# AjayAlluri/realtime-fraud-detection

Measured on AMD Instinct MI355X. Metric: scored transactions/sec (whole node), higher is better.
Workload: dtype f32 (features f64, forests f32/f64, blend f64)

## Files before the change

### include/fdengine.h

```cpp
#ifndef FDENGINE_H
#define FDENGINE_H

#include <stddef.h>
#include <stdint.h>

#ifdef __cplusplus
extern "C" {
#endif

#define FD_ABI_VERSION 15

enum fd_status {
  FD_OK = 0,
  FD_ERR_INVALID_ARG = 1,
  FD_ERR_HIP = 2,
  FD_ERR_NOT_LOADED = 3,
  FD_ERR_UNSUPPORTED = 4,
  FD_ERR_OOM = 5,
  FD_ERR_IO = 6,
};

enum fd_forest_kind {
  FD_FOREST_XGB_BINARY_LOGISTIC = 1,
  FD_FOREST_SKLEARN_IFOREST = 2,
  FD_FOREST_SKLEARN_PROBA = 3,
};

typedef struct fd_engine fd_engine;

typedef struct {
  int32_t n_trees;
  const int64_t* tree_offsets;
  const int32_t* left;
  const int32_t* right;
  const int32_t* feature;
  const double* threshold;
  const uint8_t* default_left;
  const double* leaf_value;
} fd_tree_arrays;

typedef struct {
  int32_t kind;
  int32_t num_feature;
  double base_score;
  double if_offset;
  double if_denominator;
} fd_forest_params;

#define FD_MAX_MODELS 8
enum fd_blend_strategy { FD_BLEND_WEIGHTED_AVERAGE = 0, FD_BLEND_VOTING = 1, FD_BLEND_STACKING = 2 };
enum fd_decision { FD_APPROVE = 0, FD_REVIEW = 1, FD_DECLINE = 2, FD_APPROVE_WITH_MONITORING = 3 };
enum fd_risk { FD_VERY_LOW = 0, FD_LOW = 1, FD_MEDIUM = 2, FD_HIGH = 3, FD_CRITICAL = 4 };
typedef struct {
  int32_t n_models;
  int32_t strategy;
  double weight[FD_MAX_MODELS];
  double conf_mult[FD_MAX_MODELS];
  double fraud_threshold;
  double confidence_threshold;
} fd_blend_params;

const char* fd_last_error(void);
int fd_abi_version(void);
const char* fd_build_id(void);
int fd_device_count(int* out);
int fd_engine_create(int device, fd_engine** out);
int fd_engine_destroy(fd_engine* eng);
int fd_engine_set_stream(fd_engine* eng, void* hip_stream);
int fd_engine_reset_stream(fd_engine* eng);
int fd_engine_sync(fd_engine* eng);

int fd_load_forest(fd_engine* eng, int slot, const fd_forest_params* params, const fd_tree_arrays* trees);
int fd_unload_forest(fd_engine* eng, int slot);

int fd_load_xgboost_json(fd_engine* eng, int slot, const char* path);

int fd_xgboost_json_read(const char* path, fd_forest_params* params, int32_t* n_trees, int64_t* n_nodes,
                         fd_tree_arrays* trees);
int fd_forest_info(fd_engine* eng, int slot, int32_t* n_trees, int32_t* depth, int32_t* num_feature);

int fd_forest_predict_device(fd_engine* eng, int slot, const float* d_X, int64_t n, int32_t ld,
                             double* d_prob, double* d_raw, int32_t* d_leaf);
int fd_forest_predict_host(fd_engine* eng, int slot, const float* X, int64_t n, int32_t ld,
                           double* prob, double* raw, int32_t* leaf);

typedef struct {
  int32_t n_trees;
  int32_t n_chunks;
  int32_t chunk;
  int32_t depth;
  int64_t tree_bytes;
  int64_t chunk_stride;
  int64_t blob_bytes;
  int64_t n_leaf_ids;
  float base_margin;
  int32_t layout;
  int64_t n_thresholds;
  int32_t bin_steps;
} fd_pack_info;
int fd_pack_forest_host(const fd_forest_params* params, const fd_tree_arrays* trees, void* blob,
                        int64_t blob_cap, int32_t* leaf_ids, int64_t ids_cap, fd_pack_info* info);
int fd_pack_forest_binned_host(const fd_forest_params* params, const fd_tree_arrays* trees, void* blob,
                               int64_t blob_cap, float* thresholds, int64_t thr_cap, int32_t* offsets,
                               fd_pack_info* info);

typedef struct {
  int32_t kind;
  int32_t n_trees;
  int32_t depth;
  int32_t leaf_bytes;
  int64_t n_nodes;
  int64_t n_leaves;
  float base_margin;
  int32_t pad;
} fd_sparse_info;
int fd_pack_forest_sparse_host(const fd_forest_params* params, const fd_tree_arrays* trees, void* nodes,
                               int64_t nodes_cap, void* leaf_values, int64_t values_cap, int32_t* leaf_ids,
                               int64_t ids_cap, fd_sparse_info* info);

int fd_blend_device(fd_engine* eng, const fd_blend_params* params, int64_t n,
                    const double* const* d_probs, const uint8_t* present,
                    double* d_fraud_prob, double* d_confidence, uint8_t* d_decision, uint8_t* d_risk);
int fd_blend_host(fd_engine* eng, const fd_blend_params* params, int64_t n,
                  const double* const* probs, const uint8_t* present,
                  double* fraud_prob, double* confidence, uint8_t* decision, uint8_t* risk);

enum fd_window_mode {
  FD_WINDOW_REDIS_COMPAT = 0,
  FD_WINDOW_SLIDING = 1
};
#define FD_RAW_FEATURES 16
#define FD_VECTOR_WIDTH 64
#define FD_MAX_SEQ_LEN 16
typedef struct {
  int64_t capacity;
  int32_t window_mode;
  int32_t ring_k;
  int32_t seq_len;
} fd_state_params;
int fd_state_init(fd_engine* eng, const fd_state_params* params);
int fd_state_clear(fd_engine* eng);
int fd_state_info(fd_engine* eng, int64_t* capacity, int64_t* cards);
typedef struct {
  int64_t n;
  const uint64_t* key;
  const double* avg_amount;
  const int32_t* account_age_days;
  const uint64_t* device_fp;
} fd_users;
int fd_state_load_users_host(fd_engine* eng, const fd_users* users);
typedef struct {
  int64_t n;
  const double* fraud_rate;
  const double* risk_multiplier;
} fd_merchants;
int fd_load_merchants_host(fd_engine* eng, const fd_merchants* merchants);
typedef struct {
  const uint64_t* card_key;
  const int64_t* ts_ms;
  const int64_t* amount_cents;
  const int32_t* merchant;
  const uint64_t* device_fp;
  const uint8_t* ip_class;
  const uint8_t* hour;
  const uint8_t* weekend;
} fd_txn_batch;
int fd_features_device(fd_engine* eng, const fd_txn_batch* txns, int64_t n, float* d_vectors, double* d_raw);
int fd_features_host(fd_engine* eng, const fd_txn_batch* txns, int64_t n, float* vectors, double* raw);

#define FD_FEATURE_MAP_WIDTH 64
#define FD_CODE_UNKNOWN 254
typedef struct {
  const double* geo_lat;
  const double* geo_lon;
  const double* merchant_lat;
  const double* merchant_lon;
  const uint8_t* payment_method;
  const uint8_t* transaction_type;
  const uint8_t* card_type;
  const uint8_t* user_agent_flag;
  const double* fraud_score;
} fd_txn_context;
typedef struct {
  double tp_score;
  double fe_score;
  uint8_t tp_decision;
  uint8_t tp_risk;
  uint8_t fe_decision;
  uint8_t fe_risk;
  uint8_t pad[4];
} fd_rule_scores;
typedef struct {
  int64_t n;
  const uint64_t* key;
  const double* risk_score;
  const uint8_t* kyc_status;
  const uint8_t* verified;
  const int8_t* pref_start;
  const int8_t* pref_end;
  const double* weekend_activity;
  const double* online_preference;
  const double* intl_preference;
  const int32_t* txn_frequency;
  const uint8_t* has_patterns;
} fd_users_ext;
typedef struct {
  int64_t n;
  const double* avg_amount;
  const uint8_t* risk_level;
  const uint8_t* blacklisted;
  const uint8_t* category;
  const uint8_t* high_risk_category;
  const uint8_t* open_hour;
  const uint8_t* close_hour;
  const uint8_t* suspicious_name;
} fd_merchants_ext;
int fd_state_load_users_ext_host(fd_engine* eng, const fd_users_ext* users);
int fd_load_merchants_ext_host(fd_engine* eng, const fd_merchants_ext* merchants);
int fd_load_vocab_host(fd_engine* eng, const uint8_t* payment_high_risk, const uint8_t* type_is_refund);
int fd_features_full_device(fd_engine* eng, const fd_txn_batch* txns, const fd_txn_context* ctx, int64_t n,
                            float* d_vectors, double* d_raw, double* d_fmap, fd_rule_scores* d_rules);

typedef struct {
  int32_t input_size;
  int32_t hidden;
  int32_t n_out;
  const float* w_ih;
  const float* w_hh;
  const float* b_ih;
  const float* b_hh;
  const float* w_out;
  const float* b_out;
} fd_lstm_params;
int fd_load_lstm(fd_engine* eng, const fd_lstm_params* params);
int fd_unload_lstm(fd_engine* eng);
int fd_lstm_predict_device(fd_engine* eng, const float* d_seq, int64_t n, int32_t T, double* d_prob);
int fd_lstm_predict_host(fd_engine* eng, const float* seq, int64_t n, int32_t T, double* prob);
#define FD_SLOT_LSTM 64
int fd_features_seq_device(fd_engine* eng, const fd_txn_batch* txns, int64_t n, float* d_vectors, double* d_raw,
                           float* d_seq);

typedef struct {
  int32_t n_layers;
  int32_t dims[9];
  const float* weight[8];
  const float* bias[8];
} fd_mlp_params;
int fd_load_mlp(fd_engine* eng, const fd_mlp_params* params);
int fd_unload_mlp(fd_engine* eng);
int fd_mlp_info(fd_engine* eng, int32_t* n_layers, int32_t* in_dim, int32_t* hidden);
int fd_mlp_predict_device(fd_engine* eng, const float* d_X, int64_t n, int32_t ld, double* d_prob);
int fd_mlp_predict_host(fd_engine* eng, const float* X, int64_t n, int32_t ld, double* prob);
int fd_pack_mlp_host(const fd_mlp_params* params, void* blob, int64_t cap, int64_t* bytes);
#define FD_SLOT_MLP 65

#define FD_GRAPH_FEATURES 5
typedef struct {
// ... 249 lines not shown
```

### realtime-fraud-detection_amd/csrc/engine.hip

```cpp
#include <algorithm>
#include <chrono>
#include <mutex>
#include <cstring>
#include <string>

#include "blend_row.h"
#include "abtest_row.h"
#include "fd_internal.h"
#include "graph_row.h"
#include "host_stage.h"
#include "ingest_parse.h"
#include "text_row.h"

namespace fd {

static thread_local std::string g_last_error;

void set_error(const std::string& msg) { g_last_error = msg; }

Engine::Timed* Engine::next_event_pair(int kind) {
  if (timing_every > 1 && kind >= 0 && kind < 16 && (timing_seq[kind]++ % (unsigned)timing_every) != 0)
    return nullptr;
  if (events_used == events.size()) {
    hipEvent_t a, b;
// ... 361 lines not shown
    ok = fd::comm_sync_stream(e, e.pipe_slot_stream) && ok;
    FD_REQUIRE(ok, FD_ERR_HIP, "engine leaked: streams still busy " + std::to_string(e.comm.timeout_ms) +
                                   " ms after the communicators were aborted (" + e.comm.abort_reason + ")");
  }
  (void)hipStreamSynchronize(e.stream);
  for (auto& f : e.forests) {
    for (auto* b : {&f.split.bins, &f.split.nan, &f.split.leaves}) b->release();
    f.blob.release();
    f.leaf_ids.release();
    f.b_blob.release();
    f.b_thr.release();
    f.b_thr_off.release();
  }
  e.stage.release();
  e.scratch_probs.release();
  e.feat_vec.release();
  fd::windows_release(e);
  fd::sink_release(e);
  fd::graph_release(e);
  fd::text_release(e);
  fd::ab_release(e);
  for (auto* b : {&e.route_blk, &e.route_blk_stream, &e.route_out, &e.route_err, &e.seq_buf, &e.seq_desc, &e.lstm.wpk, &e.lstm.wpk4, &e.lstm.bias,
                  &e.lstm.wout, &e.lstm.bout, &e.state.seq, &e.mlp.blob})
    b->release();
  if (e.aux_stream) {
    (void)hipStreamSynchronize(e.aux_stream);
    (void)hipStreamDestroy(e.aux_stream);
    (void)hipEventDestroy(e.fork_ev);
    (void)hipEventDestroy(e.join_ev);
  }
  if (e.aux2_stream) {
    (void)hipStreamSynchronize(e.aux2_stream);
    (void)hipStreamDestroy(e.aux2_stream);
    (void)hipEventDestroy(e.join2_ev);
  }
  try {
    fd::comm_destroy(e);
  } catch (...) {
  }
  for (hipStream_t st : e.pipe_stream)
    if (st) {
      (void)hipStreamSynchronize(st);
      (void)hipStreamDestroy(st);
    }
  if (e.pipe_slot_stream) {
    (void)hipStreamSynchronize(e.pipe_slot_stream);
    (void)hipStreamDestroy(e.pipe_slot_stream);
  }
  if (e.pipe_entry_ev) (void)hipEventDestroy(e.pipe_entry_ev);
  for (int k = 0; k < Engine::kPipeSlots; ++k) {
    if (e.pipe_slot_ev[k]) (void)hipEventDestroy(e.pipe_slot_ev[k]);
    if (e.pipe_feat_ev[k]) (void)hipEventDestroy(e.pipe_feat_ev[k]);
    if (e.pipe_copy_ev[k]) (void)hipEventDestroy(e.pipe_copy_ev[k]);
    e.pipe_vec[k].release();
    e.pipe_out[k].release();
    e.pipe_seq[k].release();
  }
  for (int k = 0; k < Engine::kSplitRing; ++k) {
    if (e.pipe_done_ev[k]) (void)hipEventDestroy(e.pipe_done_ev[k]);
    e.pipe_split[k].release();
  }
  for (auto* b : {&e.state.uext, &e.state.mext, &e.state.vocab, &e.feat_ext}) b->release();
  for (auto& P1 : e.ens1)
    for (auto* b : {&P1.nodes[0], &P1.nodes[1], &P1.thr}) b->release();
  for (auto* b : {&e.ens.nodes[0], &e.ens.nodes[1], &e.ens.thr})
    b->release();
  {
    fd::IngestTables& t = e.ingest;
    for (auto* b : {&t.mkeys, &t.mvals}) b->release();
    for (int w = 0; w < 3; ++w) {
      t.vkeys[w].release();
      t.vvals[w].release();
    }
  }
  for (auto* b : {&e.state.pages, &e.state.keys, &e.state.merchants, &e.state.err, &e.state.sat,
                  &e.state.bucket_scr})
    b->release();
  for (auto& g : e.state.gs)
    for (auto* b : {&g.slot, &g.bucket_fill, &g.pairs, &g.ovf_cnt, &g.ovf_key, &g.ovf_b, &g.prep}) b->release();
  for (auto& ev : e.events) {
    (void)hipEventDestroy(ev.a);
    (void)hipEventDestroy(ev.b);
    if (ev.c) (void)hipEventDestroy(ev.c);
    if (ev.d) (void)hipEventDestroy(ev.d);
  }
  if (e.own_stream) (void)hipStreamDestroy(e.own_stream);
  delete eng;
  FD_API_END
}

static void rebind_stream(Engine& e, hipStream_t s) {
  for (int k = 0; k < Engine::kDoneRing; ++k)
    if (e.pipe_done_live[k] && s != e.stream) FD_HIP(hipStreamWaitEvent(s, e.pipe_done_ev[k], 0));
  e.stream = s;
}

int fd_engine_set_stream(fd_engine* eng, void* hip_stream) {
  FD_API_BEGIN
  FD_ENGINE_LOCK(eng);
  Engine& e = E(eng);
  rebind_stream(e, static_cast<hipStream_t>(hip_stream));
  FD_API_END
}

int fd_engine_reset_stream(fd_engine* eng) {
  FD_API_BEGIN
  FD_ENGINE_LOCK(eng);
  Engine& e = E(eng);
  rebind_stream(e, e.own_stream);
  FD_API_END
}

int fd_engine_sync(fd_engine* eng) {
  FD_API_BEGIN
  FD_ENGINE_LOCK(eng);
  Engine& e = E(eng);
  if (e.comm.aborted) {
    bool ok = fd::comm_sync_stream(e, e.comm.x_fwd);
    ok = fd::comm_sync_stream(e, e.stream) && ok;
    for (hipStream_t st : e.pipe_stream) ok = fd::comm_sync_stream(e, st) && ok;
    for (hipStream_t st : {e.pipe_slot_stream, e.aux_stream, e.aux2_stream}) ok = fd::comm_sync_stream(e, st) && ok;
    FD_REQUIRE(ok, FD_ERR_HIP, "streams still busy " + std::to_string(e.comm.timeout_ms) +
                                   " ms after the communicators were aborted (" + e.comm.abort_reason + ")");
  }
  FD_HIP(hipStreamSynchronize(e.stream));
  if (e.comm.x_fwd) FD_HIP(hipStreamSynchronize(e.comm.x_fwd));
  for (hipStream_t st : e.pipe_stream)
    if (st) FD_HIP(hipStreamSynchronize(st));
  if (e.pipe_slot_stream) FD_HIP(hipStreamSynchronize(e.pipe_slot_stream));
  if (e.aux_stream) FD_HIP(hipStreamSynchronize(e.aux_stream));
  if (e.aux2_stream) FD_HIP(hipStreamSynchronize(e.aux2_stream));
  fd::route_check(e);
  FD_API_END
}

int fd_engine_set_timing(fd_engine* eng, int enable) {
  FD_API_BEGIN
  FD_ENGINE_LOCK(eng);
  Engine& e = E_quiet(eng);
  e.timing = enable != 0;
  FD_API_END
}

int fd_engine_get_counter(fd_engine* eng, const char* key, int64_t* value) {
  FD_API_BEGIN
  FD_ENGINE_LOCK(eng);
  Engine& e = E_quiet(eng);
  FD_REQUIRE(key && value, FD_ERR_INVALID_ARG, "null key/value");
  const std::string k(key);
  if (k == "pipelined_batches") {
    *value = (int64_t)e.pipe_iter_total;
  } else if (k == "ensemble_single_launches") {
    *value = (int64_t)e.ens_single_total;
  } else if (k == "forest_sparse_launches") {
    *value = (int64_t)e.sparse_total;
  } else if (k == "mlp_launches") {
    *value = (int64_t)e.mlp_total;
  } else if (k == "graph_steps") {
    *value = (int64_t)e.graph.steps;
  } else if (k == "text_calls") {
    *value = (int64_t)e.text.calls;
  } else if (k == "text_nonascii_rows") {
    *value = fd::text_nonascii_rows(e);
  } else if (k == "latency_prebinned_batches") {
    *value = (int64_t)e.prebin_total;
  } else if (k == "pipelined_split_batches") {
    *value = (int64_t)e.pipe_split_total;
  } else if (k == "pipelined_compact_batches") {
    *value = (int64_t)e.pipe_compact_total;
  } else if (k == "pipelined_host_ns") {
    *value = (int64_t)e.pipe_host_ns;
  } else if (k == "pipelined_slot_stream_batches") {
    *value = (int64_t)e.pipe_slot_stream_total;
  } else if (k == "window_saturated") {
    FD_REQUIRE(e.state.ready, FD_ERR_NOT_LOADED, "card state not initialised (fd_state_init)");
    FD_HIP(hipStreamSynchronize(e.stream));
    for (hipStream_t st : e.pipe_stream)
      if (st) FD_HIP(hipStreamSynchronize(st));
    unsigned long long v = 0;
    FD_HIP(hipMemcpy(&v, e.state.sat.ptr, 8, hipMemcpyDeviceToHost));
    *value = (int64_t)v;
  } else if (k == "sharded_steps") {
    *value = (int64_t)e.comm.steps.load();
  } else if (k == "rccl_ops") {
    *value = (int64_t)e.comm.ops.load();
  } else if (k.rfind("sharded_host_ns_", 0) == 0) {
    int i = 0;
    while (i < fd::ShardComm::kHostPhases && k.compare(16, std::string::npos, fd::kShardHostPhase[i]) != 0) ++i;
    FD_REQUIRE(i < fd::ShardComm::kHostPhases, FD_ERR_INVALID_ARG, "unknown counter: " + k);
    *value = (int64_t)e.comm.host_ns[i].load();
  } else {
    FD_REQUIRE(false, FD_ERR_INVALID_ARG, "unknown counter: " + k);
  }
  FD_API_END
}

int fd_engine_set_option(fd_engine* eng, const char* key, int64_t value) {
  FD_API_BEGIN
  FD_ENGINE_LOCK(eng);
  Engine& e = E_quiet(eng);
  FD_REQUIRE(key, FD_ERR_INVALID_ARG, "null key");
  const std::string k(key);
  if (k == "forest_kernel") {
    FD_REQUIRE(value == 0 || value == 1 || value == 2 || value == 3 || value == 6 || value == 8 || value == 11,
               FD_ERR_INVALID_ARG, "forest_kernel must be 0, 1, 2, 3, 6, 8 or 11");
    e.forest_variant = (int)value;
  } else if (k == "ensemble") {
    FD_REQUIRE(value == 0 || value == 1, FD_ERR_INVALID_ARG, "ensemble must be 0 or 1");
    e.ensemble_on = value != 0;
  } else if (k == "ensemble_owner") {
    FD_REQUIRE(value == 0 || value == 1, FD_ERR_INVALID_ARG, "ensemble_owner must be 0 or 1");
    e.ens_owner_fixed = value != 0;
  } else if (k == "ensemble_prio") {
    FD_REQUIRE(value == 0 || value == 1, FD_ERR_INVALID_ARG, "ensemble_prio must be 0 or 1");
    e.ens_prio = value != 0;
  } else if (k == "ensemble_chunks") {
    FD_REQUIRE(value >= 0 && value <= 2, FD_ERR_INVALID_ARG, "ensemble_chunks must be 0, 1 or 2");
    e.ens_chunks = (int)value;
  } else if (k == "compact_vectors") {
    FD_REQUIRE(value >= 0 && value <= 2, FD_ERR_INVALID_ARG, "compact_vectors must be 0, 1 or 2");
    e.compact_vectors = (int)value;
  } else if (k == "latency_fused") {
    FD_REQUIRE(value == 0 || value == 1, FD_ERR_INVALID_ARG, "latency_fused must be 0 or 1");
    e.latency_fused = value != 0;
  } else if (k == "pipeline_lean") {
    FD_REQUIRE(value == 0 || value == 1, FD_ERR_INVALID_ARG, "pipeline_lean must be 0 or 1");
    e.pipe_lean = value != 0;
  } else if (k == "pipeline_gather") {
    FD_REQUIRE(value == 0 || value == 1, FD_ERR_INVALID_ARG, "pipeline_gather must be 0 or 1");
    e.pipe_gather = value != 0;
  } else if (k == "latency_prebin") {
    FD_REQUIRE(value >= 0 && value <= 3, FD_ERR_INVALID_ARG, "latency_prebin must be 0, 1, 2 or 3");
    e.latency_prebin = value != 0;
    if (value) e.latency_prebin_mode = (int)value;
  } else if (k == "small_streams") {
    FD_REQUIRE(value >= 0 && value <= 2, FD_ERR_INVALID_ARG, "small_streams must be 0, 1 or 2");
    e.small_streams = (int)value;
  } else if (k == "count_exchange") {
    FD_REQUIRE(value >= -1 && value <= 1, FD_ERR_INVALID_ARG, "count_exchange must be -1, 0 or 1");
    FD_REQUIRE(!e.comm.pending, FD_ERR_INVALID_ARG, "count_exchange: a prefetched batch's counts are in flight");
    e.comm.count_mode = (int)value;
    e.comm.count_gather = value == 1 || (value < 0 && e.comm.world >= 4);
  } else if (k == "comm_timeout_ms") {
    FD_REQUIRE(value >= 1, FD_ERR_INVALID_ARG, "comm_timeout_ms must be >= 1");
    e.comm.timeout_ms = value;
  } else if (k == "stream_priority") {
    FD_REQUIRE(value >= 0 && value <= 3, FD_ERR_INVALID_ARG, "stream_priority must be in 0..3");
    FD_REQUIRE(!e.pipe_stream[0] && !e.comm.x_fwd, FD_ERR_INVALID_ARG,
               "stream_priority: set before the first pipelined call and fd_comm_init");
    e.stream_prio = (int)value;
  } else if (k == "bucket_keys") {
    FD_REQUIRE(value == 0 || (value >= 8 && value <= 512 && (value & (value - 1)) == 0), FD_ERR_INVALID_ARG,
               "bucket_keys must be 0 or a power of two in 8..512");
    e.state.bucket_keys = (int)value;
  } else if (k == "ensemble_bin_global") {
    FD_REQUIRE(value == 0 || value == 1, FD_ERR_INVALID_ARG, "ensemble_bin_global must be 0 or 1");
    e.ens_bin_global = value != 0;
  } else if (k == "lean_group") {
    FD_REQUIRE(value >= 0 && value <= 2, FD_ERR_INVALID_ARG, "lean_group must be 0, 1 or 2");
    e.state.lean_group = (int)value;
  } else if (k == "slot_gather") {
    FD_REQUIRE(value == 0 || value == 1, FD_ERR_INVALID_ARG, "slot_gather must be 0 or 1");
    e.state.slot_gather = value != 0;
  } else if (k == "slot_stream") {
    FD_REQUIRE(value >= -1 && value <= 2, FD_ERR_INVALID_ARG, "slot_stream must be -1, 0, 1 or 2");
    FD_REQUIRE(!e.pipe_slot_stream || (int)value == e.pipe_slot_mode, FD_ERR_INVALID_ARG,
               "slot_stream: set before the first pipelined call");
    e.pipe_slot_mode = (int)value;
  } else if (k == "slot_prio") {
    FD_REQUIRE(value == 0 || value == 1, FD_ERR_INVALID_ARG, "slot_prio must be 0 or 1");
    e.state.slot_prio = value != 0;
  } else if (k == "feature_prio") {
    FD_REQUIRE(value == 0 || value == 1, FD_ERR_INVALID_ARG, "feature_prio must be 0 or 1");
    e.state.feat_prio = value != 0;
  } else if (k == "bucket_spread") {
    FD_REQUIRE(value == 0 || value == 1, FD_ERR_INVALID_ARG, "bucket_spread must be 0 or 1");
    e.state.bucket_spread = value != 0;
  } else if (k == "timing_every") {
    FD_REQUIRE(value >= 1 && value <= 1000000, FD_ERR_INVALID_ARG, "timing_every must be >= 1");
    e.timing_every = (int)value;
    for (auto& q : e.timing_seq) q = 0;
  } else if (k == "seq_ring_lstm") {
    FD_REQUIRE(value == 0 || value == 1, FD_ERR_INVALID_ARG, "seq_ring_lstm must be 0 or 1");
    e.seq_ring_lstm = value != 0;
  } else if (k == "lstm_rows") {
    FD_REQUIRE(value == 0 || value == 4 || value == 16, FD_ERR_INVALID_ARG, "lstm_rows must be 0, 4 or 16");
    e.lstm_rows = (int)value;
  } else if (k == "mlp_form") {
    FD_REQUIRE(value == 0 || value == 1, FD_ERR_INVALID_ARG, "mlp_form must be 0 or 1");
    e.mlp_form = (int)value;
  } else if (k == "mlp_wgs_per_cu") {
    FD_REQUIRE(value >= 0 && value <= 8, FD_ERR_INVALID_ARG, "mlp_wgs_per_cu must be in 0..8");
    e.mlp_wgs_per_cu = (int)value;
  } else if (k == "ingest_stop_after") {
    FD_REQUIRE(value >= 0 && value <= 3, FD_ERR_INVALID_ARG, "ingest_stop_after must be in 0..3");
    e.ingest.stop_after = (int)value;
  } else if (k == "rule_fraud_threshold_permille") {
    FD_REQUIRE(value >= 0 && value <= 1000, FD_ERR_INVALID_ARG, "rule_fraud_threshold_permille must be in 0..1000");
    e.state.tp_threshold = (double)value / 1000.0;
  } else {
    throw fd::Error(FD_ERR_INVALID_ARG, "unknown option: " + k);
  }
  FD_API_END
}

int fd_timing_read(fd_engine* eng, int kind, double* total_ms, int64_t* launches) {
  FD_API_BEGIN
  FD_ENGINE_LOCK(eng);
  Engine& e = E_quiet(eng);
  double tot = 0.0;
  int64_t cnt = 0;
  for (size_t i = 0; i < e.events_used; ++i) {
    if (kind >= 0 && e.events[i].kind != kind) continue;
    FD_HIP(hipEventSynchronize(e.events[i].b));
    float ms = 0.f;
    FD_HIP(hipEventElapsedTime(&ms, e.events[i].a, e.events[i].b));
    tot += ms;
    if (e.events[i].split) {
      FD_HIP(hipEventSynchronize(e.events[i].d));
      FD_HIP(hipEventElapsedTime(&ms, e.events[i].c, e.events[i].d));
      tot += ms;
    }
    ++cnt;
  }
  if (total_ms) *total_ms = tot;
  if (launches) *launches = cnt;
  FD_API_END
}

int fd_timing_reset(fd_engine* eng) {
  FD_API_BEGIN
  FD_ENGINE_LOCK(eng);
  Engine& e = E_quiet(eng);
  for (size_t i = 0; i < e.events_used; ++i) {
    FD_HIP(hipEventSynchronize(e.events[i].b));
    if (e.events[i].split) FD_HIP(hipEventSynchronize(e.events[i].d));
  }
  e.events_used = 0;
  FD_API_END
}

int fd_load_forest(fd_engine* eng, int slot, const fd_forest_params* params, const fd_tree_arrays* trees) {
  FD_API_BEGIN
  FD_ENGINE_LOCK(eng);
  Engine& e = E(eng);
  FD_REQUIRE(params && trees, FD_ERR_INVALID_ARG, "null params/trees");
  fd::PackedForest& pf = slot_of(e, slot);
  FD_HIP(hipStreamSynchronize(e.stream));
  pf.loaded = false;
  fd::repack_forest(pf, *params, *trees);
  FD_API_END
}

int fd_pack_forest_host(const fd_forest_params* params, const fd_tree_arrays* trees, void* blob,
                        int64_t blob_cap, int32_t* leaf_ids, int64_t ids_cap, fd_pack_info* info) {
  FD_API_BEGIN
  FD_REQUIRE(params && trees && info, FD_ERR_INVALID_ARG, "null params/trees/info");
  const fd::HostPack hp = fd::pack_forest_host(*params, *trees);
  info->n_trees = hp.n_trees;
  info->n_chunks = hp.n_chunks;
  info->chunk = hp.chunk;
  info->depth = hp.depth;
  info->tree_bytes = (int64_t)hp.tree_bytes;
  info->chunk_stride = (int64_t)hp.chunk_stride;
  info->blob_bytes = (int64_t)hp.blob.size();
  info->n_leaf_ids = (int64_t)hp.leaf_ids.size();
  info->base_margin = hp.base_margin;
  info->layout = 0;
  info->n_thresholds = (int64_t)hp.b_thr.size();
  info->bin_steps = hp.bin_steps;
  if (blob) {
    FD_REQUIRE(blob_cap >= (int64_t)hp.blob.size(), FD_ERR_INVALID_ARG, "blob buffer too small");
    std::memcpy(blob, hp.blob.data(), hp.blob.size());
  }
  if (leaf_ids) {
    FD_REQUIRE(ids_cap >= (int64_t)hp.leaf_ids.size(), FD_ERR_INVALID_ARG, "leaf id buffer too small");
    std::memcpy(leaf_ids, hp.leaf_ids.data(), hp.leaf_ids.size() * sizeof(int32_t));
  }
  FD_API_END
}

int fd_pack_forest_binned_host(const fd_forest_params* params, const fd_tree_arrays* trees, void* blob,
                               int64_t blob_cap, float* thresholds, int64_t thr_cap, int32_t* offsets,
                               fd_pack_info* info) {
  FD_API_BEGIN
  FD_REQUIRE(params && trees && info, FD_ERR_INVALID_ARG, "null params/trees/info");
  const fd::HostPack hp = fd::pack_forest_host(*params, *trees);
  FD_REQUIRE(hp.binned, FD_ERR_UNSUPPORTED,
             "forest has no binned layout (depth > 8 or > 65534 distinct thresholds in a feature)");
  info->n_trees = hp.n_trees;
  info->n_chunks = hp.b_n_chunks;
  info->chunk = hp.b_chunk;
  info->depth = hp.depth;
  info->tree_bytes = (int64_t)hp.b_tree_bytes;
  info->chunk_stride = (int64_t)hp.b_chunk_stride;
  info->blob_bytes = (int64_t)hp.b_blob.size();
  info->n_leaf_ids = (int64_t)hp.leaf_ids.size();
  info->base_margin = hp.base_margin;
  info->layout = 1;
  info->n_thresholds = (int64_t)hp.b_thr.size();
  info->bin_steps = hp.bin_steps;
  if (blob) {
    FD_REQUIRE(blob_cap >= (int64_t)hp.b_blob.size(), FD_ERR_INVALID_ARG, "blob buffer too small");
    std::memcpy(blob, hp.b_blob.data(), hp.b_blob.size());
  }
  if (thresholds) {
    FD_REQUIRE(thr_cap >= (int64_t)hp.b_thr.size(), FD_ERR_INVALID_ARG, "threshold buffer too small");
    std::memcpy(thresholds, hp.b_thr.data(), hp.b_thr.size() * sizeof(float));
  }
  if (offsets) std::memcpy(offsets, hp.b_thr_off.data(), hp.b_thr_off.size() * sizeof(int32_t));
  FD_API_END
}

int fd_pack_forest_sparse_host(const fd_forest_params* params, const fd_tree_arrays* trees, void* nodes,
                               int64_t nodes_cap, void* leaf_values, int64_t values_cap, int32_t* leaf_ids,
                               int64_t ids_cap, fd_sparse_info* info) {
  FD_API_BEGIN
  FD_REQUIRE(params && trees && info, FD_ERR_INVALID_ARG, "null params/trees/info");
  const fd::SparsePack sp = fd::pack_forest_sparse_host(*params, *trees);
  *info = fd_sparse_info{};
  info->kind = sp.kind;
  info->n_trees = sp.n_trees;
  info->depth = sp.depth;
  info->leaf_bytes = sp.leaf_bytes;
  info->n_nodes = sp.n_nodes;
  info->n_leaves = sp.n_leaves;
  info->base_margin = sp.base_margin;
  if (nodes) {
    FD_REQUIRE(nodes_cap >= sp.n_nodes, FD_ERR_INVALID_ARG, "node buffer too small");
    std::memcpy(nodes, sp.nodes.data(), sp.nodes.size() * sizeof(uint32_t));
  }
  if (leaf_values) {
    FD_REQUIRE(values_cap >= sp.n_leaves, FD_ERR_INVALID_ARG, "leaf value buffer too small");
    std::memcpy(leaf_values, sp.leaf_val.data(), sp.leaf_val.size());
  }
  if (leaf_ids) {
    FD_REQUIRE(ids_cap >= sp.n_leaves, FD_ERR_INVALID_ARG, "leaf id buffer too small");
    std::memcpy(leaf_ids, sp.leaf_ids.data(), sp.leaf_ids.size() * sizeof(int32_t));
  }
  FD_API_END
}

int fd_load_xgboost_json(fd_engine* eng, int slot, const char* path) {
  FD_API_BEGIN
  FD_ENGINE_LOCK(eng);
  Engine& e = E(eng);
  fd::PackedForest& pf = slot_of(e, slot);
  fd::XgbModel m;
  fd::read_xgboost_json(path, m);
  fd_forest_params p{};
  p.kind = FD_FOREST_XGB_BINARY_LOGISTIC;
  p.num_feature = m.num_feature;
  p.base_score = m.base_score;
  fd_tree_arrays t{};
  t.n_trees = (int32_t)(m.offsets.size() - 1);
  t.tree_offsets = m.offsets.data();
  t.left = m.left.data();
  t.right = m.right.data();
  t.feature = m.feature.data();
  t.threshold = m.threshold.data();
  t.default_left = m.default_left.data();
  t.leaf_value = m.leaf_value.data();
  FD_REQUIRE(t.n_trees > 0, FD_ERR_INVALID_ARG, "xgboost json: no trees");
  FD_HIP(hipStreamSynchronize(e.stream));
  pf.loaded = false;
  fd::repack_forest(pf, p, t);
  FD_API_END
}

int fd_xgboost_json_read(const char* path, fd_forest_params* params, int32_t* n_trees, int64_t* n_nodes,
                         fd_tree_arrays* trees) {
  FD_API_BEGIN
  fd::XgbModel m;
  fd::read_xgboost_json(path, m);
  const int32_t T = (int32_t)(m.offsets.size() - 1);
  const int64_t M = (int64_t)m.left.size();
  if (params) {
    *params = fd_forest_params{};
    params->kind = FD_FOREST_XGB_BINARY_LOGISTIC;
    params->num_feature = m.num_feature;
    params->base_score = m.base_score;
  }
  if (n_trees) *n_trees = T;
  if (n_nodes) *n_nodes = M;
  if (trees) {
    FD_REQUIRE(trees->tree_offsets && trees->left && trees->right && trees->feature && trees->threshold &&
                   trees->default_left && trees->leaf_value,
               FD_ERR_INVALID_ARG, "incomplete output arrays");
    trees->n_trees = T;
    std::memcpy(const_cast<int64_t*>(trees->tree_offsets), m.offsets.data(), (size_t)(T + 1) * 8);
    std::memcpy(const_cast<int32_t*>(trees->left), m.left.data(), (size_t)M * 4);
    std::memcpy(const_cast<int32_t*>(trees->right), m.right.data(), (size_t)M * 4);
    std::memcpy(const_cast<int32_t*>(trees->feature), m.feature.data(), (size_t)M * 4);
    std::memcpy(const_cast<double*>(trees->threshold), m.threshold.data(), (size_t)M * 8);
    std::memcpy(const_cast<uint8_t*>(trees->default_left), m.default_left.data(), (size_t)M);
    std::memcpy(const_cast<double*>(trees->leaf_value), m.leaf_value.data(), (size_t)M * 8);
  }
  FD_API_END
}

int fd_unload_forest(fd_engine* eng, int slot) {
  FD_API_BEGIN
  FD_ENGINE_LOCK(eng);
  Engine& e = E(eng);
  fd::PackedForest& pf = slot_of(e, slot);
  FD_HIP(hipStreamSynchronize(e.stream));
  pf.blob.release();
  pf.leaf_ids.release();
  pf.b_blob.release();
  pf.b_thr.release();
  pf.b_thr_off.release();
  for (auto* b : {&pf.split.bins, &pf.split.nan, &pf.split.leaves}) b->release();
  for (auto* b : {&pf.sp.nodes, &pf.sp.leaf_val, &pf.sp.leaf_ids}) b->release();
  pf.sp.gen = 0;
  pf.sparse_only = false;
  pf.binned = false;
  pf.loaded = false;
  pf.gen = 0;
  FD_API_END
}

int fd_forest_info(fd_engine* eng, int slot, int32_t* n_trees, int32_t* depth, int32_t* num_feature) {
  FD_API_BEGIN
  FD_ENGINE_LOCK(eng);
  Engine& e = E(eng);
  fd::PackedForest& pf = slot_of(e, slot);
  FD_REQUIRE(pf.loaded, FD_ERR_NOT_LOADED, "Model in slot " + std::to_string(slot) + " not loaded");
  if (n_trees) *n_trees = pf.n_trees;
  if (depth) *depth = pf.depth;
  if (num_feature) *num_feature = pf.num_feature;
  FD_API_END
}

int fd_forest_predict_device(fd_engine* eng, int slot, const float* d_X, int64_t n, int32_t ld,
// ... 105 lines not shown
  st.out(dr, raw, (size_t)n * FD_RAW_FEATURES);
  st.upload();
  fd::launch_features(e, d, n, dv, dr);
  st.download(false);
  fd::features_check(e);
  FD_API_END
}

int fd_score_matrix_device(fd_engine* eng, const fd_blend_params* params, const int32_t* slots,
                           const double* const* ext_probs, const uint8_t* present, const float* d_X,
                           int64_t n, int32_t ld, double* d_model_probs, double* d_fraud_prob,
                           double* d_confidence, uint8_t* d_decision, uint8_t* d_risk) {
  FD_API_BEGIN
  FD_ENGINE_LOCK(eng);
  Engine& e = E(eng);
  FD_REQUIRE(params && d_X && ld > 0 && n >= 0, FD_ERR_INVALID_ARG, "bad arguments");
  score_matrix(e, *params, slots, ext_probs, present, d_X, n, ld, d_model_probs, d_fraud_prob, d_confidence,
               d_decision, d_risk);
  FD_API_END
}

int fd_score_matrix_host(fd_engine* eng, const fd_blend_params* params, const int32_t* slots,
                         const double* const* ext_probs, const uint8_t* present, const float* X, int64_t n,
                         int32_t ld, double* model_probs, double* fraud_prob, double* confidence,
                         uint8_t* decision, uint8_t* risk) {
  FD_API_BEGIN
  FD_ENGINE_LOCK(eng);
  Engine& e = E(eng);
  FD_REQUIRE(params && slots && X && fraud_prob && ld > 0 && n >= 0, FD_ERR_INVALID_ARG, "bad arguments");
  FD_REQUIRE(params->n_models > 0 && params->n_models <= FD_MAX_MODELS, FD_ERR_INVALID_ARG, "n_models out of range");
  if (n == 0) return FD_OK;
  const int M = params->n_models;
  Stage st(e);
  const float* dX;
  const double* dext[FD_MAX_MODELS] = {};
  double *dMP, *dfp, *dconf;
  uint8_t *ddec, *drisk;
  st.in(dX, X, (size_t)n * ld);
  for (int m = 0; m < M; ++m) {
    if (slots[m] >= 0 || (present && !present[m])) continue;
    FD_REQUIRE(ext_probs && ext_probs[m], FD_ERR_INVALID_ARG, "model without slot needs an external probability column");
    st.in(dext[m], ext_probs[m], (size_t)n);
  }
  st.out(dMP, model_probs, (size_t)n * M);
  st.out(dfp, fraud_prob, (size_t)n);
  st.out(dconf, confidence, (size_t)n);
  st.out(ddec, decision, (size_t)n);
  st.out(drisk, risk, (size_t)n);
  st.upload();
  score_matrix(e, *params, slots, dext, present, dX, n, ld, dMP, dfp, dconf, ddec, drisk);
  st.download();
  FD_API_END
}

static void score_batch_body(Engine& e, const fd_blend_params& p, const int32_t* slots, const double* const* ext,
                             const uint8_t* present, const fd_txn_batch& t, int64_t n, float* d_vectors,
                             double* dMP, double* dfp, double* dconf, uint8_t* ddec, uint8_t* drisk) {
  float* vec = d_vectors;
  if (!vec) {
    e.feat_vec.ensure((size_t)n * FD_VECTOR_WIDTH * 4);
    vec = e.feat_vec.as<float>();
  }
  float* seq = lstm_seq_buffer(e, p, slots, present, n);
  unsigned long long* desc = nullptr;
  if (seq && e.seq_ring_lstm && n < 4096 && (e.lstm_rows == 0 || e.lstm_rows == 4)) {
    e.seq_desc.ensure((size_t)n * sizeof(unsigned long long));
    desc = e.seq_desc.as<unsigned long long>();
    if (!e.state.slot_gather) FD_HIP(hipMemsetAsync(desc, 0xff, (size_t)n * sizeof(unsigned long long), e.stream));
  }
  fd::launch_features(e, t, n, vec, nullptr, seq, nullptr, nullptr, false, 0, nullptr, false, desc);
  score_matrix(e, p, slots, ext, present, vec, n, FD_VECTOR_WIDTH, dMP, dfp, dconf, ddec, drisk, seq, e.state.S,
               nullptr, nullptr, false, desc);
}

int fd_score_batch_device(fd_engine* eng, const fd_blend_params* params, const int32_t* slots,
                          const double* const* ext_probs, const uint8_t* present, const fd_txn_batch* txns,
                          int64_t n, float* d_vectors, double* d_model_probs, double* d_fraud_prob,
                          double* d_confidence, uint8_t* d_decision, uint8_t* d_risk) {
  FD_API_BEGIN
  FD_ENGINE_LOCK(eng);
  Engine& e = E(eng);
  FD_REQUIRE(params && txns && n >= 0, FD_ERR_INVALID_ARG, "bad arguments");
  if (n == 0) return FD_OK;
  FD_REQUIRE(slots != nullptr && d_fraud_prob != nullptr, FD_ERR_INVALID_ARG, "null slots/output");
  score_batch_body(e, *params, slots, ext_probs, present, *txns, n, d_vectors, d_model_probs, d_fraud_prob,
                   d_confidence, d_decision, d_risk);
  FD_API_END
}

__global__ void __launch_bounds__(256)
pipe_out_copy_kernel(const double* __restrict__ fp, const double* __restrict__ conf, const uint8_t* __restrict__ dec,
                     const uint8_t* __restrict__ risk, const double* __restrict__ mp, int n_mp, int64_t n,
                     double* __restrict__ o_fp, double* __restrict__ o_conf, uint8_t* __restrict__ o_dec,
                     uint8_t* __restrict__ o_risk, double* __restrict__ o_mp, const float4* __restrict__ vec,
                     float4* __restrict__ o_vec, const uint64_t* __restrict__ res, uint64_t* __restrict__ o_res) {
  const int64_t i = (int64_t)blockIdx.x * blockDim.x + threadIdx.x;
  const int64_t stride = (int64_t)gridDim.x * blockDim.x;
  if (o_vec) {
    const int64_t total = n * (FD_VECTOR_WIDTH / 4);
    for (int64_t q = i; q < total; q += stride) o_vec[q] = vec[q];
  }
  if (o_res) {
    const int64_t total = n * (int64_t)(sizeof(fd::ResultRecord) / 8);
    for (int64_t q = i; q < total; q += stride) o_res[q] = res[q];
  }
  if (i >= n) return;
  if (o_fp) o_fp[i] = fp[i];
  if (o_conf) o_conf[i] = conf[i];
  if (o_dec) o_dec[i] = dec[i];
  if (o_risk) o_risk[i] = risk[i];
  for (int m = 0; m < n_mp; ++m) o_mp[(size_t)m * n + i] = mp[(size_t)m * n + i];
}

static void pipe_step(Engine& e, const fd_blend_params* params, const int32_t* slots, const double* const* ext_probs,
                      const uint8_t* present, const fd_txn_batch* txns, const void* records, int64_t n,
                      float* d_vectors, double* d_model_probs, double* d_fraud_prob, double* d_confidence,
                      uint8_t* d_decision, uint8_t* d_risk, void* d_results, void* input_ready,
                      bool results_in_place = false) {
  for (int k = 0; k < 2; ++k)
    if (!e.pipe_stream[k]) e.pipe_stream[k] = fd::make_stream(e.stream_prio >= 1 ? 1 : 0);
  if (e.pipe_slot_mode < 0)
    e.pipe_slot_mode = (e.state.ready && e.state.cap >= (1ll << 26)) ? 2 : 0;
  if (e.pipe_slot_mode && !e.pipe_slot_stream) {
    e.pipe_slot_stream = fd::make_stream(e.pipe_slot_mode == 1 ? 1 : -1);
    for (int k = 0; k < Engine::kPipeSlots; ++k) FD_HIP(hipEventCreateWithFlags(&e.pipe_slot_ev[k], kStreamEventFlags));
  }
  if (!e.pipe_entry_ev) {
    FD_HIP(hipEventCreateWithFlags(&e.pipe_entry_ev, kStreamEventFlags));
    for (int k = 0; k < Engine::kPipeSlots; ++k) {
      FD_HIP(hipEventCreateWithFlags(&e.pipe_feat_ev[k], kStreamEventFlags));
      FD_HIP(hipEventCreateWithFlags(&e.pipe_copy_ev[k], kStreamEventFlags));
    }
    for (int k = 0; k < Engine::kDoneRing; ++k) FD_HIP(hipEventCreateWithFlags(&e.pipe_done_ev[k], kStreamEventFlags));
  }
  constexpr int nbuf = 2;
  const int s = (int)(e.pipe_iter % (unsigned long long)nbuf);
  const int prev = s ^ 1;
  hipStream_t Sc = e.pipe_stream[e.pipe_iter & 1];
  hipStream_t Sf = Sc;
  hipStream_t Ss = e.pipe_slot_stream;
  if (e.pipe_dirty) {
    FD_HIP(hipEventRecord(e.pipe_entry_ev, e.stream));
    FD_HIP(hipStreamWaitEvent(Sf, e.pipe_entry_ev, 0));
    if (Ss) FD_HIP(hipStreamWaitEvent(Ss, e.pipe_entry_ev, 0));
    e.pipe_dirty = false;
  }
  if (input_ready) FD_HIP(hipStreamWaitEvent(Sf, static_cast<hipEvent_t>(input_ready), 0));
  if (Ss && input_ready) FD_HIP(hipStreamWaitEvent(Ss, static_cast<hipEvent_t>(input_ready), 0));
  if (Ss && e.pipe_feat_live[s]) FD_HIP(hipStreamWaitEvent(Ss, e.pipe_feat_ev[s], 0));
  if (e.pipe_copy_live[s] && e.pipe_copy_vec[s]) FD_HIP(hipStreamWaitEvent(Sf, e.pipe_copy_ev[s], 0));
  hipEvent_t before_buckets = e.pipe_feat_live[prev] ? e.pipe_feat_ev[prev] : nullptr;
  int compact = (e.compact_vectors && d_vectors == nullptr && fd::ensemble_applies(e, *params, slots, present, n))
                    ? e.compact_vectors : 0;
  e.pipe_vec[s].ensure((size_t)n * FD_VECTOR_WIDTH * 4);
  float* vec = e.pipe_vec[s].as<float>();
  const int sr = (int)(e.pipe_iter % (unsigned long long)Engine::kSplitRing);
  float* seq = nullptr;
  bool want_seq = false;
  for (int m = 0; m < params->n_models && m < FD_MAX_MODELS; ++m)
    want_seq = want_seq || (slots && slots[m] == FD_SLOT_LSTM && !(present && !present[m]));
  if (want_seq) {
    FD_REQUIRE(e.state.ready && e.state.S > 0, FD_ERR_INVALID_ARG,
               "the LSTM head needs card history: fd_state_params.seq_len > 0");
    e.pipe_seq[s].ensure((size_t)n * e.state.S * fd::kSeqInput * sizeof(float));
    seq = e.pipe_seq[s].as<float>();
  }
  const bool lean = e.pipe_lean && !(e.pipe_gather && e.state.slot_gather && n <= fd::kGatherBatchMax && !Ss);
  if (compact == 2 && (!lean || want_seq || e.state.S > 0)) compact = 1;
  if (compact == 2) {
    e.pipe_split[sr].ensure((size_t)n * 64);
    vec = e.pipe_split[sr].as<float>();
    if (Ss && e.pipe_done_live[sr]) FD_HIP(hipStreamWaitEvent(Ss, e.pipe_done_ev[sr], 0));
  }
  {
    struct SlotPass {
      Engine& e;
      ~SlotPass() { e.slot_pass_stream = nullptr, e.slot_pass_ev = nullptr; }
    } slot_pass{e};
    e.slot_pass_stream = Ss;
    e.slot_pass_ev = Ss ? e.pipe_slot_ev[s] : nullptr;
    if (records)
      fd::launch_features_records(e, records, n, vec, seq, Sf, lean, s, before_buckets, compact);
    else
      fd::launch_features(e, *txns, n, vec, nullptr, seq, nullptr, Sf, lean, s, before_buckets, compact);
  }
  FD_HIP(hipEventRecord(e.pipe_feat_ev[s], Sf));
  e.pipe_feat_live[s] = true;
  const int pr = (sr + Engine::kDoneRing - 1) % Engine::kDoneRing;
  if (e.pipe_done_live[pr] && !compact && !fd::ensemble_applies(e, *params, slots, present, n))
    FD_HIP(hipStreamWaitEvent(Sc, e.pipe_done_ev[pr], 0));
  const int n_mp = d_model_probs ? params->n_models : 0;
  const size_t n8 = (size_t)n * 8, a8 = ((size_t)n + 7) & ~(size_t)7;
  const bool in_place = records && results_in_place;
  const size_t rbytes = records && !in_place ? (size_t)n * sizeof(fd::ResultRecord) : 0;
  e.pipe_out[s].ensure((2 + (size_t)n_mp) * n8 + 2 * a8 + rbytes);
  char* so = e.pipe_out[s].as<char>();
  double* s_fp = reinterpret_cast<double*>(so);
  double* s_conf = (d_confidence || records) ? reinterpret_cast<double*>(so + n8) : nullptr;
  double* s_mp = n_mp ? reinterpret_cast<double*>(so + 2 * n8) : nullptr;
  uint8_t* s_dec = (d_decision || records) ? reinterpret_cast<uint8_t*>(so + (2 + (size_t)n_mp) * n8) : nullptr;
  uint8_t* s_risk = (d_risk || records) ? reinterpret_cast<uint8_t*>(so + (2 + (size_t)n_mp) * n8 + a8) : nullptr;
  auto* s_res = !records ? nullptr
                         : in_place ? static_cast<fd::ResultRecord*>(d_results)
                                    : reinterpret_cast<fd::ResultRecord*>(so + (2 + (size_t)n_mp) * n8 + 2 * a8);
  if (e.pipe_copy_live[s]) FD_HIP(hipStreamWaitEvent(Sc, e.pipe_copy_ev[s], 0));
  ++e.pipe_iter;
  ++e.pipe_iter_total;
  e.pipe_compact_total += compact != 0;
  e.pipe_split_total += compact == 2;
  e.pipe_slot_stream_total += Ss != nullptr;
  {
    struct Swap {
      Engine& e;
      hipStream_t saved;
      ~Swap() { e.stream = saved; }
    } swap{e, e.stream};
    e.stream = Sc;
    const auto* rec = static_cast<const fd::RouteRecord*>(records);
    if (!score_matrix(e, *params, slots, ext_probs, present, vec, n, FD_VECTOR_WIDTH, s_mp, s_fp, s_conf, s_dec,
                      s_risk, seq, e.state.S, rec, s_res, compact) &&
        records)
      fd::launch_result_pack(e, s_fp, s_conf, s_dec, s_risk, rec, n, s_res);
  }
  FD_HIP(hipEventRecord(e.pipe_done_ev[sr], Sc));
  e.pipe_done_live[sr] = true;
  FD_HIP(hipStreamWaitEvent(e.stream, e.pipe_done_ev[sr], 0));
  if (in_place) {
    e.pipe_copy_live[s] = false;
    return;
  }
  hipLaunchKernelGGL(pipe_out_copy_kernel, dim3((unsigned)((n + 255) / 256)), dim3(256), 0, e.stream, s_fp, s_conf,
                     s_dec, s_risk, s_mp, n_mp, n, records ? nullptr : d_fraud_prob, d_confidence, d_decision, d_risk,
                     d_model_probs, reinterpret_cast<const float4*>(vec), reinterpret_cast<float4*>(d_vectors),
                     reinterpret_cast<const uint64_t*>(s_res), static_cast<uint64_t*>(d_results));
  FD_HIP(hipGetLastError());
  FD_HIP(hipEventRecord(e.pipe_copy_ev[s], e.stream));
  e.pipe_copy_live[s] = true;
  e.pipe_copy_vec[s] = d_vectors != nullptr;
}

int fd_score_batch_pipelined(fd_engine* eng, const fd_blend_params* params, const int32_t* slots,
                             const double* const* ext_probs, const uint8_t* present, const fd_txn_batch* txns,
                             int64_t n, float* d_vectors, double* d_model_probs, double* d_fraud_prob,
                             double* d_confidence, uint8_t* d_decision, uint8_t* d_risk, void* input_ready) {
  FD_API_BEGIN
  FD_ENGINE_LOCK(eng);
  Engine& e = E_quiet(eng);
  FD_REQUIRE(params && txns && n >= 0, FD_ERR_INVALID_ARG, "bad arguments");
  if (n == 0) return FD_OK;
  FD_REQUIRE(d_fraud_prob != nullptr, FD_ERR_INVALID_ARG, "null fraud_prob output");
  FD_REQUIRE(params->n_models >= 1 && params->n_models <= FD_MAX_MODELS, FD_ERR_INVALID_ARG, "bad n_models");
  const auto t0 = std::chrono::steady_clock::now();
  pipe_step(e, params, slots, ext_probs, present, txns, nullptr, n, d_vectors, d_model_probs, d_fraud_prob,
            d_confidence, d_decision, d_risk, nullptr, input_ready);
  e.pipe_host_ns += (unsigned long long)std::chrono::duration_cast<std::chrono::nanoseconds>(
                        std::chrono::steady_clock::now() - t0).count();
  FD_API_END
}

int fd_score_records_pipelined(fd_engine* eng, const fd_blend_params* params, const int32_t* slots,
                               const uint8_t* present, const void* d_records, int64_t n, void* d_results,
                               void* input_ready) {
  FD_API_BEGIN
  FD_ENGINE_LOCK(eng);
  Engine& e = E_quiet(eng);
  FD_REQUIRE(params && slots && n >= 0, FD_ERR_INVALID_ARG, "bad arguments");
  FD_REQUIRE(params->n_models >= 1 && params->n_models <= FD_MAX_MODELS, FD_ERR_INVALID_ARG, "bad n_models");
  for (int m = 0; m < params->n_models; ++m)
    FD_REQUIRE(slots[m] >= 0 || (present && !present[m]), FD_ERR_INVALID_ARG,
               "routed scoring needs every present model in a forest slot, FD_SLOT_LSTM or FD_SLOT_MLP");
  if (n == 0) return FD_OK;
  FD_REQUIRE(d_records != nullptr && d_results != nullptr, FD_ERR_INVALID_ARG, "null records / results");
  pipe_step(e, params, slots, nullptr, present, nullptr, d_records, n, nullptr, nullptr, nullptr, nullptr, nullptr,
            nullptr, d_results, input_ready);
  FD_API_END
}

extern "C++" hipStream_t fd::make_stream(int level) {
  hipStream_t st = nullptr;
  if (level == 0) {
    FD_HIP(hipStreamCreateWithFlags(&st, hipStreamNonBlocking));
    return st;
  }
  int least = 0, greatest = 0;
  FD_HIP(hipDeviceGetStreamPriorityRange(&least, &greatest));
  FD_HIP(hipStreamCreateWithPriority(&st, hipStreamNonBlocking, level > 0 ? greatest : least));
  return st;
}

int fd_comm_unique_id(const char* rccl_path, uint8_t* id_out) {
  FD_API_BEGIN
  FD_REQUIRE(id_out, FD_ERR_INVALID_ARG, "null id");
  fd::comm_unique_id(rccl_path, id_out);
  FD_API_END
}

int fd_comm_init(fd_engine* eng, const char* rccl_path, int32_t rank, int32_t world, const uint8_t* id_fwd,
                 const uint8_t* id_back) {
  FD_API_BEGIN
  FD_ENGINE_LOCK(eng);
  Engine& e = E_quiet(eng);
  fd::comm_init(e, rccl_path, rank, world, id_fwd, id_back);
  FD_API_END
}

int fd_comm_destroy(fd_engine* eng) {
  FD_API_BEGIN
  FD_ENGINE_LOCK(eng);
  Engine& e = E_quiet(eng);
  fd::comm_destroy(e);
  FD_API_END
}

int fd_sharded_step(fd_engine* eng, const fd_blend_params* params, const int32_t* slots, const uint8_t* present,
                    const fd_txn_batch* txns, int64_t n, uint64_t batch_id, void* input_ready,
                    const fd_txn_batch* next, int64_t next_n, uint64_t next_id, void* next_ready,
                    double* d_fraud_prob, double* d_confidence, uint8_t* d_decision, uint8_t* d_risk,
                    int64_t* split_sizes) {
  FD_API_BEGIN
  FD_ENGINE_LOCK(eng);
  Engine& e = E_quiet(eng);
  fd::ShardComm& c = e.comm;
  FD_REQUIRE(c.ready, FD_ERR_NOT_LOADED, "no communicators (fd_comm_init)");
  FD_REQUIRE(!c.aborted, FD_ERR_HIP, "communicators aborted (" + c.abort_reason + "): fd_comm_destroy, then fd_comm_init");
  FD_REQUIRE(params && slots && txns && n >= 0 && (!next || next_n >= 0), FD_ERR_INVALID_ARG, "bad arguments");
// ... 943 lines not shown
```

### realtime-fraud-detection_amd/csrc/ensemble.hip

```cpp
#include <algorithm>
#include <atomic>
#include <cstring>

#include "blend_row.h"
#include "walk_common.h"

namespace fd {

static std::atomic<uint64_t> g_forest_gen{0};

void forest_loaded(PackedForest& pf, const fd_forest_params& p, const fd_tree_arrays& t) {
  pf.gen = ++g_forest_gen;
  pf.params = p;
  const int64_t m = t.tree_offsets[t.n_trees];
  pf.t_off.assign(t.tree_offsets, t.tree_offsets + t.n_trees + 1);
  pf.t_left.assign(t.left, t.left + m);
  pf.t_right.assign(t.right, t.right + m);
  pf.t_feature.assign(t.feature, t.feature + m);
  pf.t_threshold.assign(t.threshold, t.threshold + m);
  pf.t_leaf.assign(t.leaf_value, t.leaf_value + m);
  if (t.default_left)
    pf.t_dleft.assign(t.default_left, t.default_left + m);
  else
    pf.t_dleft.assign((size_t)m, 0);
}

namespace {

constexpr int kEnsWG = 1024;
constexpr int kMaxPass = 64;

template <bool WIDE>
struct EnsCfg {
  static constexpr int CHA = WIDE ? 24 : 20;
  static constexpr int CHB = WIDE ? 16 : 12;
  static constexpr uint32_t BUF = (uint32_t)(CHA * (1024 + 256 * 4) > CHB * (1024 + 256 * 8) ? CHA * (1024 + 256 * 4)
                                                                                             : CHB * (1024 + 256 * 8));
};
inline uint32_t ens_buf(bool wide) { return wide ? EnsCfg<true>::BUF : EnsCfg<false>::BUF; }
constexpr uint32_t kEnsTile = 4u * kTile * 8u;

__host__ __device__ constexpr uint32_t ens_xs_bytes(int nf) { return (uint32_t)((nf + 1) / 2) * 1024u; }

size_t ens_lds(int nf, bool wide) {
  return (size_t)ens_xs_bytes(nf) + 2 * (size_t)ens_buf(wide) + 2 * (size_t)kEnsTile + kTile * 4 + kTile * 8 + 128 +
         1024;
}

struct EnsArgs {
  const float* X;
  int64_t n;
  int ld, nf;
  const float* thr;
  int vec4;
  int compact;
  int owner_fixed;
  int prio;
  int n_pass;
  int pad0;
  unsigned long long pass_global;
  const char* img;
  const char* nodes[2];
  int n_chunks[2];
  int stride[2];
  float base_margin;
  int pad1;
  double if_offset, if_denom;
  int pos[2];
  int mcol[2];
  double* mp;
  double* fp;
  double* conf;
  uint8_t* dec;
  uint8_t* risk;
  const RouteRecord* rec;
  ResultRecord* res;
  int pass_f[kMaxPass + 1];
  int img_off[kMaxPass + 1];
  int thr_off[kMaxFeatures + 1];
  uint16_t cbin[kMaxFeatures];
  alignas(4) uint16_t lut[8 * 32];
  BlendConsts blend;
#ifdef FD_FOREST_PROFILE
  int prof_slot;
  int clk_slot;
#endif
};

constexpr uint32_t kLinkMask = 0x3F8u;

template <int D, int TPG, bool NAN_AWARE>
__device__ __forceinline__ void walk_ens(uint32_t buf, int t0, uint32_t lane4, uint32_t (&leaf)[TPG]) {
  uint32_t tb[TPG], node[TPG], kl[TPG], kr[TPG], xw[TPG];
#pragma unroll
  for (int j = 0; j < TPG; ++j) {
    tb[j] = buf + (uint32_t)(t0 + j) * 1024u;
    asm volatile("" : "+v"(tb[j]));
    node[j] = lds_load<uint32_t>(tb[j] + 4u);
  }
#pragma unroll
  for (int j = 0; j < TPG; ++j) {
    xw[j] = lds_load<uint16_t>((node[j] & 0xFC02u) | lane4);
    if (D > 1) {
      const u32x2 k = lds_load<u32x2>(tb[j] + 8u);
      kl[j] = k.x;
      kr[j] = k.y;
    }
  }
#pragma unroll
  for (int l = 0; l < D; ++l) {
#pragma unroll
    for (int j = 0; j < TPG; ++j) {
      bool right = xw[j] > (node[j] >> 16);
      if (NAN_AWARE) {
        if (xw[j] == 0xFFFFu) right = (node[j] & 1u) == 0u;
      }
      if (l + 1 < D) {
        uint32_t a = kl[j], b = kr[j];
        asm volatile("" : "+v"(a), "+v"(b));
        node[j] = right ? b : a;
        xw[j] = lds_load<uint16_t>((node[j] & 0xFC02u) | lane4);
        if (l + 2 < D) {
          const u32x2 k = lds_load<u32x2>((node[j] & kLinkMask) | tb[j]);
          kl[j] = k.x;
          kr[j] = k.y;
        }
      } else {
        leaf[j] = ((node[j] & kLinkMask) >> 2) + (right ? 1u : 0u);
      }
    }
  }
}

template <int D, int TPG>
__device__ __forceinline__ unsigned long long walk_pack(uint32_t cur, int gg, uint32_t lane4, bool tile_nan) {
  static_assert(TPG <= 8, "a byte per tree in a u64");
  uint32_t leaf[TPG];
  if (tile_nan)
    walk_ens<D, TPG, true>(cur, gg * TPG, lane4, leaf);
  else
    walk_ens<D, TPG, false>(cur, gg * TPG, lane4, leaf);
  uint32_t lo = 0, hi = 0;
#pragma unroll
  for (int j = 0; j < TPG; ++j) {
    if (j < 4) lo |= leaf[j] << (8 * j);
    else hi |= leaf[j] << (8 * (j - 4));
  }
  return ((unsigned long long)hi << 32) | lo;
}

template <int D, int TPG, int CH, typename LeafT>
__device__ __forceinline__ void owner_sum(uint32_t buf, uint32_t tile, uint32_t acc, int txn) {
  constexpr int NL = 1 << D;
  unsigned long long w[4];
#pragma unroll
  for (int q = 0; q < 4; ++q) w[q] = lds_load<unsigned long long>(tile + (uint32_t)(q * kTile + txn) * 8u);
  LeafT v[CH];
#pragma unroll
  for (int t = 0; t < CH; ++t) {
    const uint32_t idx = (uint32_t)(w[t / TPG] >> (8 * (t % TPG))) & 0xFFu;
    v[t] = lds_load<LeafT>(buf + (uint32_t)(CH * 1024) + ((uint32_t)(t * NL) + idx) * (uint32_t)sizeof(LeafT));
  }
  LeafT s = lds_load<LeafT>(acc + (uint32_t)txn * (uint32_t)sizeof(LeafT));
#pragma unroll
  for (int t = 0; t < CH; ++t) s += v[t];
  lds_store<LeafT>(acc + (uint32_t)txn * (uint32_t)sizeof(LeafT), s);
}

__device__ __forceinline__ void stage_pieces(const char* __restrict__ src, uint32_t dst, int bytes, int nparts,
                                             int part) {
  const int lane = threadIdx.x & 63;
  const int pieces = bytes >> 10;
  for (int p = part; p < pieces; p += nparts) {
    const char* g = src + (p << 10) + lane * 16;
    const uint32_t m0 = __builtin_amdgcn_readfirstlane(dst + ((uint32_t)p << 10));
    asm volatile(
        "s_mov_b32 m0, %0\n\t"
        "s_nop 0\n\t"
        "global_load_lds_dwordx4 %1, off"
        :
        : "s"(m0), "v"(g)
        : "memory", "m0");
  }
}

__host__ __device__ __forceinline__ int thr_pad(int g) { return g + (g >> 5); }

#ifdef FD_FOREST_PROFILE
constexpr int kEprofSlots = 4;
__device__ unsigned long long g_eprof[kEprofSlots * 256 * 16 * 16];
static int g_eprof_next = 0;
constexpr int kEclkSlots = 1024;
__device__ unsigned long long g_eclk[kEclkSlots * 4 * 4];
static int g_eclk_next = 0;
#define FD_ESTAMP(var) const unsigned long long var = __builtin_amdgcn_s_memtime()
#else
#define FD_ESTAMP(var)
#endif

template <int L>
__device__ __forceinline__ void search_lockstep(const float (&vv)[L], const int (&o)[L], const int (&cnt)[L],
                                                int (&pos)[L], int steps, bool glob, uint32_t tl, int o0,
                                                const float* __restrict__ thr) {
  if (!glob) {
    for (int st = steps; st > 0; st >>= 1) {
      float t[L];
#pragma unroll
      for (int k = 0; k < L; ++k) {
        const int np = pos[k] + st;
        const int idx = np <= cnt[k] ? np - 1 : 0;
        t[k] = lds_load<float>(tl + (uint32_t)thr_pad(o[k] - o0 + idx) * 4u);
      }
#pragma unroll
      for (int k = 0; k < L; ++k) {
        const int np = pos[k] + st;
        pos[k] = (np <= cnt[k] && t[k] <= vv[k]) ? np : pos[k];
      }
    }
  } else {
    for (int st = steps; st > 0; st >>= 1) {
      float t[L];
#pragma unroll
      for (int k = 0; k < L; ++k) {
        const int np = pos[k] + st;
        t[k] = thr[o[k] + (np <= cnt[k] ? np - 1 : 0)];
      }
#pragma unroll
      for (int k = 0; k < L; ++k) {
        const int np = pos[k] + st;
        pos[k] = (np <= cnt[k] && t[k] <= vv[k]) ? np : pos[k];
      }
    }
  }
}

template <int Q>
__device__ __forceinline__ void bin_compact_constants(const EnsArgs& a, uint16_t* Xs, int txn) {
  uint32_t* X32 = reinterpret_cast<uint32_t*>(Xs);
#pragma unroll
  for (int j = Q; j < kMaxFeatures / 2; j += 4) {
    const int f = 2 * j;
    const bool c0 = compact_src(f) < 0 && f < a.nf, c1 = compact_src(f + 1) < 0 && f + 1 < a.nf;
    if (c0 && c1)
      X32[j * 256 + txn] = (uint32_t)a.cbin[f] | ((uint32_t)a.cbin[f + 1] << 16);
    else if (c0)
      Xs[j * 512 + txn * 2] = a.cbin[f];
    else if (c1)
      Xs[j * 512 + txn * 2 + 1] = a.cbin[f + 1];
  }
}

constexpr int kLutN = 32;
static_assert(kIntSlots * kLutN == 8 * 32, "EnsArgs::lut");
constexpr int kIntOf[4][6] = {{-1, 2, -1, 6, -1, -1}, {-1, 3, 5, -1, -1, -1}, {0, 4, -1, -1, -1, -1},
                              {1, -1, -1, 7, -1, -1}};
constexpr int kNSearched[4] = {4, 4, 3, 3};
constexpr int kSearched[4][4] = {{0, 2, 4, 5}, {0, 3, 4, 5}, {2, 3, 4, 0}, {1, 2, 4, 0}};
constexpr bool int_tables_agree() {
  for (int q = 0; q < 4; ++q) {
    int ns = 0;
    for (int i = 0; i < 6; ++i) {
      const int ci = q + 4 * i;
      const int want = ci < kCompactSlots ? int_slot(ci) : -1;
      if (kIntOf[q][i] != want) return false;
      if (ci < kCompactSlots && want < 0) {
        if (ns >= 4 || kSearched[q][ns] != i) return false;
        ++ns;
      }
    }
    if (ns != kNSearched[q]) return false;
  }
  return true;
}
static_assert(int_tables_agree(), "kIntOf / kSearched must follow kIntCompact and kCompactSlot");

template <int Q>
__device__ __forceinline__ void load_compact(const float* __restrict__ xr, float (&v)[16]) {
  const unsigned long long ib = *reinterpret_cast<const unsigned long long*>(xr + 14);
#pragma unroll
  for (int i = 0; i < 6; ++i) {
    const int ci = Q + 4 * i;
    if (ci >= kCompactSlots) {
      v[i] = 0.f;
    } else if (int_slot(ci) >= 0) {
      v[i] = (float)(unsigned)((ib >> (8 * int_slot(ci))) & 0xFFull);
    } else {
      v[i] = xr[compact_word(ci)];
    }
  }
}

template <int Q>
__device__ __forceinline__ void load_split(const uint4* __restrict__ ra, const uint4* __restrict__ rb,
                                           float (&v)[16]) {
  const uint4 a0 = ra[0], a1 = ra[1], b0 = rb[0], b1 = rb[1];
  const unsigned fa = a1.w >> 24;
  const int na = (fa & 1u) ? 1 : 0;
  const int nu = ((b1.z >> 8) & 1u) ? 1 : 0;
  const int nc = ((b1.y >> 8) & 0xFFu) ? 1 : 0;
  const int n2 = na + nu + nc;
  auto byte = [](unsigned w, int k) { return (float)((w >> (8 * k)) & 0xFFu); };
#pragma unroll
  for (int i = 0; i < 6; ++i) {
    const int ci = Q + 4 * i;
    float x = 0.f;
    switch (ci) {
      case 0: x = __uint_as_float(a0.x); break;
      case 1: x = __uint_as_float(a0.y); break;
      case 2: x = byte(a1.w, 0); break;
      case 3: x = byte(a1.w, 1); break;
      case 4: x = byte(a1.w, 2); break;
      case 5: x = byte(b1.y, 0); break;
      case 6: x = byte(b1.y, 1); break;
      case 7: x = __uint_as_float(b0.x); break;
      case 8: x = __uint_as_float(b0.y); break;
      case 9: x = byte(b1.y, 2); break;
      case 10: x = __uint_as_float(a0.w); break;
      case 11: x = __uint_as_float(a1.x); break;
      case 12: x = byte(b1.y, 3); break;
      case 13: x = __uint_as_float(a1.y); break;
      case 14: x = __uint_as_float(b0.z); break;
      case 15: x = byte(b1.z, 0); break;
      default:
        if (ci < kCompactSlots) {
          const int k = ci - 16;
          const float first = (na && k == 0) ? __uint_as_float(a0.z)
                                             : ((nu && k == na) ? __uint_as_float(b0.w) : __uint_as_float(b1.x));
          const int t = k - n2;
          x = k < n2 ? first
                     : (t == 0 ? __uint_as_float(a1.z)
                               : (t == 1 ? ((fa & 2u) ? 1.f : 0.f) : (t == 2 ? ((fa & 4u) ? 1.f : 0.f) : 0.f)));
        }
        break;
    }
    v[i] = x;
  }
}

template <int Q, int L, bool LUT>
__device__ __forceinline__ void bin_compact_pass(const EnsArgs& a, const float (&v)[16], uint16_t* Xs,
                                                 int txn, int f0, int f1, bool glob, uint32_t tl, int o0,
                                                 int& anynan, uint32_t lut) {
  constexpr int NV = (kCompactSlots - Q + 3) / 4;
  constexpr int NS = LUT ? kNSearched[Q] : NV;
#pragma unroll
  for (int i = 0; i < NV; ++i) {
    const int ks = LUT ? kIntOf[Q][i] : -1;
    if (ks < 0) continue;
    const int f = kCompactSlot[Q + 4 * i];
    if (!(f >= f0 && f < f1 && f < a.nf)) continue;
    const float x = v[i];
    uint16_t bin;
    if (x != x) {
      anynan = 1;
      bin = (uint16_t)0xFFFFu;
    } else if (x >= 0.f && x < (float)kLutN && x == truncf(x)) {
      bin = lds_load<uint16_t>(lut + (uint32_t)(ks * kLutN + (int)x) * 2u);
    } else {
      const int o = a.thr_off[f], cnt = a.thr_off[f + 1] - o;
      int pos = 0;
#pragma unroll
      for (int st = 1 << 15; st > 0; st >>= 1)
        if (pos + st <= cnt && a.thr[o + pos + st - 1] <= x) pos += st;
      bin = (uint16_t)pos;
    }
    Xs[(f >> 1) * 512 + txn * 2 + (f & 1)] = bin;
  }
#pragma unroll
  for (int g0 = 0; g0 < NS; g0 += L) {
    float vv[L];
    int o[L], cnt[L], pos[L];
    bool act[L];
    int steps = 0;
#pragma unroll
    for (int k = 0; k < L; ++k) {
      const int i = LUT ? kSearched[Q][g0 + k < NS ? g0 + k : 0] : (g0 + k < NS ? g0 + k : 0);
      const int f = kCompactSlot[Q + 4 * i];
      act[k] = g0 + k < NS && f >= f0 && f < f1 && f < a.nf;
      vv[k] = act[k] ? v[i] : 0.f;
      o[k] = act[k] ? a.thr_off[f] : o0;
      cnt[k] = act[k] ? a.thr_off[f + 1] - o[k] : 0;
      pos[k] = 0;
      steps = max(steps, lift_steps(cnt[k]));
    }
    search_lockstep<L>(vv, o, cnt, pos, steps, glob, tl, o0, a.thr);
#pragma unroll
    for (int k = 0; k < L; ++k) {
      const int i = LUT ? kSearched[Q][g0 + k < NS ? g0 + k : 0] : (g0 + k < NS ? g0 + k : 0);
      const int f = kCompactSlot[Q + 4 * i];
      if (act[k]) {
        const bool nan = vv[k] != vv[k];
        anynan |= nan ? 1 : 0;
        Xs[(f >> 1) * 512 + txn * 2 + (f & 1)] = nan ? (uint16_t)0xFFFFu : (uint16_t)pos[k];
      }
    }
  }
}

template <int D, int OUT, bool WIDE, bool LUT = true>
__global__ void __launch_bounds__(kEnsWG) ensemble_kernel(EnsArgs a) {
  constexpr int kCHA = EnsCfg<WIDE>::CHA, kCHB = EnsCfg<WIDE>::CHB;
  constexpr uint32_t kEnsBuf = EnsCfg<WIDE>::BUF;
  constexpr int TPGA = kCHA / 4, TPGB = kCHB / 4;
  extern __shared__ __attribute__((aligned(16))) char smem[];
  const uint32_t sdyn = (uint32_t)(size_t)((lds_char*)smem);
  const uint32_t s0 = (sdyn + 1023u) & ~1023u;
  char* const lbase = smem + (s0 - sdyn);
  const int tid = threadIdx.x, wave = tid >> 6, lane = tid & 63;
  const int gg = __builtin_amdgcn_readfirstlane(wave >> 2);
  const int txn = ((wave & 3) << 6) + lane;
  const uint32_t lane4 = s0 + (uint32_t)txn * 4u;
  const uint32_t bufA = s0 + ens_xs_bytes(a.nf), bufB = bufA + kEnsBuf;
  const uint32_t tile0 = bufB + kEnsBuf, tile1 = tile0 + kEnsTile;
  const uint32_t accA = tile1 + kEnsTile, accB = accA + kTile * 4;
  const uint32_t flags = accB + kTile * 8, owner_cnt = flags + 64;
  const int64_t row = (int64_t)blockIdx.x * kTile + txn;
  const bool valid = row < a.n;
  const int nA = a.n_chunks[0], G = nA + a.n_chunks[1];

#ifdef FD_FOREST_PROFILE
  unsigned long long pr_top = 0, pr_walk = 0, pr_sync = 0, pr_dma = 0, pr_st[8] = {0, 0, 0, 0, 0, 0, 0, 0};
#endif
  FD_ESTAMP(pr_t0);
#ifdef FD_FOREST_PROFILE
  const unsigned long long pr_rt0 = __builtin_amdgcn_s_memrealtime();
#endif
  {
    const int k_prio = a.prio, k_compact = a.compact, k_npass = a.n_pass, k_vec4 = a.vec4, k_ld = a.ld;
    const unsigned long long k_pg = a.pass_global;
    const float* k_x = a.X;
    const char* k_img = a.img;
    const int k_i0 = a.img_off[0], k_i1 = a.img_off[1], k_f1 = a.pass_f[1];
    asm volatile("" ::"s"(k_prio), "s"(k_compact), "s"(k_npass), "s"(k_vec4), "s"(k_ld), "s"(k_pg), "s"(k_x),
                 "s"(k_img), "s"(k_i0), "s"(k_i1), "s"(k_f1), "s"(nA), "s"(G), "s"(a.n));
  }
  if (a.prio) __builtin_amdgcn_s_setprio(2);
  int anynan = 0;
  const bool early0 = G > 0 && a.n_pass == 1 && (a.pass_global & 1ull) != 0;
  {
    uint16_t* Xs = reinterpret_cast<uint16_t*>(lbase);
    const int q = __builtin_amdgcn_readfirstlane(tid >> 8);
    const int fq = q * 16;
    float v[16];
    if (valid && a.compact == 2) {
      const uint4* ra = reinterpret_cast<const uint4*>(a.X) + 2 * row;
      const uint4* rb = reinterpret_cast<const uint4*>(a.X) + 2 * (a.n + row);
      switch (q) {
        case 0: load_split<0>(ra, rb, v); bin_compact_constants<0>(a, Xs, txn); break;
        case 1: load_split<1>(ra, rb, v); bin_compact_constants<1>(a, Xs, txn); break;
        case 2: load_split<2>(ra, rb, v); bin_compact_constants<2>(a, Xs, txn); break;
        default: load_split<3>(ra, rb, v); bin_compact_constants<3>(a, Xs, txn); break;
      }
    } else if (valid && a.compact) {
      const float* xr = a.X + row * (int64_t)kCompactWidth;
      switch (q) {
        case 0: load_compact<0>(xr, v); bin_compact_constants<0>(a, Xs, txn); break;
        case 1: load_compact<1>(xr, v); bin_compact_constants<1>(a, Xs, txn); break;
        case 2: load_compact<2>(xr, v); bin_compact_constants<2>(a, Xs, txn); break;
        default: load_compact<3>(xr, v); bin_compact_constants<3>(a, Xs, txn); break;
      }
    } else if (valid) {
      const float* xr = a.X + row * (int64_t)a.ld;
      const int ncopy = a.ld < a.nf ? a.ld : a.nf;
      if (a.vec4 && fq + 16 <= ncopy) {
        const float4* x4 = reinterpret_cast<const float4*>(xr + fq);
#pragma unroll
        for (int k = 0; k < 4; ++k) {
          const float4 t = x4[k];
          v[4 * k] = t.x;
          v[4 * k + 1] = t.y;
          v[4 * k + 2] = t.z;
          v[4 * k + 3] = t.w;
        }
      } else {
#pragma unroll
        for (int k = 0; k < 16; ++k) v[k] = fq + k < ncopy ? xr[fq + k] : __builtin_nanf("");
      }
    }
    if (a.n_pass > 0 && !(a.pass_global & 1ull))
      stage_pieces(a.img + a.img_off[0], bufA, a.img_off[1] - a.img_off[0], kEnsWG / 64, wave);
    if (early0) stage_chunk_asm(nA > 0 ? a.nodes[0] : a.nodes[1], bufA, nA > 0 ? a.stride[0] : a.stride[1], kEnsWG / 64);
#ifdef FD_FOREST_PROFILE
    pr_st[0] = __builtin_amdgcn_s_memtime();
#endif
    if (LUT && a.compact && tid < kIntSlots * kLutN / 2)
      lds_store<uint32_t>(accA + (uint32_t)tid * 4u, reinterpret_cast<const uint32_t*>(a.lut)[tid]);
    constexpr int kLock = 4;
    for (int p = 0; p < a.n_pass; ++p) {
      const int f0 = a.pass_f[p], f1 = a.pass_f[p + 1];
      const bool glob = (a.pass_global >> p) & 1ull;
      const int o0 = a.thr_off[f0];
      const uint32_t tl = bufA;
      if (!glob) {
        if (p > 0)
          stage_pieces(a.img + a.img_off[p], bufA, a.img_off[p + 1] - a.img_off[p], kEnsWG / 64, wave);
        dma_wait();
        __syncthreads();
      } else if (LUT && a.compact && p == 0) {
        __syncthreads();
      }
#ifdef FD_FOREST_PROFILE
      if (p < 3) pr_st[1 + 2 * p] = __builtin_amdgcn_s_memtime();
#endif
      if (LUT && valid && a.compact) {
        switch (q) {
          case 0: bin_compact_pass<0, kLock, true>(a, v, Xs, txn, f0, f1, glob, tl, o0, anynan, accA); break;
          case 1: bin_compact_pass<1, kLock, true>(a, v, Xs, txn, f0, f1, glob, tl, o0, anynan, accA); break;
          case 2: bin_compact_pass<2, kLock, true>(a, v, Xs, txn, f0, f1, glob, tl, o0, anynan, accA); break;
          default: bin_compact_pass<3, kLock, true>(a, v, Xs, txn, f0, f1, glob, tl, o0, anynan, accA); break;
        }
      } else if (valid && a.compact) {
        switch (q) {
          case 0: bin_compact_pass<0, kLock, false>(a, v, Xs, txn, f0, f1, glob, tl, o0, anynan, accA); break;
          case 1: bin_compact_pass<1, kLock, false>(a, v, Xs, txn, f0, f1, glob, tl, o0, anynan, accA); break;
          case 2: bin_compact_pass<2, kLock, false>(a, v, Xs, txn, f0, f1, glob, tl, o0, anynan, accA); break;
          default: bin_compact_pass<3, kLock, false>(a, v, Xs, txn, f0, f1, glob, tl, o0, anynan, accA); break;
        }
      } else if (valid) {
#pragma unroll
        for (int kk = 0; kk < 16; kk += kLock) {
          const int fb = fq + kk;
          if (fb + kLock - 1 < f0 || fb >= f1) continue;
          float vv[kLock];
          int o[kLock], cnt[kLock], pos[kLock];
          bool act[kLock];
          int steps = 0;
#pragma unroll
          for (int k = 0; k < kLock; ++k) {
            const int f = fb + k;
            act[k] = f >= f0 && f < f1;
            vv[k] = act[k] ? v[kk + k] : 0.f;
            o[k] = act[k] ? a.thr_off[f] : o0;
            cnt[k] = act[k] ? a.thr_off[f + 1] - o[k] : 0;
            pos[k] = 0;
            steps = max(steps, lift_steps(cnt[k]));
          }
          if (!glob) {
            for (int st = steps; st > 0; st >>= 1) {
              float t[kLock];
#pragma unroll
              for (int k = 0; k < kLock; ++k) {
                const int np = pos[k] + st;
                const int idx = np <= cnt[k] ? np - 1 : 0;
                t[k] = lds_load<float>(tl + (uint32_t)thr_pad(o[k] - o0 + idx) * 4u);
              }
#pragma unroll
              for (int k = 0; k < kLock; ++k) {
                const int np = pos[k] + st;
                pos[k] = (np <= cnt[k] && t[k] <= vv[k]) ? np : pos[k];
              }
            }
          } else {
            for (int st = steps; st > 0; st >>= 1) {
              float t[kLock];
#pragma unroll
              for (int k = 0; k < kLock; ++k) {
                const int np = pos[k] + st;
                t[k] = a.thr[o[k] + (np <= cnt[k] ? np - 1 : 0)];
              }
#pragma unroll
              for (int k = 0; k < kLock; ++k) {
                const int np = pos[k] + st;
                pos[k] = (np <= cnt[k] && t[k] <= vv[k]) ? np : pos[k];
              }
            }
          }
#pragma unroll
          for (int k = 0; k < kLock; ++k) {
            const int f = fb + k;
            if (act[k]) {
              const bool nan = vv[k] != vv[k];
              anynan |= nan ? 1 : 0;
              Xs[(f >> 1) * 512 + txn * 2 + (f & 1)] = nan ? (uint16_t)0xFFFFu : (uint16_t)pos[k];
            }
          }
        }
      }
      __syncthreads();
#ifdef FD_FOREST_PROFILE
      if (p < 3) pr_st[2 + 2 * p] = __builtin_amdgcn_s_memtime();
#endif
    }
  }
  if (G > 0 && !early0)
    stage_pieces(nA > 0 ? a.nodes[0] : a.nodes[1], bufA, nA > 0 ? a.stride[0] : a.stride[1], kEnsWG / 64, wave);
  if (gg == 0) {
    lds_store<float>(accA + txn * 4, a.base_margin);
    lds_store<double>(accB + txn * 8, 0.0);
  }
  if (tid == 0) lds_store<uint32_t>(owner_cnt, 0u);
  dma_wait();
  const bool tile_nan = tile_any(anynan, reinterpret_cast<uint32_t*>(lbase + (flags - s0)), kEnsWG / 64);

  FD_ESTAMP(pr_t1);
  for (int g = 0; g < G; ++g) {
    FD_ESTAMP(q0);
    const bool owner = gg == (a.owner_fixed ? 0 : ((g - 1) & 3));
    if (owner) {
      if (g > 0) {
        const int c = g - 1;
        const uint32_t bp = (c & 1) ? bufB : bufA, tp = (c & 1) ? tile1 : tile0;
        if (c < nA) owner_sum<D, TPGA, kCHA, float>(bp, tp, accA, txn);
        else owner_sum<D, TPGB, kCHB, double>(bp, tp, accB, txn);
        if (lane == 0)
          __hip_atomic_fetch_add(reinterpret_cast<uint32_t*>(lbase + (owner_cnt - s0)), 1u, __ATOMIC_RELAXED,
                                 __HIP_MEMORY_SCOPE_WORKGROUP);
        while (__hip_atomic_load(reinterpret_cast<uint32_t*>(lbase + (owner_cnt - s0)), __ATOMIC_RELAXED,
                                 __HIP_MEMORY_SCOPE_WORKGROUP) < 4u * (uint32_t)g)
          __builtin_amdgcn_s_sleep(1);
      }
      if (g + 1 < G) {
        const int h = g + 1, fb = h >= nA ? 1 : 0;
        stage_pieces(a.nodes[fb] + (size_t)(fb ? h - nA : h) * a.stride[fb], (g & 1) ? bufA : bufB, a.stride[fb], 4,
                  wave & 3);
      }
    }
    const uint32_t cur = (g & 1) ? bufB : bufA, tw = (g & 1) ? tile1 : tile0;
    FD_ESTAMP(q1);
    const unsigned long long w =
        g < nA ? walk_pack<D, TPGA>(cur, gg, lane4, tile_nan) : walk_pack<D, TPGB>(cur, gg, lane4, tile_nan);
    lds_store<unsigned long long>(tw + (uint32_t)(gg * kTile + txn) * 8u, w);
    FD_ESTAMP(q2);
    if (owner) dma_wait();
#ifdef FD_FOREST_PROFILE
    const unsigned long long q2d = __builtin_amdgcn_s_memtime();
#endif
    __syncthreads();
#ifdef FD_FOREST_PROFILE
    const unsigned long long q3 = __builtin_amdgcn_s_memtime();
    pr_top += q1 - q0;
    pr_walk += q2 - q1;
    pr_dma += q2d - q2;
    pr_sync += q3 - q2;
#endif
  }
  if (G > 0 && gg == (a.owner_fixed ? 0 : ((G - 1) & 3))) {
    const int c = G - 1;
    const uint32_t bp = (c & 1) ? bufB : bufA, tp = (c & 1) ? tile1 : tile0;
    if (c < nA) owner_sum<D, TPGA, kCHA, float>(bp, tp, accA, txn);
    else owner_sum<D, TPGB, kCHB, double>(bp, tp, accB, txn);
  }
  __syncthreads();
#ifdef FD_FOREST_PROFILE
  if (lane == 0 && blockIdx.x < 256) {
    unsigned long long* o = g_eprof + (size_t)a.prof_slot * 256 * 16 * 16 + ((size_t)blockIdx.x * 16 + wave) * 16;
    for (int k = 0; k < 7; ++k) o[6 + k] = pr_st[k] ? pr_st[k] - pr_t0 : 0;
    o[0] = pr_t1 - pr_t0;
    o[1] = pr_top;
    o[2] = pr_walk;
    o[3] = pr_sync;
    o[13] = pr_dma;
    o[4] = pr_t0;
    o[5] = __builtin_amdgcn_s_memtime();
    o[14] = pr_rt0;
    o[15] = __builtin_amdgcn_s_memrealtime();
    if (wave == 0 && (blockIdx.x & 63) == 0) {
      unsigned long long* c = g_eclk + ((size_t)a.clk_slot * 4 + (blockIdx.x >> 6)) * 4;
      c[0] = pr_t0;
      c[1] = o[5];
      c[2] = pr_rt0;
      c[3] = o[15];
    }
  }
#endif
  if (gg != 0 || !valid) return;

  double pa, pb;
  {
    const float mg = lds_load<float>(accA + txn * 4);
    const float xm = fminf(-mg, 88.7f);
    const float denom = expf(xm) + 1.0f + 1e-16f;
    pa = (double)(1.0f / denom);
  }
  {
    const double d = lds_load<double>(accB + txn * 8);
    const double qd = (a.if_denom != 0.0) ? d / a.if_denom : 1.0;
    const double score = pow(2.0, -qd);
    const double decision = -score - a.if_offset;
    pb = 1.0 / (1.0 + exp(decision));
  }
  if (OUT == 2) {
    a.fp[row] = nA > 0 ? pa : pb;
    if (a.mp) a.mp[row] = nA > 0 ? (double)lds_load<float>(accA + txn * 4) : lds_load<double>(accB + txn * 8);
    return;
  }
  double raw[FD_MAX_MODELS];
#pragma unroll
  for (int m = 0; m < FD_MAX_MODELS; ++m) raw[m] = m == a.pos[0] ? pa : (m == a.pos[1] ? pb : 0.0);
  if (a.mp) {
    a.mp[(size_t)a.mcol[0] * a.n + row] = pa;
    a.mp[(size_t)a.mcol[1] * a.n + row] = pb;
  }
  double fp, conf;
  uint8_t dec, risk;
  blend_row(a.blend, raw, fp, conf, dec, risk);
  if (OUT == 0) {
    a.fp[row] = fp;
    if (a.conf) a.conf[row] = conf;
    if (a.dec) a.dec[row] = dec;
    if (a.risk) a.risk[row] = risk;
  } else {
    ResultRecord r;
    r.fraud_prob = fp;
    r.confidence = conf;
    r.seq = a.rec[row].seq;
    r.decision = dec;
    r.risk = risk;
    r.pad = 0;
    a.res[row] = r;
  }
}

template <int OUT, bool WIDE>
const void* pick_ensemble(int D) {
  switch (D) {
    case 1: return (const void*)ensemble_kernel<1, OUT, WIDE>;
    case 2: return (const void*)ensemble_kernel<2, OUT, WIDE>;
    case 3: return (const void*)ensemble_kernel<3, OUT, WIDE>;
    case 4: return (const void*)ensemble_kernel<4, OUT, WIDE>;
    case 5: return (const void*)ensemble_kernel<5, OUT, WIDE>;
    case 6: return (const void*)ensemble_kernel<6, OUT, WIDE>;
    case 7: return (const void*)ensemble_kernel<7, OUT, WIDE>;
    case 8: return (const void*)ensemble_kernel<8, OUT, WIDE>;
    default: return nullptr;
  }
}

const void* pick_ensemble(int out, bool wide, int D) {
  if (wide) return out == 1 ? pick_ensemble<1, true>(D) : out == 2 ? pick_ensemble<2, true>(D) : pick_ensemble<0, true>(D);
  return out == 1 ? pick_ensemble<1, false>(D) : out == 2 ? pick_ensemble<2, false>(D) : pick_ensemble<0, false>(D);
}

fd_tree_arrays arrays_of(const PackedForest& f) {
  fd_tree_arrays t{};
  t.n_trees = f.n_trees;
  t.tree_offsets = f.t_off.data();
  t.left = f.t_left.data();
  t.right = f.t_right.data();
  t.feature = f.t_feature.data();
  t.threshold = f.t_threshold.data();
  t.default_left = f.t_dleft.data();
  t.leaf_value = f.t_leaf.data();
  return t;
}

void plan_passes(const std::vector<float>& thr, const std::vector<int32_t>& off, int nf, bool wide, EnsPassSet& ps,
                 std::vector<float>& img) {
  const size_t stage_floats = (2 * (size_t)ens_buf(wide) + 2 * (size_t)kEnsTile) / 4;
  ps = EnsPassSet{};
  ps.f.push_back(0);
  ps.img_off.push_back((int)(img.size() * 4));
  int f = 0;
  while (f < nf) {
    int g = f;
    while (g < nf && (size_t)(off[g + 1] - off[f]) + (size_t)(off[g + 1] - off[f]) / 32 + 1 <= stage_floats) ++g;
    const int np = (int)ps.f.size() - 1;
    FD_REQUIRE(np < kMaxPass, FD_ERR_UNSUPPORTED, "ensemble binning plan too long");
    if (g == f) {
      ps.glob |= 1ull << np;
      g = f + 1;
    } else {
      const int cnt = off[g] - off[f];
      const size_t words = cnt > 0 ? (size_t)thr_pad(cnt - 1) + 1 : 0;
      const size_t base = img.size();
      img.resize(base + (words + 255) / 256 * 256, 0.f);
      for (int i = 0; i < cnt; ++i) img[base + (size_t)thr_pad(i)] = thr[(size_t)off[f] + i];
    }
    ps.f.push_back(g);
    ps.img_off.push_back((int)(img.size() * 4));
    f = g;
  }
}

bool build_plan(Engine& e, EnsemblePlan& P, int sa, int sb, bool wide) {
  P.valid = false;
  const PackedForest* F[2] = {sa >= 0 ? &e.forests[sa] : nullptr, sb >= 0 ? &e.forests[sb] : nullptr};
  if (!F[0] && !F[1]) return false;
  int D = 0, nf = -1;
  for (const PackedForest* f : F) {
    if (!f) continue;
    if (f->sparse_only || !f->binned || f->t_off.empty() || (nf >= 0 && f->num_feature != nf)) return false;
    nf = f->num_feature;
    D = std::max(D, f->depth);
  }
  if (D > 8) return false;
  if (ens_lds(nf, wide) > kLdsBudget) return false;
  HostPack hp[2];
  for (int k = 0; k < 2; ++k) {
    if (!F[k]) continue;
    hp[k] = pack_forest_host(F[k]->params, arrays_of(*F[k]), D);
    if (!hp[k].binned || hp[k].depth != D) return false;
  }
  std::vector<std::vector<float>> merged(nf);
  for (int f = 0; f < nf; ++f) {
    for (int k = 0; k < 2; ++k) {
      if (!F[k]) continue;
      const HostPack& h = hp[k];
      merged[f].insert(merged[f].end(), h.b_thr.begin() + h.b_thr_off[f], h.b_thr.begin() + h.b_thr_off[f + 1]);
    }
    std::sort(merged[f].begin(), merged[f].end());
    merged[f].erase(std::unique(merged[f].begin(), merged[f].end()), merged[f].end());
    if (merged[f].size() > (size_t)kMaxBins) return false;
  }
  std::vector<float> thr;
  std::vector<int32_t> off(nf + 1, 0);
  int maxc = 0;
  for (int f = 0; f < nf; ++f) {
    thr.insert(thr.end(), merged[f].begin(), merged[f].end());
    off[f + 1] = (int32_t)thr.size();
    maxc = std::max(maxc, (int)merged[f].size());
  }
  const int NL = 1 << D;
  const int CH[2] = {wide ? EnsCfg<true>::CHA : EnsCfg<false>::CHA, wide ? EnsCfg<true>::CHB : EnsCfg<false>::CHB};
  const size_t leaf_sz[2] = {sizeof(float), sizeof(double)};
  for (int k = 0; k < 2; ++k) {
    if (!F[k]) {
      P.n_trees[k] = P.n_chunks[k] = 0;
      P.CH[k] = CH[k];
      P.stride[k] = 0;
      continue;
    }
    const HostPack& h = hp[k];
    const int T = h.n_trees, nc = (T + CH[k] - 1) / CH[k];
    const size_t leaf_bytes = (size_t)CH[k] * NL * leaf_sz[k];
    const size_t stride = ((size_t)CH[k] * 1024 + leaf_bytes + 1023) / 1024 * 1024;
    FD_REQUIRE(stride <= ens_buf(wide), FD_ERR_UNSUPPORTED, "ensemble chunk exceeds its LDS buffer");
    std::vector<char> blob((size_t)nc * stride, 0);
    for (int i = 0; i < T; ++i) {
      const char* src = h.b_blob.data() + (size_t)(i / h.b_chunk) * h.b_chunk_stride + (size_t)(i % h.b_chunk) *
                                                                                          h.b_tree_bytes;
      char* chunk = blob.data() + (size_t)(i / CH[k]) * stride;
      uint32_t* dst = reinterpret_cast<uint32_t*>(chunk + (size_t)(i % CH[k]) * 1024);
      for (int s = 1; s < NL; ++s) {
        uint32_t w;
        std::memcpy(&w, src + (size_t)s * 4, 4);
        const uint32_t f = (w >> 10) & 63u;
        if (!h.pad[(size_t)i * NL + s]) {
          const int j = (int)(w >> 16);
          const float t = h.b_thr[h.b_thr_off[f] + j];
          const uint32_t jm = (uint32_t)(std::lower_bound(merged[f].begin(), merged[f].end(), t) - merged[f].begin());
          w = (jm << 16) | (w & 0xFFFFu);
        }
        const uint32_t link = s < (NL >> 1) ? (uint32_t)s : (uint32_t)(s - (NL >> 1));
        dst[s] = (w & 0xFFFF0001u) | ((f >> 1) << 10) | (link << 3) | ((f & 1u) << 1);
      }
      std::memcpy(chunk + (size_t)CH[k] * 1024 + (size_t)(i % CH[k]) * NL * leaf_sz[k], src + (size_t)NL * 4,
                  (size_t)NL * leaf_sz[k]);
    }
    P.nodes[k].ensure(blob.size());
    FD_HIP(hipMemcpy(P.nodes[k].ptr, blob.data(), blob.size(), hipMemcpyHostToDevice));
    P.n_trees[k] = T;
    P.CH[k] = CH[k];
    P.n_chunks[k] = nc;
    P.stride[k] = stride;
  }
  P.thr.ensure(std::max<size_t>(4, thr.size() * sizeof(float)));
  if (!thr.empty()) FD_HIP(hipMemcpy(P.thr.ptr, thr.data(), thr.size() * sizeof(float), hipMemcpyHostToDevice));
  P.h_thr_off = off;
  P.h_cbin.assign(kMaxFeatures, 0);
  for (int f = 0; f < nf && f < kMaxFeatures; ++f) {
    const int src = compact_src(f);
    if (src >= 0) continue;
    const float val = src == -2 ? 0.5f : 0.0f;
    P.h_cbin[f] = (uint16_t)(std::upper_bound(merged[f].begin(), merged[f].end(), val) - merged[f].begin());
  }
  {
    std::vector<uint16_t> lut((size_t)kIntSlots * kLutN, 0);
    for (int k = 0; k < kIntSlots; ++k) {
      const int f = kCompactSlot[kIntCompact[k]];
      if (f >= nf) continue;
      for (int x = 0; x < kLutN; ++x)
        lut[(size_t)k * kLutN + x] =
            (uint16_t)(std::upper_bound(merged[f].begin(), merged[f].end(), (float)x) - merged[f].begin());
    }
    P.h_lut = lut;
  }
  {
    std::vector<float> img;
    plan_passes(thr, off, nf, wide, P.passes, img);
    P.img.ensure(std::max<size_t>(1024, img.size() * sizeof(float)));
    if (!img.empty()) FD_HIP(hipMemcpy(P.img.ptr, img.data(), img.size() * sizeof(float), hipMemcpyHostToDevice));
  }
  P.max_feature_thr = maxc;
  P.slot[0] = sa;
  P.slot[1] = sb;
  P.gen[0] = F[0] ? F[0]->gen : 0;
  P.gen[1] = F[1] ? F[1]->gen : 0;
  P.n_forests = (F[0] ? 1 : 0) + (F[1] ? 1 : 0);
  P.D = D;
  P.nf = nf;
  P.wide = wide;
  P.kind[0] = FD_FOREST_XGB_BINARY_LOGISTIC;
  P.kind[1] = FD_FOREST_SKLEARN_IFOREST;
  P.base_margin = F[0] ? hp[0].base_margin : 0.f;
  P.if_offset = F[1] ? F[1]->if_offset : 0.0;
  P.if_denominator = F[1] ? F[1]->if_denominator : 0.0;
  P.valid = true;
  return true;
}

bool plan_current(const Engine& e, const EnsemblePlan& P, int sa, int sb, bool wide) {
  return P.valid && P.wide == wide && P.slot[0] == sa && P.slot[1] == sb &&
         P.gen[0] == (sa >= 0 ? e.forests[sa].gen : 0) && P.gen[1] == (sb >= 0 ? e.forests[sb].gen : 0);
}

bool want_wide(const Engine& e) { return e.ens_chunks == 1 || (e.ens_chunks == 0 && !e.comm.ready); }

}

#ifdef FD_FOREST_PROFILE
extern "C" __attribute__((visibility("default"))) int fd_debug_ens_profile(unsigned long long* out, int n) {
  return (int)hipMemcpyFromSymbol(out, HIP_SYMBOL(g_eprof), sizeof(unsigned long long) * (size_t)n);
}
extern "C" __attribute__((visibility("default"))) int fd_debug_ens_profile_next(void) { return g_eprof_next; }
extern "C" __attribute__((visibility("default"))) int fd_debug_ens_clock(unsigned long long* out, int n) {
  return (int)hipMemcpyFromSymbol(out, HIP_SYMBOL(g_eclk), sizeof(unsigned long long) * (size_t)n);
}
extern "C" __attribute__((visibility("default"))) int fd_debug_ens_clock_next(void) { return g_eclk_next; }
#endif

namespace {
struct Pair {
  int sa = -1, sb = -1, pa = -1, pb = -1, ma = -1, mb = -1;
};

bool select_pair(Engine& e, const fd_blend_params& p, const int32_t* slots, const uint8_t* present, int64_t n,
                 Pair& q) {
  if (!e.ensemble_on || e.forest_variant != 0 || n <= 0) return false;
  if ((n + kTile - 1) / kTile < kSplitTiles) return false;
  int k = 0;
  for (int m = 0; m < p.n_models; ++m) {
    if (present && !present[m]) continue;
    const int s = slots[m];
    if (s < 0 || s >= kMaxSlots || !e.forests[s].loaded || e.forests[s].sparse_only) return false;
    const int kind = e.forests[s].kind;
    if (kind == FD_FOREST_XGB_BINARY_LOGISTIC && q.sa < 0) {
      q.sa = s;
      q.pa = k;
      q.ma = m;
    } else if (kind == FD_FOREST_SKLEARN_IFOREST && q.sb < 0) {
      q.sb = s;
      q.pb = k;
      q.mb = m;
    } else {
      return false;
    }
    ++k;
  }
  if (q.sa < 0 || q.sb < 0) return false;
  const bool wide = want_wide(e);
  if (!plan_current(e, e.ens, q.sa, q.sb, wide) && !build_plan(e, e.ens, q.sa, q.sb, wide)) return false;
  return true;
}
}

namespace {
void plan_args(const EnsemblePlan& P, const float* dX, int64_t n, int32_t ld, bool owner_fixed, EnsArgs& a) {
  a.X = dX;
  a.n = n;
  a.ld = ld;
  a.nf = P.nf;
  a.thr = P.thr.as<const float>();
  FD_REQUIRE(P.nf <= kMaxFeatures, FD_ERR_UNSUPPORTED, "ensemble: more than 64 features");
  for (int f = 0; f <= P.nf; ++f) a.thr_off[f] = P.h_thr_off[f];
  a.owner_fixed = owner_fixed ? 1 : 0;
  for (int f = 0; f < kMaxFeatures; ++f) a.cbin[f] = f < (int)P.h_cbin.size() ? P.h_cbin[f] : 0;
  for (size_t k = 0; k < P.h_lut.size() && k < sizeof(a.lut) / sizeof(a.lut[0]); ++k) a.lut[k] = P.h_lut[k];
  a.vec4 = (ld % 4 == 0 && (reinterpret_cast<uintptr_t>(dX) & 15u) == 0) ? 1 : 0;
  const EnsPassSet& ps = P.passes;
  a.n_pass = (int)ps.f.size() - 1;
  for (int p = 0; p <= a.n_pass; ++p) {
    a.pass_f[p] = ps.f[p];
    a.img_off[p] = ps.img_off[p];
  }
  a.pass_global = ps.glob;
  a.img = P.img.as<const char>();
  for (int q = 0; q < 2; ++q) {
    a.nodes[q] = P.nodes[q].as<const char>();
    a.n_chunks[q] = P.n_chunks[q];
    a.stride[q] = (int)P.stride[q];
  }
  a.base_margin = P.base_margin;
  a.if_offset = P.if_offset;
  a.if_denom = P.if_denominator;
}

bool run_plan(Engine& e, const EnsemblePlan& P, EnsArgs& a, int out, int timing_kind) {
  const void* fn = pick_ensemble(out, P.wide, P.D);
  if (!fn) return false;
  const size_t lds = ens_lds(P.nf, P.wide);
  FD_HIP(hipFuncSetAttribute(fn, hipFuncAttributeMaxDynamicSharedMemorySize, (int)lds));
  const int64_t blocks = (a.n + kTile - 1) / kTile;
  Engine::Timed* ev = e.timing ? e.next_event_pair(timing_kind) : nullptr;
  if (ev) FD_HIP(hipEventRecord(ev->a, e.stream));
#ifdef FD_FOREST_PROFILE
  a.prof_slot = g_eprof_next;
  g_eprof_next = (g_eprof_next + 1) % kEprofSlots;
  a.clk_slot = g_eclk_next;
  g_eclk_next = (g_eclk_next + 1) % kEclkSlots;
#endif
  void* args[] = {&a};
  FD_HIP(hipLaunchKernel(fn, dim3((unsigned)blocks), dim3(kEnsWG), args, lds, e.stream));
  if (ev) FD_HIP(hipEventRecord(ev->b, e.stream));
  return true;
}
}

bool ensemble_applies(Engine& e, const fd_blend_params& p, const int32_t* slots, const uint8_t* present, int64_t n) {
  Pair q;
  return select_pair(e, p, slots, present, n, q);
}

bool launch_ensemble(Engine& e, const fd_blend_params& p, const int32_t* slots, const uint8_t* present,
                     const float* dX, int64_t n, int32_t ld, double* dMP, double* dfp, double* dconf, uint8_t* ddec,
                     uint8_t* drisk, const RouteRecord* records, ResultRecord* results, int compact) {
  Pair q;
  if (!select_pair(e, p, slots, present, n, q)) return false;
  const int pa = q.pa, pb = q.pb, ma = q.ma, mb = q.mb;
  EnsArgs a{};
  plan_args(e.ens, dX, n, compact ? kCompactWidth : ld, e.ens_owner_fixed, a);
  a.compact = compact;
  if (compact && e.ens_bin_global) {
    a.n_pass = 1;
    a.pass_f[0] = 0;
    a.pass_f[1] = e.ens.nf;
    a.pass_global = 1ull;
  }
  a.prio = e.ens_prio ? 1 : 0;
  a.pos[0] = pa;
  a.pos[1] = pb;
  a.mcol[0] = ma;
  a.mcol[1] = mb;
  a.blend = blend_consts(p, present);
  a.mp = dMP;
  a.fp = dfp;
  a.conf = dconf;
  a.dec = ddec;
  a.risk = drisk;
  a.rec = records;
  a.res = results;
  const int out = results ? 1 : 0;
  FD_REQUIRE(out == 1 || dfp != nullptr, FD_ERR_INVALID_ARG, "null output");
  return run_plan(e, e.ens, a, out, FD_TIMING_ENSEMBLE);
}

bool launch_ensemble_single(Engine& e, int slot, const float* dX, int64_t n, int32_t ld, double* dprob,
                            double* draw, hipStream_t stream) {
  if (!e.ensemble_on || e.forest_variant != 0 || n <= 0) return false;
  if ((n + kTile - 1) / kTile < kSplitTiles) return false;
  if (slot < 0 || slot >= kMaxSlots || !e.forests[slot].loaded || e.forests[slot].sparse_only) return false;
  const bool xgb = e.forests[slot].kind == FD_FOREST_XGB_BINARY_LOGISTIC;
  const int sa = xgb ? slot : -1, sb = xgb ? -1 : slot;
  EnsemblePlan& P = e.ens1[slot];
  const bool wide = want_wide(e);
  if (!plan_current(e, P, sa, sb, wide) && !build_plan(e, P, sa, sb, wide)) return false;
  EnsArgs a{};
  plan_args(P, dX, n, ld, e.ens_owner_fixed, a);
  a.prio = e.ens_prio ? 1 : 0;
  a.fp = dprob;
  a.mp = draw;
  const hipStream_t saved = e.stream;
  if (stream) e.stream = stream;
  bool ok = false;
  try {
    ok = run_plan(e, P, a, 2, xgb ? FD_TIMING_XGB : FD_TIMING_IFOREST);
  } catch (...) {
    e.stream = saved;
    throw;
  }
  e.stream = saved;
  if (ok) ++e.ens_single_total;
  return ok;
}


}
```

### realtime-fraud-detection_amd/csrc/fd_internal.h

```cpp
#pragma once

#include <hip/hip_runtime.h>

#include <atomic>
#include <chrono>
#include <condition_variable>
#include <cstddef>
#include <cstdint>
#include <mutex>
#include <stdexcept>
#include <string>
#include <thread>
#include <vector>

#include "fdengine.h"
#include "key_hash.h"

namespace fd {

constexpr int kMaxSlots = 8;
constexpr int kTile = 256;
constexpr int kGatherBatchMax = 4096;
constexpr int kMaxFeatures = 64;
constexpr int kCompactWidth = 16;
// ... 19 lines not shown
  for (int k = 0; k < kCompactSlots; ++k)
    if (kCompactSlot[k] == f) return k;
  return (f == 12 || f == 24 || f == 25 || f == 33 || f == 34) ? -2 : -1;
}
constexpr int kMaxDepth = 10;
constexpr int64_t kSparseMaxNodes = 1ll << 24;
constexpr size_t kLdsBudget = 160 * 1024;
constexpr int kMaxBins = 65534;
constexpr int kSplitTiles = 128;
constexpr int kSeqInput = 16;
constexpr unsigned long long kSeqMaterialized = 1ull << 63;
constexpr int kLstmHidden = 128;

#ifdef FD_FOREST_PROFILE
constexpr int kTlKernels = 8;
#define FD_TL_BUF(name) __device__ unsigned long long name[fd::kTlKernels * 1024 * 4]
#define FD_TL(buf, kid, k)                                                                            \
  do {                                                                                                \
    const unsigned tl_b = blockIdx.x + blockIdx.y * gridDim.x;                                        \
    if (threadIdx.x == 0 && tl_b < 1024u) buf[((kid) * 1024 + tl_b) * 4 + (k)] = __builtin_amdgcn_s_memrealtime(); \
  } while (0)
#else
#define FD_TL(buf, kid, k) \
  do {                     \
  } while (0)
#endif

struct Error : std::runtime_error {
  int code;
  Error(int c, const std::string& m) : std::runtime_error(m), code(c) {}
};

void set_error(const std::string& msg);

#define FD_HIP(call)                                                                       \
  do {                                                                                     \
    hipError_t _e = (call);                                                                \
    if (_e != hipSuccess)                                                                  \
      throw ::fd::Error(FD_ERR_HIP, std::string(#call) + ": " + hipGetErrorString(_e));    \
  } while (0)

#define FD_REQUIRE(cond, code, msg)              \
  do {                                           \
    if (!(cond)) throw ::fd::Error((code), (msg)); \
  } while (0)


struct DeviceBuffer {
  void* ptr = nullptr;
  size_t bytes = 0;
  void ensure(size_t need) {
    if (need <= bytes) return;
    release();
    FD_HIP(hipMalloc(&ptr, need));
    bytes = need;
  }
  void ensure_headroom(size_t need) {
    if (need > bytes) ensure(need + need / 4);
  }
  void release() {
    if (ptr) (void)hipFree(ptr);
    ptr = nullptr;
    bytes = 0;
  }
  template <class T>
  T* as() const { return static_cast<T*>(ptr); }
};

struct SplitScratch {
  DeviceBuffer bins, nan, leaves;
};

struct PreBin {
  const float* thr[2] = {};
  const int32_t* thr_off[2] = {};
  uint32_t* bins[2] = {};
  uint32_t* nan[2] = {};
  int nf[2] = {};
  int64_t n = 0, n_pad = 0;
  int ld = 0;
  int steps[2] = {};
  bool thr_nonempty = false;
  const void* fx = nullptr;
  const void* ff = nullptr;
  const float* X = nullptr;
  bool want = false, done = false;
};

struct SparseImage {
  DeviceBuffer nodes, leaf_val, leaf_ids;
  int64_t n_nodes = 0, n_leaves = 0;
  uint64_t gen = 0;
};

struct PackedForest {
  bool loaded = false;
  bool sparse_only = false;
  mutable SparseImage sp;
  int kind = 0;
  int n_trees = 0;
  int n_chunks = 0;
  int chunk = 0;
  int depth = 0;
  int num_feature = 0;
  size_t tree_bytes = 0;
  size_t chunk_stride = 0;
  float base_margin = 0.f;
  double if_offset = 0.0;
  double if_denominator = 0.0;
  DeviceBuffer blob;
  DeviceBuffer leaf_ids;
  bool binned = false;
  int b_chunk = 0, b_n_chunks = 0, bin_steps = 0;
  size_t b_tree_bytes = 0, b_chunk_stride = 0;
  DeviceBuffer b_blob;
  DeviceBuffer b_thr;
  DeviceBuffer b_thr_off;
  int b_n_thr = 0;
  int n_chunk = 0, n_n_chunks = 0;
  size_t n_chunk_stride = 0;
  DeviceBuffer n_blob;
  DeviceBuffer n_leaves;
  mutable SplitScratch split;
  uint64_t gen = 0;
  fd_forest_params params{};
  std::vector<int64_t> t_off;
  std::vector<int32_t> t_left, t_right, t_feature;
  std::vector<double> t_threshold, t_leaf;
  std::vector<uint8_t> t_dleft;
};

struct EnsPassSet {
  std::vector<int> f, img_off;
  unsigned long long glob = 0;
};

struct EnsemblePlan {
  bool valid = false;
  bool wide = true;
  int slot[2] = {-1, -1};
  uint64_t gen[2] = {0, 0};
  int n_forests = 0, D = 0, nf = 0;
  int kind[2] = {0, 0}, n_trees[2] = {0, 0}, CH[2] = {0, 0}, n_chunks[2] = {0, 0};
  size_t stride[2] = {0, 0};
  float base_margin = 0.f;
  double if_offset = 0.0, if_denominator = 0.0;
  DeviceBuffer nodes[2], thr;
  std::vector<int32_t> h_thr_off;
  std::vector<uint16_t> h_cbin;
  std::vector<uint16_t> h_lut;
  DeviceBuffer img;
  EnsPassSet passes;
  int max_feature_thr = 0;
};

struct __attribute__((aligned(16))) RouteRecord {
  unsigned long long key;
  long long ts;
  long long cents;
  unsigned long long dfp;
  int merchant;
  unsigned seq;
  unsigned char ipc, hour, wk;
  unsigned char pm;
  unsigned flags;
};
struct __attribute__((aligned(8))) ResultRecord {
  double fraud_prob;
  double confidence;
  unsigned seq;
  unsigned char decision, risk;
  unsigned short pad;
};

struct LstmModel {
  bool loaded = false;
  int input_size = 0, n_out = 0;
  DeviceBuffer wpk, wpk4, bias, wout, bout;
  bool hh_finite = false;
};

constexpr int kGraphChunk = 16384;
struct GraphState {
  bool ready = false;
  int H = 0;
  int cap = 0;
  int cur = 0;
  int64_t total = 0;
  int64_t base = 0;
  DeviceBuffer log[2];
  DeviceBuffer dm;
  unsigned long long steps = 0;
};

constexpr int kTextChunk = 65536;
struct TextState {
  DeviceBuffer acc;
  DeviceBuffer count;
  unsigned long long calls = 0;
};

struct AbTest {
  bool live = false;
  uint64_t salt = 0;
  double threshold = 0.0;
};
struct AbState {
  AbTest tests[FD_AB_MAX_TESTS];
  DeviceBuffer state;
  DeviceBuffer partials;
  DeviceBuffer part;
  DeviceBuffer index;
  DeviceBuffer rows;
};
struct AbScatter {
  const int32_t* idx;
  int64_t n;
  int64_t count[2];
  int models[2];
  int m_max;
  const double *p_fp, *p_conf;
  const uint8_t *p_dec, *p_risk;
  const double* p_mp[2];
  double *fp, *conf;
  uint8_t *dec, *risk;
  double* mp;
};

struct MlpModel {
  bool loaded = false;
  bool hot = false;
  int n_layers = 0;
  int dims[9] = {};
  int words = 0;
  int cus = 0, occ_ref = 1, occ_lds = 1;
  DeviceBuffer blob;
};

struct __attribute__((aligned(128))) CardHeader {
  long long last_ts;
  unsigned char ring_n, ring_head;
  unsigned char unsorted;
  unsigned char pad0;
  unsigned char wc[3], pad1;
  unsigned flags;
  int rc_cnt;
  long long ws[3];
  unsigned wod[3];
  unsigned pad2;
  unsigned long long key;
  double avg;
  int age;
  int pad3;
  unsigned long long fp[3];
  long long pad4[2];
};
static_assert(sizeof(CardHeader) == 128, "CardHeader must be one 128-B line");
static_assert(offsetof(CardHeader, key) == 64 && offsetof(CardHeader, wod) + sizeof(unsigned) * 3 <= 64,
              "the mutable fields in bytes 0-63, the key at 64 (snapshot.hip reads it there)");
constexpr int kCardHeaderBytes = (int)sizeof(CardHeader);

struct __attribute__((aligned(16))) RingEvent {
  long long ts;
  long long cents;
};

struct CardPages {
  char* base;
  long long stride;
  __host__ __device__ __forceinline__ CardHeader* hdr(long long s) const {
    return reinterpret_cast<CardHeader*>(base + s * stride);
  }
  __host__ __device__ __forceinline__ RingEvent* ring(long long s) const {
    return reinterpret_cast<RingEvent*>(base + s * stride + kCardHeaderBytes);
  }
};

#ifdef __HIP_DEVICE_COMPILE__
#define FD_CARD_SLOT_QUAL __device__ __forceinline__
#else
#define FD_CARD_SLOT_QUAL __device__ inline
#endif
FD_CARD_SLOT_QUAL long long card_slot(unsigned long long* keys, CardPages pg, long long mask, unsigned long long key) {
  if (key == 0ull) key = 1ull;
  long long h = (long long)(fmix64(key) & (unsigned long long)mask);
  if (mask >= 7) {
    long long g = h & ~7ll;
    int j0 = (int)(h & 7);
    for (long long p = 0; p <= mask + 8; p += 8) {
      const uint4* q = reinterpret_cast<const uint4*>(keys + g);
      uint4 w[4];
#pragma unroll
      for (int u = 0; u < 4; ++u) w[u] = q[u];
#pragma unroll
      for (int j = 0; j < 8; ++j) {
        if (j < j0) continue;
        const uint4 v = w[j >> 1];
        const unsigned long long k = (j & 1) ? (((unsigned long long)v.w << 32) | v.z)
                                             : (((unsigned long long)v.y << 32) | v.x);
        if (k == key) return g + j;
        if (k == 0ull) {
          const unsigned long long old = atomicCAS(&keys[g + j], 0ull, key);
          if (old == 0ull) {
            pg.hdr(g + j)->key = key;
            return g + j;
          }
          if (old == key) return g + j;
// ... 51 lines not shown
struct WindowState {
  bool ready = false;
  int64_t cap = 0, cand_cap = 0;
  int64_t ooo = 10000;
  int64_t wm = INT64_MIN;
  int64_t min_seen = INT64_MAX;
  int64_t max_seen = INT64_MIN;
  bool observed = false;
  DeviceBuffer ulog[2], mlog[2];
  int ucur = 0, mcur = 0;
  int64_t ucount = 0, mcount = 0;
  DeviceBuffer keys, vals, sort_tmp, uout, mout, scalars;
};

struct SinkState {
  bool ready = false;
  unsigned long long cap = 0, ucap = 0;
  DeviceBuffer table, users, err;
};

struct IngestTables {
  DeviceBuffer mkeys, mvals, vkeys[3], vvals[3];
  unsigned long long mmask = 0, vmask[3] = {0, 0, 0};
  bool mloaded = false, vloaded[3] = {false, false, false};
  int stop_after = 0;
};

struct ShardComm {
  bool ready = false;
  bool aborted = false;
  std::string abort_reason;
  int rank = 0, world = 1;
  const void* api = nullptr;
  void* fwd = nullptr;
  void* back = nullptr;
  hipStream_t x_fwd = nullptr;
  DeviceBuffer rec[2], cnt[2], back_buf;
  static constexpr int kInbox = 3;
  DeviceBuffer inbox[kInbox];
  DeviceBuffer res[kInbox];
  hipEvent_t in_ev[kInbox] = {}, inbox_ev[kInbox] = {};
  bool inbox_live[kInbox] = {};
  int inbox_next = 0;
  int inbox_of[2] = {0, 0};
  DeviceBuffer route_blk;
  int64_t* h_cnt[2] = {nullptr, nullptr};
  int64_t* d_hcnt[2] = {nullptr, nullptr};
  unsigned long long cnt_seq[2] = {0, 0};
  bool pending = false;
  unsigned long long pending_id = 0;
  int64_t pending_n = 0;
  int pending_slot = 0, next_slot = 0;
  int64_t split[2][2 * FD_MAX_SHARDS] = {};
  int64_t timeout_ms = 120000;
  int count_mode = -1;
  bool count_gather = false;
  int device = 0;
  static constexpr int kHostPhases = 8;
  std::atomic<unsigned long long> steps{0}, host_ns[kHostPhases] = {};
  std::atomic<unsigned long long> ops{0};
};
inline const char* const kShardHostPhase[ShardComm::kHostPhases] = {
    "wait", "partition", "counts", "count_copy", "records", "score", "back", "scatter"};
struct HostLaps {
  ShardComm& c;
  std::chrono::steady_clock::time_point t = std::chrono::steady_clock::now();
  void operator()(int ph) {
    const auto now = std::chrono::steady_clock::now();
    c.host_ns[ph].fetch_add((unsigned long long)std::chrono::duration_cast<std::chrono::nanoseconds>(now - t).count(),
                            std::memory_order_relaxed);
    t = now;
  }
};

inline int64_t floor_div_host(int64_t a, int64_t b) {
  int64_t q = a / b;
  if ((a % b != 0) && ((a < 0) != (b < 0))) --q;
  return q;
}

struct Engine {
  int device = 0;
  hipStream_t own_stream = nullptr;
  hipStream_t stream = nullptr;
  PackedForest forests[kMaxSlots];
  CardStore state;
  LstmModel lstm;
  MlpModel mlp;
  unsigned long long mlp_total = 0;
  GraphState graph;
  TextState text;
  AbState ab;
  WindowState windows;
  IngestTables ingest;
  SinkState sink;
  hipStream_t aux_stream = nullptr;
  hipEvent_t fork_ev = nullptr, join_ev = nullptr;
  hipStream_t aux2_stream = nullptr;
  hipEvent_t join2_ev = nullptr;
  DeviceBuffer seq_buf;
  DeviceBuffer seq_desc;
  DeviceBuffer feat_vec, feat_ext;
  static constexpr int kPipeSlots = 2;
  hipStream_t pipe_stream[2] = {nullptr, nullptr};
  static constexpr int kDoneRing = 4;
  hipEvent_t pipe_entry_ev = nullptr, pipe_feat_ev[kPipeSlots] = {}, pipe_done_ev[kDoneRing] = {};
  bool pipe_feat_live[kPipeSlots] = {}, pipe_done_live[kDoneRing] = {};
  bool pipe_dirty = true;
  int pipe_slot_mode = -1;
  hipStream_t pipe_slot_stream = nullptr;
  hipEvent_t pipe_slot_ev[kPipeSlots] = {};
  hipStream_t slot_pass_stream = nullptr;
  hipEvent_t slot_pass_ev = nullptr;
  unsigned long long pipe_iter = 0;
  unsigned long long pipe_iter_total = 0;
  unsigned long long sparse_total = 0;
  unsigned long long ens_single_total = 0;
  unsigned long long pipe_split_total = 0;
  unsigned long long pipe_compact_total = 0;
  unsigned long long pipe_host_ns = 0;
  unsigned long long pipe_slot_stream_total = 0;
  bool pipe_lean = true;
  bool pipe_gather = true;
  DeviceBuffer pipe_vec[kPipeSlots], pipe_seq[kPipeSlots];
  static constexpr int kSplitRing = 4;
  static_assert(kSplitRing == kDoneRing, "the split-row ring's buffers are released by the done events");
  DeviceBuffer pipe_split[kSplitRing];
  DeviceBuffer pipe_out[kPipeSlots];
  hipEvent_t pipe_copy_ev[kPipeSlots] = {};
  bool pipe_copy_live[kPipeSlots] = {};
  bool pipe_copy_vec[kPipeSlots] = {};
  int small_streams = 0;
  bool latency_fused = true;
  bool seq_ring_lstm = true;
  bool latency_prebin = true;
  int latency_prebin_mode = 3;
  PreBin prebin;
  unsigned long long prebin_total = 0;
  bool ens_prio = true;
  bool ens_bin_global = false;
  int compact_vectors = 2;
  int stream_prio = 3;
  DeviceBuffer stage;
  DeviceBuffer scratch_probs;
  DeviceBuffer route_blk, route_out, route_err;
  DeviceBuffer route_blk_stream;
  ShardComm comm;
  EnsemblePlan ens;
  EnsemblePlan ens1[kMaxSlots];
  bool route_err_live = false;
  int forest_variant = 0;
  bool ens_owner_fixed = true;
  int ens_chunks = 0;
  int mlp_form = 0;
  int mlp_wgs_per_cu = 0;
  int lstm_rows = 0;
  bool ensemble_on = true;
  bool timing = false;
  int timing_every = 1;
  unsigned long long timing_seq[16] = {};
  struct Timed {
    hipEvent_t a, b;
    int kind;
    hipEvent_t c = nullptr, d = nullptr;
    bool split = false;
  };
  std::vector<Timed> events;
  size_t events_used = 0;
  void activate() const { FD_HIP(hipSetDevice(device)); }
  Timed* next_event_pair(int kind);
};

struct HostPack {
  std::vector<char> blob;
  std::vector<int32_t> leaf_ids;
  int kind = 0, n_trees = 0, n_chunks = 0, chunk = 0, depth = 0, num_feature = 0;
  size_t tree_bytes = 0, chunk_stride = 0;
  float base_margin = 0.f;
  bool binned = false;
  std::vector<char> b_blob;
  std::vector<float> b_thr;
  std::vector<int32_t> b_thr_off;
  int b_chunk = 0, b_n_chunks = 0, bin_steps = 0;
  size_t b_tree_bytes = 0, b_chunk_stride = 0;
  std::vector<char> n_blob, n_leaves;
  int n_chunk = 0, n_n_chunks = 0;
  size_t n_chunk_stride = 0;
  std::vector<uint8_t> pad;
};
HostPack pack_forest_host(const fd_forest_params& p, const fd_tree_arrays& t, int min_depth = 0);
void repack_forest(PackedForest& pf, const fd_forest_params& p, const fd_tree_arrays& t);
float sklearn_threshold_to_lt(double thr);
struct SparsePack {
  std::vector<uint32_t> nodes;
  std::vector<char> leaf_val;
  std::vector<int32_t> leaf_ids;
  int kind = 0, n_trees = 0, depth = 0, num_feature = 0, leaf_bytes = 0;
  int64_t n_nodes = 0, n_leaves = 0;
  float base_margin = 0.f;
};
SparsePack pack_forest_sparse_host(const fd_forest_params& p, const fd_tree_arrays& t);
int forest_depth_probe(const fd_tree_arrays& t);
void load_forest_sparse(PackedForest& pf, const fd_forest_params& p, const fd_tree_arrays& t);
void launch_forest_sparse(Engine& e, const PackedForest& pf, const float* d_X, int64_t n, int32_t ld, double* d_prob,
                          double* d_raw, int32_t* d_leaf, hipStream_t stream);
bool launch_forest_pair(Engine& e, const PackedForest& pa, const PackedForest& pb, const float* d_X, int64_t n,
                        int32_t ld, double* d_prob_a, double* d_prob_b);
void launch_forest(Engine& e, const PackedForest& pf, const float* d_X, int64_t n, int32_t ld,
                   double* d_prob, double* d_raw, int32_t* d_leaf, hipStream_t stream = nullptr);
struct BlendConsts;
bool launch_forest_pair_blend(Engine& e, const PackedForest& p1, const PackedForest& p2, const float* d_X, int64_t n,
                              int32_t ld, const BlendConsts& bc, const double* const* cols, int pos1, int pos2,
                              double* dfp, double* dconf, uint8_t* ddec, uint8_t* drisk,
                              hipEvent_t before_blend = nullptr);
bool forest_pair_prebin(Engine& e, const PackedForest& p1, const PackedForest& p2, const float* d_X, int64_t n,
                        int32_t ld);
void windows_init(Engine& e, const fd_window_params& p);
void windows_step(Engine& e, const fd_txn_batch& t, const fd_window_inputs& in, int64_t n, bool flush,
                  fd_user_window* u_out, int64_t u_cap, int64_t* n_user, fd_merchant_window* m_out, int64_t m_cap,
                  int64_t* n_merch);
void windows_release(Engine& e);
void windows_observe(Engine& e, int64_t max_event_ts);
void merchant_windows_merge(const fd_merchant_window* p, int64_t n, fd_merchant_window* out, int64_t* n_out);
void ingest_set_vocab(Engine& e, int which, const uint8_t* bytes, const int64_t* offsets, int64_t n);
void ingest_set_merchants(Engine& e, const uint8_t* bytes, const int64_t* offsets, int64_t n);
void launch_ingest(Engine& e, const uint8_t* d_bytes, const int64_t* d_offsets, int64_t n, const fd_ingest_out& out);
void sink_init(Engine& e, const fd_sink_params& p);
void sink_update(Engine& e, const fd_txn_batch& t, const fd_window_inputs& in, int64_t n);
void sink_query(Engine& e, int kind, const int64_t* bucket, const int32_t* merchant, int64_t n, fd_aggregate* out);
void sink_evict_before(Engine& e, int64_t hour, int64_t* kept_entries, int64_t* kept_users);
void sink_release(Engine& e);
void state_snapshot(Engine& e, const char* path, int shard, int n_shards, int64_t* bytes_written);
void state_restore(Engine& e, const char* path, int shard, int n_shards, int flags, int64_t* cards_restored);
void state_init(Engine& e, const fd_state_params& p);
void state_clear(Engine& e);
int64_t state_count(Engine& e);
void load_users(Engine& e, const fd_users& u);
void load_merchants(Engine& e, const fd_merchants& m);
void launch_features(Engine& e, const fd_txn_batch& t, int64_t n, float* d_vec, double* d_raw,
                     float* d_seq = nullptr, double* d_vel5 = nullptr, hipStream_t stream = nullptr,
                     bool lean = false, int set = 0, hipEvent_t before_buckets = nullptr, int compact = 0,
                     unsigned long long* d_seq_desc = nullptr);
void launch_features_records(Engine& e, const void* d_records, int64_t n, float* d_vec, float* d_seq,
                             hipStream_t stream = nullptr, bool lean = false, int set = 0,
                             hipEvent_t before_buckets = nullptr, int compact = 0);
void load_users_ext(Engine& e, const fd_users_ext& u);
void load_merchants_ext(Engine& e, const fd_merchants_ext& m);
void load_vocab(Engine& e, const uint8_t* pay_high_risk, const uint8_t* type_refund);
void launch_features_full(Engine& e, const fd_txn_batch& t, const fd_txn_context& c, int64_t n, float* d_vec,
                          double* d_raw, double* d_fmap, fd_rule_scores* d_rules);
void features_check(Engine& e);
hipStream_t make_stream(int level);
unsigned shard_of_host(unsigned long long key, unsigned G);
void launch_route_partition(Engine& e, const fd_txn_batch& t, const fd_window_inputs* extra, int64_t n, int G,
                            void* d_records, int64_t* d_counts, hipStream_t stream = nullptr,
                            DeviceBuffer* scratch = nullptr, bool timed = true);
void launch_route_count(const fd_txn_batch& t, int64_t n, int G, int64_t* totals, hipStream_t st, DeviceBuffer& blk);
struct CountPublish {
  int64_t* cnt;
  int G;
  int gather_rank;
  int64_t* h;
  unsigned long long* h_seq;
  unsigned long long seq;
};
void launch_route_place(const fd_txn_batch& t, int64_t n, int G, void* d_records, hipStream_t st, DeviceBuffer& blk,
                        const CountPublish* pub = nullptr);
void launch_route_unpack(Engine& e, const void* d_records, const void* d_results, int64_t n, const fd_txn_batch& out,
                         uint8_t* pm, uint8_t* fraud, double* score);
void launch_result_pack(Engine& e, const double* fp, const double* conf, const uint8_t* dec, const uint8_t* risk,
                        const RouteRecord* records, int64_t n, void* d_results);
void launch_result_scatter(Engine& e, const void* d_results, int64_t n, double* fp, double* conf, uint8_t* dec,
                           uint8_t* risk);
void route_check(Engine& e);
void comm_unique_id(const char* rccl_path, uint8_t* out);
void comm_init(Engine& e, const char* rccl_path, int rank, int world, const uint8_t* id_fwd, const uint8_t* id_back);
void comm_destroy(Engine& e);
void comm_abort(Engine& e, const std::string& reason);
bool comm_sync_stream(Engine& e, hipStream_t st);
void comm_launch_counts(Engine& e, const fd_txn_batch& t, int64_t n, hipEvent_t ready, int slot, HostLaps& L);
void comm_wait_counts(Engine& e, int slot, int64_t n, HostLaps& L);
void comm_forward_group(Engine& e, int slot, const fd_txn_batch* next, int64_t next_n, hipEvent_t next_ready,
                        int next_slot, HostLaps& L);
void comm_exchange(Engine& e, bool back, hipStream_t st, const void* sendbuf, const int64_t* send, void* recvbuf,
                   const int64_t* recv, size_t elem);
void load_lstm(Engine& e, const fd_lstm_params& p);
void launch_lstm(Engine& e, hipStream_t stream, const float* d_seq, int64_t n, int T, double* d_prob,
                 const unsigned long long* d_desc = nullptr);
std::vector<uint32_t> pack_mlp_host(const fd_mlp_params& p);
void load_mlp(Engine& e, const fd_mlp_params& p);
void launch_mlp(Engine& e, hipStream_t stream, const float* d_X, int64_t n, int32_t ld, double* d_prob);
void graph_init(Engine& e, const fd_graph_params& p);
void graph_clear(Engine& e);
void graph_release(Engine& e);
void graph_info(Engine& e, int64_t* total, int64_t* held);
void graph_step(Engine& e, const fd_txn_batch& t, int64_t n, double* d_out);
void text_release(Engine& e);
int64_t text_nonascii_rows(Engine& e);
void text_features(Engine& e, const uint8_t* d_bytes, const int64_t* d_off, int64_t n, double* d_feat,
                   uint8_t* d_patterns, uint8_t* d_status);
const AbTest& ab_test(Engine& e, int id);
void ab_create(Engine& e, int id, const fd_ab_params& p);
void ab_destroy(Engine& e, int id);
void ab_clear(Engine& e, int id);
void ab_release(Engine& e);
void ab_assign(Engine& e, int id, const uint64_t* d_keys, int64_t n, uint8_t* d_variant);
// ... 28 lines not shown
```

### realtime-fraud-detection_amd/fdengine/_native.py

```python
from __future__ import annotations

import ctypes as C
import os
from pathlib import Path

PKG_ROOT = Path(__file__).resolve().parent.parent
REPO_ROOT = PKG_ROOT.parent
LIB_PATH = Path(os.environ.get("FDENGINE_LIB", PKG_ROOT / "lib" / "libfdengine.so"))

FD_OK = 0
FD_ERR_INVALID_ARG = 1
FD_ERR_HIP = 2
FD_ERR_NOT_LOADED = 3
FD_ERR_UNSUPPORTED = 4
FD_ERR_OOM = 5
FD_ERR_IO = 6
FD_RESTORE_SKIP_WINDOWS = 1
FD_RESTORE_SKIP_SINK = 2

FD_FOREST_XGB_BINARY_LOGISTIC = 1
FD_FOREST_SKLEARN_IFOREST = 2
FD_FOREST_SKLEARN_PROBA = 3

FD_MAX_MODELS = 8
# ... 221 lines not shown
FD_SLOT_MLP = 65
FD_GRAPH_FEATURES = 5
GRAPH_COLUMNS = ("user_centrality", "merchant_centrality", "clustering_coefficient", "path_length_anomaly",
                 "community_anomaly")
FD_TEXT_FIELDS = 4
FD_TEXT_PATTERNS = 5
FD_TEXT_FEATURES = 14
FD_TEXT_NONASCII = 1
TEXT_FIELDS = ("merchant_name", "description", "category", "location")
TEXT_COLUMNS = ("merchant_name_length", "description_length", "total_text_length", "merchant_name_unique_chars",
                "merchant_name_char_diversity", "numbers_in_merchant", "numbers_in_description", "total_numbers",
                "special_chars_merchant", "special_chars_description", "total_special_chars", "merchant_word_count",
                "description_word_count", "total_word_count")
TEXT_PATTERNS = ("crypto_keywords", "gift_card_keywords", "urgent_language", "suspicious_merchant",
                 "known_scam_patterns")
FD_AB_MAX_TESTS = 8
FD_AB_NO_LABEL = 255
FD_SEQ_INPUT = 16
FD_MAX_SHARDS = 64
FD_ROUTE_RECORD_BYTES = 48
FD_RESULT_RECORD_BYTES = 24
FD_WINDOW_REDIS_COMPAT = 0
FD_WINDOW_SLIDING = 1
FD_RAW_FEATURES = 16
FD_VECTOR_WIDTH = 64
TXN_FIELDS = ("card_key", "ts_ms", "amount_cents", "merchant", "device_fp", "ip_class", "hour", "weekend")

_vp = C.c_void_p
_i32 = C.c_int32
_i64 = C.c_int64
_dp = C.POINTER(C.c_double)

SIGNATURES = {
    "fd_last_error": (C.c_char_p, []),
    "fd_build_id": (C.c_char_p, []),
    "fd_abi_version": (C.c_int, []),
    "fd_device_count": (C.c_int, [C.POINTER(C.c_int)]),
    "fd_engine_create": (C.c_int, [C.c_int, C.POINTER(_vp)]),
    "fd_engine_destroy": (C.c_int, [_vp]),
    "fd_engine_set_stream": (C.c_int, [_vp, _vp]),
    "fd_engine_reset_stream": (C.c_int, [_vp]),
    "fd_engine_sync": (C.c_int, [_vp]),
    "fd_load_forest": (C.c_int, [_vp, C.c_int, C.POINTER(fd_forest_params), C.POINTER(fd_tree_arrays)]),
    "fd_unload_forest": (C.c_int, [_vp, C.c_int]),
    "fd_load_xgboost_json": (C.c_int, [_vp, C.c_int, C.c_char_p]),
    "fd_xgboost_json_read": (C.c_int, [C.c_char_p, C.POINTER(fd_forest_params), C.POINTER(_i32), C.POINTER(_i64),
                                       C.POINTER(fd_tree_arrays)]),
    "fd_forest_info": (C.c_int, [_vp, C.c_int, C.POINTER(_i32), C.POINTER(_i32), C.POINTER(_i32)]),
    "fd_forest_predict_device": (C.c_int, [_vp, C.c_int, _vp, _i64, _i32, _vp, _vp, _vp]),
    "fd_forest_predict_host": (C.c_int, [_vp, C.c_int, _vp, _i64, _i32, _vp, _vp, _vp]),
    "fd_blend_device": (C.c_int, [_vp, C.POINTER(fd_blend_params), _i64, C.POINTER(_vp), _vp, _vp, _vp, _vp, _vp]),
    "fd_blend_host": (C.c_int, [_vp, C.POINTER(fd_blend_params), _i64, C.POINTER(_vp), _vp, _vp, _vp, _vp, _vp]),
    "fd_score_matrix_device": (C.c_int, [_vp, C.POINTER(fd_blend_params), _vp, C.POINTER(_vp), _vp, _vp, _i64, _i32,
                                         _vp, _vp, _vp, _vp, _vp]),
    "fd_score_matrix_host": (C.c_int, [_vp, C.POINTER(fd_blend_params), _vp, C.POINTER(_vp), _vp, _vp, _i64, _i32,
                                       _vp, _vp, _vp, _vp, _vp]),
    "fd_state_init": (C.c_int, [_vp, C.POINTER(fd_state_params)]),
    "fd_state_clear": (C.c_int, [_vp]),
    "fd_state_info": (C.c_int, [_vp, C.POINTER(_i64), C.POINTER(_i64)]),
    "fd_state_load_users_host": (C.c_int, [_vp, C.POINTER(fd_users)]),
    "fd_load_merchants_host": (C.c_int, [_vp, C.POINTER(fd_merchants)]),
    "fd_features_device": (C.c_int, [_vp, C.POINTER(fd_txn_batch), _i64, _vp, _vp]),
    "fd_features_host": (C.c_int, [_vp, C.POINTER(fd_txn_batch), _i64, _vp, _vp]),
    "fd_score_batch_device": (C.c_int, [_vp, C.POINTER(fd_blend_params), _vp, C.POINTER(_vp), _vp,
                                        C.POINTER(fd_txn_batch), _i64, _vp, _vp, _vp, _vp, _vp, _vp]),
    "fd_score_batch_pipelined": (C.c_int, [_vp, C.POINTER(fd_blend_params), _vp, C.POINTER(_vp), _vp,
                                           C.POINTER(fd_txn_batch), _i64, _vp, _vp, _vp, _vp, _vp, _vp, _vp]),
    "fd_state_load_users_ext_host": (C.c_int, [_vp, C.POINTER(fd_users_ext)]),
    "fd_load_merchants_ext_host": (C.c_int, [_vp, C.POINTER(fd_merchants_ext)]),
    "fd_load_vocab_host": (C.c_int, [_vp, _vp, _vp]),
    "fd_features_full_device": (C.c_int, [_vp, C.POINTER(fd_txn_batch), C.POINTER(fd_txn_context), _i64, _vp, _vp,
                                          _vp, _vp]),
    "fd_load_lstm": (C.c_int, [_vp, C.POINTER(fd_lstm_params)]),
    "fd_unload_lstm": (C.c_int, [_vp]),
    "fd_lstm_predict_device": (C.c_int, [_vp, _vp, _i64, _i32, _vp]),
    "fd_lstm_predict_host": (C.c_int, [_vp, _vp, _i64, _i32, _vp]),
    "fd_load_mlp": (C.c_int, [_vp, C.POINTER(fd_mlp_params)]),
    "fd_unload_mlp": (C.c_int, [_vp]),
    "fd_mlp_info": (C.c_int, [_vp, C.POINTER(_i32), C.POINTER(_i32), C.POINTER(_i32)]),
    "fd_mlp_predict_device": (C.c_int, [_vp, _vp, _i64, _i32, _vp]),
    "fd_mlp_predict_host": (C.c_int, [_vp, _vp, _i64, _i32, _vp]),
    "fd_pack_mlp_host": (C.c_int, [C.POINTER(fd_mlp_params), _vp, _i64, C.POINTER(_i64)]),
    "fd_graph_init": (C.c_int, [_vp, C.POINTER(fd_graph_params)]),
    "fd_graph_clear": (C.c_int, [_vp]),
    "fd_graph_info": (C.c_int, [_vp, C.POINTER(_i64), C.POINTER(_i64)]),
    "fd_graph_step_device": (C.c_int, [_vp, C.POINTER(fd_txn_batch), _i64, _vp]),
    "fd_graph_step_host": (C.c_int, [_vp, C.POINTER(fd_txn_batch), _i64, _vp]),
    "fd_graph_features_host": (C.c_int, [_vp, _vp, _vp, _i64, _i32, _vp]),
    "fd_text_features_device": (C.c_int, [_vp, C.POINTER(fd_text_batch), _i64, _vp, _vp, _vp]),
    "fd_text_features_host": (C.c_int, [_vp, C.POINTER(fd_text_batch), _i64, _vp, _vp, _vp]),
    "fd_text_features_ref_host": (C.c_int, [_vp, _vp, _i64, _vp, _vp, _vp]),
    "fd_ab_create": (C.c_int, [_vp, _i32, C.POINTER(fd_ab_params)]),
    "fd_ab_destroy": (C.c_int, [_vp, _i32]),
    "fd_ab_clear": (C.c_int, [_vp, _i32]),
    "fd_ab_assign_device": (C.c_int, [_vp, _i32, _vp, _i64, _vp]),
    "fd_ab_assign_host": (C.c_int, [_vp, _i32, _vp, _i64, _vp]),
    "fd_ab_partition_device": (C.c_int, [_vp, _vp, _i64, _vp, _vp]),
    "fd_ab_partition_host": (C.c_int, [_vp, _vp, _i64, _vp, _vp]),
    "fd_ab_score_matrix_device": (C.c_int, [_vp, _i32, C.POINTER(fd_ab_model_set), C.POINTER(fd_ab_model_set), _vp,
                                            _vp, _i64, _i32, _vp, _vp, _vp, _vp, _vp, _vp]),
    "fd_ab_score_matrix_host": (C.c_int, [_vp, _i32, C.POINTER(fd_ab_model_set), C.POINTER(fd_ab_model_set), _vp,
                                          _vp, _i64, _i32, _vp, _vp, _vp, _vp, _vp, _vp]),
    "fd_ab_record_device": (C.c_int, [_vp, _i32, _vp, _vp, _vp, _vp, C.c_double, _vp, _i64]),
    "fd_ab_record_host": (C.c_int, [_vp, _i32, _vp, _vp, _vp, _vp, C.c_double, _vp, _i64]),
    "fd_ab_state_host": (C.c_int, [_vp, _i32, C.POINTER(fd_ab_state)]),
    "fd_ab_state_merge_host": (C.c_int, [C.POINTER(fd_ab_state), C.POINTER(fd_ab_state), C.POINTER(fd_ab_state)]),
    "fd_ab_bucket_host": (C.c_int, [_vp, _i64, C.c_uint64, _vp]),
    "fd_ab_record_ref_host": (C.c_int, [_vp, _vp, _vp, _vp, C.c_double, _vp, _i64, C.POINTER(fd_ab_state)]),
    "fd_features_seq_device": (C.c_int, [_vp, C.POINTER(fd_txn_batch), _i64, _vp, _vp, _vp]),
    "fd_shard_of_host": (C.c_int, [_vp, _i64, _i32, _vp]),
    "fd_route_partition_device": (C.c_int, [_vp, C.POINTER(fd_txn_batch), _i64, _i32, _vp, _vp]),
    "fd_route_partition_ex_device": (C.c_int, [_vp, C.POINTER(fd_txn_batch), C.POINTER(fd_window_inputs), _i64, _i32,
                                               _vp, _vp]),
    "fd_route_unpack_device": (C.c_int, [_vp, _vp, _vp, _i64, C.POINTER(fd_txn_batch), _vp, _vp, _vp]),
    "fd_windows_observe": (C.c_int, [_vp, _i64]),
    "fd_merchant_windows_merge": (C.c_int, [_vp, _i64, _vp, C.POINTER(_i64)]),
    "fd_score_records_device": (C.c_int, [_vp, C.POINTER(fd_blend_params), _vp, _vp, _vp, _i64, _vp]),
    "fd_score_records_pipelined": (C.c_int, [_vp, C.POINTER(fd_blend_params), _vp, _vp, _vp, _i64, _vp, _vp]),
    "fd_comm_unique_id": (C.c_int, [C.c_char_p, _vp]),
    "fd_comm_init": (C.c_int, [_vp, C.c_char_p, _i32, _i32, _vp, _vp]),
    "fd_comm_destroy": (C.c_int, [_vp]),
    "fd_sharded_step": (C.c_int, [_vp, C.POINTER(fd_blend_params), _vp, _vp, C.POINTER(fd_txn_batch), _i64,
                                  C.c_uint64, _vp, C.POINTER(fd_txn_batch), _i64, C.c_uint64, _vp, _vp, _vp, _vp, _vp,
                                  _vp]),
    "fd_route_partition_stream": (C.c_int, [_vp, C.POINTER(fd_txn_batch), C.POINTER(fd_window_inputs), _i64, _i32,
                                            _vp, _vp, _vp]),
    "fd_route_scatter_results_device": (C.c_int, [_vp, _vp, _i64, _vp, _vp, _vp, _vp]),
    "fd_windows_init": (C.c_int, [_vp, C.POINTER(fd_window_params)]),
    "fd_windows_step_device": (C.c_int, [_vp, C.POINTER(fd_txn_batch), C.POINTER(fd_window_inputs), _i64, C.c_int,
                                         _vp, _i64, C.POINTER(_i64), _vp, _i64, C.POINTER(_i64)]),
    "fd_windows_step_host": (C.c_int, [_vp, C.POINTER(fd_txn_batch), C.POINTER(fd_window_inputs), _i64, C.c_int,
                                       _vp, _i64, C.POINTER(_i64), _vp, _i64, C.POINTER(_i64)]),
    "fd_windows_stats": (C.c_int, [_vp, C.POINTER(_i64), C.POINTER(_i64), C.POINTER(_i64)]),
    "fd_state_snapshot": (C.c_int, [_vp, C.c_char_p, _i32, _i32, C.POINTER(_i64)]),
    "fd_state_restore": (C.c_int, [_vp, C.c_char_p, _i32, _i32, _i32, C.POINTER(_i64)]),
    "fd_hash64": (C.c_int, [_vp, _i64, C.POINTER(C.c_uint64)]),
    "fd_sink_init": (C.c_int, [_vp, C.POINTER(fd_sink_params)]),
    "fd_sink_update_device": (C.c_int, [_vp, C.POINTER(fd_txn_batch), C.POINTER(fd_window_inputs), _i64]),
    "fd_sink_update_host": (C.c_int, [_vp, C.POINTER(fd_txn_batch), C.POINTER(fd_window_inputs), _i64]),
    "fd_sink_query_host": (C.c_int, [_vp, _i32, _vp, _vp, _i64, _vp]),
    "fd_sink_evict_before": (C.c_int, [_vp, _i64, C.POINTER(_i64), C.POINTER(_i64)]),
    "fd_ingest_set_vocab": (C.c_int, [_vp, _i32, _vp, _vp, _i64]),
    "fd_ingest_set_merchants": (C.c_int, [_vp, _vp, _vp, _i64]),
    "fd_ingest_json_device": (C.c_int, [_vp, _vp, _vp, _i64, C.POINTER(fd_ingest_out)]),
    "fd_ingest_json_host": (C.c_int, [_vp, _vp, _vp, _i64, C.POINTER(fd_ingest_out)]),
    "fd_ingest_scalar_host": (C.c_int, [_i32, _vp, _i32, _dp, C.POINTER(_i64), C.POINTER(_i32)]),
    "fd_engine_set_timing": (C.c_int, [_vp, C.c_int]),
    "fd_engine_set_option": (C.c_int, [_vp, C.c_char_p, _i64]),
    "fd_engine_get_counter": (C.c_int, [_vp, C.c_char_p, C.POINTER(_i64)]),
    "fd_timing_read": (C.c_int, [_vp, C.c_int, _dp, C.POINTER(_i64)]),
    "fd_timing_reset": (C.c_int, [_vp]),
    "fd_pack_forest_host": (C.c_int, [C.POINTER(fd_forest_params), C.POINTER(fd_tree_arrays), _vp, _i64, _vp, _i64,
                                      C.POINTER(fd_pack_info)]),
    "fd_pack_forest_binned_host": (C.c_int, [C.POINTER(fd_forest_params), C.POINTER(fd_tree_arrays), _vp, _i64,
                                             _vp, _i64, _vp, C.POINTER(fd_pack_info)]),
    "fd_pack_forest_sparse_host": (C.c_int, [C.POINTER(fd_forest_params), C.POINTER(fd_tree_arrays), _vp, _i64,
                                             _vp, _i64, _vp, _i64, C.POINTER(fd_sparse_info)]),
}


class NativeError(RuntimeError):
    def __init__(self, code: int, fn: str, msg: str):
        super().__init__(f"{fn} failed ({code}): {msg}")
        self.code = code


def _preload_hip_runtime() -> None:
    if os.environ.get("FDENGINE_HIP_RUNTIME", "") == "system":
        return
    import importlib.util
    try:
        spec = importlib.util.find_spec("torch")
    except (ImportError, ValueError):
        spec = None
    if spec is None or not spec.origin:
        return
    cand = Path(spec.origin).parent / "lib" / "libamdhip64.so"
    if cand.exists():
        C.CDLL(str(cand), mode=C.RTLD_GLOBAL)


def _load() -> C.CDLL:
    _preload_hip_runtime()
    if not LIB_PATH.exists():
        raise ImportError(
            f"libfdengine.so not found at {LIB_PATH}. Build it with "
            "`python -c 'import __graft_entry__ as g; g.build()'` (hipcc --offload-arch=gfx950). "
            "There is no CPU fallback for the scoring path.")
    lib = C.CDLL(str(LIB_PATH))
    for name, (res, args) in SIGNATURES.items():
        fn = getattr(lib, name)
        fn.restype = res
        fn.argtypes = args
    from . import _buildid
    src_pkg = Path(os.environ.get("FDENGINE_SRC_ROOT", PKG_ROOT))
    src_repo = Path(os.environ.get("FDENGINE_SRC_REPO", src_pkg.parent))
    if (src_pkg / "csrc").is_dir():
        _buildid.check(lib.fd_build_id().decode(), src_pkg, src_repo)
    return lib


lib = _load()


def check(code: int, fn: str) -> None:
    if code != FD_OK:
        msg = lib.fd_last_error().decode("utf-8", "replace")
        if code == FD_ERR_NOT_LOADED:
            raise ValueError(msg)
        raise NativeError(code, fn, msg)


def call(fn: str, *args) -> None:
    check(getattr(lib, fn)(*args), fn)
```

### realtime-fraud-detection_amd/fdengine/engine.py

```python
from __future__ import annotations

import ctypes as C
import os
from typing import Dict, Optional, Sequence

import numpy as np

from . import _native as N
from .forest import ForestArrays


def _ptr(a: Optional[np.ndarray]):
    return None if a is None else C.c_void_p(a.ctypes.data)


class FraudEngine:
    def __init__(self, device: int = 0):
        h = C.c_void_p()
        N.call("fd_engine_create", int(device), C.byref(h))
        self._h = h
        self.device = int(device)
        self.forests: Dict[int, dict] = {}

    def close(self) -> None:
# ... 531 lines not shown
        out = N.fd_ab_state()
        N.call("fd_ab_state_host", self._h, int(test_id), C.byref(out))
        return out

    def route_partition_device(self, txn_ptrs: dict, n: int, n_shards: int, records_ptr: int, counts_ptr: int) -> None:
        b = N.fd_txn_batch(*[int(txn_ptrs[f]) for f in N.TXN_FIELDS])
        N.call("fd_route_partition_device", self._h, C.byref(b), int(n), int(n_shards),
               C.c_void_p(records_ptr) if records_ptr else None, C.c_void_p(counts_ptr))

    def route_partition_ex_device(self, txn_ptrs: dict, extra_ptrs: Optional[dict], n: int, n_shards: int,
                                  records_ptr: int, counts_ptr: int) -> None:
        b = N.fd_txn_batch(*[int(txn_ptrs[f]) for f in N.TXN_FIELDS])
        wi = N.fd_window_inputs(*[int(extra_ptrs[f]) if extra_ptrs and extra_ptrs.get(f) else None
                                  for f in ("payment_method", "is_fraud")], None)
        N.call("fd_route_partition_ex_device", self._h, C.byref(b), C.byref(wi), int(n), int(n_shards),
               C.c_void_p(records_ptr) if records_ptr else None, C.c_void_p(counts_ptr))

    def route_partition_stream(self, txn_ptrs: dict, extra_ptrs: Optional[dict], n: int, n_shards: int,
                               records_ptr: int, counts_ptr: int, stream_ptr: int) -> None:
        b = N.fd_txn_batch(*[int(txn_ptrs[f]) for f in N.TXN_FIELDS])
        wi = N.fd_window_inputs(*[int(extra_ptrs[f]) if extra_ptrs and extra_ptrs.get(f) else None
                                  for f in ("payment_method", "is_fraud")], None)
        N.call("fd_route_partition_stream", self._h, C.byref(b), C.byref(wi), int(n), int(n_shards),
               C.c_void_p(records_ptr) if records_ptr else None, C.c_void_p(counts_ptr),
               C.c_void_p(int(stream_ptr)) if stream_ptr else None)

    def route_unpack_device(self, records_ptr: int, results_ptr: int, n: int, out_ptrs: dict, pm_ptr: int = 0,
                            fraud_ptr: int = 0, score_ptr: int = 0) -> None:
        opt = lambda p: C.c_void_p(p) if p else None
        b = N.fd_txn_batch(*[int(out_ptrs.get(f) or 0) or None for f in N.TXN_FIELDS])
        N.call("fd_route_unpack_device", self._h, opt(records_ptr), opt(results_ptr), int(n), C.byref(b),
               opt(pm_ptr), opt(fraud_ptr), opt(score_ptr))

    def score_records_device(self, params: N.fd_blend_params, slots: Sequence[int], records_ptr: int, n: int,
                             results_ptr: int, present: Optional[Sequence[int]] = None) -> None:
        M = params.n_models
        sl = np.array(list(slots) + [-1] * (N.FD_MAX_MODELS - len(slots)), np.int32)
        pres = np.array([1] * M if present is None else list(present), np.uint8)
        N.call("fd_score_records_device", self._h, C.byref(params), _ptr(sl), _ptr(pres),
               C.c_void_p(records_ptr) if records_ptr else None, int(n),
               C.c_void_p(results_ptr) if results_ptr else None)

    def score_records_pipelined(self, params: N.fd_blend_params, slots: Sequence[int], records_ptr: int, n: int,
                                results_ptr: int, input_ready: int = 0, present: Optional[Sequence[int]] = None) -> None:
        M = params.n_models
        sl = np.array(list(slots) + [-1] * (N.FD_MAX_MODELS - len(slots)), np.int32)
        pres = np.array([1] * M if present is None else list(present), np.uint8)
        N.call("fd_score_records_pipelined", self._h, C.byref(params), _ptr(sl), _ptr(pres),
               C.c_void_p(records_ptr) if records_ptr else None, int(n),
               C.c_void_p(results_ptr) if results_ptr else None, C.c_void_p(input_ready) if input_ready else None)

    @staticmethod
    def comm_unique_id(rccl_path: str) -> bytes:
        buf = (C.c_uint8 * 128)()
        N.call("fd_comm_unique_id", os.fsencode(rccl_path), C.cast(buf, C.c_void_p))
        return bytes(buf)

    def comm_init(self, rccl_path: str, rank: int, world: int, id_fwd: bytes, id_back: bytes) -> None:
        a = (C.c_uint8 * 128).from_buffer_copy(id_fwd)
        b = (C.c_uint8 * 128).from_buffer_copy(id_back)
        N.call("fd_comm_init", self._h, os.fsencode(rccl_path), int(rank), int(world), C.cast(a, C.c_void_p),
               C.cast(b, C.c_void_p))

    def comm_destroy(self) -> None:
        N.call("fd_comm_destroy", self._h)

    def sharded_scorer(self, params: N.fd_blend_params, slots: Sequence[int],
                       present: Optional[Sequence[int]] = None) -> "ShardedStep":
        return ShardedStep(self, params, slots, present)

    def route_scatter_results_device(self, results_ptr: int, n: int, fp_ptr: int, conf_ptr: int = 0,
                                     dec_ptr: int = 0, risk_ptr: int = 0) -> None:
        opt = lambda p: C.c_void_p(p) if p else None
        N.call("fd_route_scatter_results_device", self._h, opt(results_ptr), int(n), opt(fp_ptr), opt(conf_ptr),
               opt(dec_ptr), opt(risk_ptr))

    @staticmethod
    def blend_params(weights: Sequence[float], conf_mult: Sequence[float], strategy: int = 0,
                     fraud_threshold: float = 0.5, confidence_threshold: float = 0.7) -> N.fd_blend_params:
        p = N.fd_blend_params()
        p.n_models = len(weights)
        p.strategy = int(strategy)
        for i, (w, m) in enumerate(zip(weights, conf_mult)):
            p.weight[i] = float(w)
            p.conf_mult[i] = float(m)
        p.fraud_threshold = float(fraud_threshold)
        p.confidence_threshold = float(confidence_threshold)
        return p

    def blend(self, params: N.fd_blend_params, probs: Sequence[Optional[np.ndarray]]):
        M = params.n_models
        assert len(probs) == M
        n = next((len(p) for p in probs if p is not None), 0)
        cols = [None if p is None else np.ascontiguousarray(p, dtype=np.float64) for p in probs]
        present = np.array([0 if c is None else 1 for c in cols], np.uint8)
        arr = (C.c_void_p * N.FD_MAX_MODELS)()
        for i, c in enumerate(cols):
            arr[i] = None if c is None else c.ctypes.data
        fp = np.empty(n, np.float64)
        conf = np.empty(n, np.float64)
        dec = np.empty(n, np.uint8)
        risk = np.empty(n, np.uint8)
        N.call("fd_blend_host", self._h, C.byref(params), n, arr, _ptr(present), _ptr(fp), _ptr(conf),
               _ptr(dec), _ptr(risk))
        return fp, conf, dec, risk

    def score_matrix(self, params: N.fd_blend_params, slots: Sequence[int], X: np.ndarray,
                     ext_probs: Optional[Sequence[Optional[np.ndarray]]] = None,
                     present: Optional[Sequence[int]] = None):
        X = np.ascontiguousarray(np.asarray(X, dtype=np.float32))
        n, ld = X.shape
        M = params.n_models
        sl = np.array(list(slots) + [-1] * (N.FD_MAX_MODELS - len(slots)), np.int32)
        pres = np.array([1] * M if present is None else list(present), np.uint8)
        ext = (C.c_void_p * N.FD_MAX_MODELS)()
        keep = []
        for m in range(M):
            if sl[m] < 0 and pres[m]:
                col = np.ascontiguousarray(ext_probs[m], dtype=np.float64)
                keep.append(col)
                ext[m] = col.ctypes.data
        mp = np.empty((M, n), np.float64)
        fp = np.empty(n, np.float64)
        conf = np.empty(n, np.float64)
        dec = np.empty(n, np.uint8)
        risk = np.empty(n, np.uint8)
        N.call("fd_score_matrix_host", self._h, C.byref(params), _ptr(sl), ext, _ptr(pres), _ptr(X), n, ld,
               _ptr(mp), _ptr(fp), _ptr(conf), _ptr(dec), _ptr(risk))
        return mp, fp, conf, dec, risk

    def blend_device(self, params: N.fd_blend_params, n: int, prob_ptrs: Sequence[Optional[int]],
                     fp_ptr: int, conf_ptr: int = 0, dec_ptr: int = 0, risk_ptr: int = 0) -> None:
        present = np.array([0 if p is None else 1 for p in prob_ptrs], np.uint8)
        arr = (C.c_void_p * N.FD_MAX_MODELS)()
        for i, p in enumerate(prob_ptrs):
            arr[i] = p if p else None
        N.call("fd_blend_device", self._h, C.byref(params), int(n), arr, _ptr(present), C.c_void_p(fp_ptr),
               C.c_void_p(conf_ptr) if conf_ptr else None, C.c_void_p(dec_ptr) if dec_ptr else None,
               C.c_void_p(risk_ptr) if risk_ptr else None)


def pack_forest_host(fa: ForestArrays):
    p, t, keep = fa.c_structs()
    info = N.fd_pack_info()
    N.call("fd_pack_forest_host", C.byref(p), C.byref(t), None, 0, None, 0, C.byref(info))
    blob = np.empty(info.blob_bytes, np.uint8)
    ids = np.empty(info.n_leaf_ids, np.int32)
    N.call("fd_pack_forest_host", C.byref(p), C.byref(t), C.c_void_p(blob.ctypes.data), info.blob_bytes,
           C.c_void_p(ids.ctypes.data), info.n_leaf_ids, C.byref(info))
    del keep
    return blob.tobytes(), ids, info


def pack_forest_binned_host(fa: ForestArrays):
    p, t, keep = fa.c_structs()
    info = N.fd_pack_info()
    N.call("fd_pack_forest_binned_host", C.byref(p), C.byref(t), None, 0, None, 0, None, C.byref(info))
    blob = np.empty(info.blob_bytes, np.uint8)
    thr = np.empty(info.n_thresholds, np.float32)
    off = np.empty(fa.num_feature + 1, np.int32)
    N.call("fd_pack_forest_binned_host", C.byref(p), C.byref(t), C.c_void_p(blob.ctypes.data), info.blob_bytes,
           C.c_void_p(thr.ctypes.data), info.n_thresholds, C.c_void_p(off.ctypes.data), C.byref(info))
    del keep
    return blob.tobytes(), thr, off, info


def pack_forest_sparse_host(fa: ForestArrays):
    p, t, keep = fa.c_structs()
    info = N.fd_sparse_info()
    N.call("fd_pack_forest_sparse_host", C.byref(p), C.byref(t), None, 0, None, 0, None, 0, C.byref(info))
    nodes = np.empty((info.n_nodes, 2), np.uint32)
    vals = np.empty(info.n_leaves, np.float32 if info.leaf_bytes == 4 else np.float64)
    ids = np.empty(info.n_leaves, np.int32)
    N.call("fd_pack_forest_sparse_host", C.byref(p), C.byref(t), C.c_void_p(nodes.ctypes.data), info.n_nodes,
           C.c_void_p(vals.ctypes.data), info.n_leaves, C.c_void_p(ids.ctypes.data), info.n_leaves, C.byref(info))
    del keep
    return nodes, vals, ids, info


def read_xgboost_json_native(path) -> ForestArrays:
    p = N.fd_forest_params()
    nt, nn = C.c_int32(), C.c_int64()
    N.call("fd_xgboost_json_read", os.fsencode(str(path)), C.byref(p), C.byref(nt), C.byref(nn), None)
    T, M = nt.value, nn.value
    fa = ForestArrays(kind=p.kind, num_feature=p.num_feature, offsets=np.zeros(T + 1, np.int64),
                      left=np.zeros(M, np.int32), right=np.zeros(M, np.int32), feature=np.zeros(M, np.int32),
                      threshold=np.zeros(M, np.float64), default_left=np.zeros(M, np.uint8),
                      leaf_value=np.zeros(M, np.float64), base_score=p.base_score)
    _, t, keep = fa.c_structs()
    N.call("fd_xgboost_json_read", os.fsencode(str(path)), C.byref(p), C.byref(nt), C.byref(nn), C.byref(t))
    out = ForestArrays(kind=fa.kind, num_feature=fa.num_feature, offsets=keep["offsets"], left=keep["left"],
                       right=keep["right"], feature=keep["feature"], threshold=keep["threshold"],
                       default_left=keep["default_left"], leaf_value=keep["leaf_value"], base_score=p.base_score)
    return out


def shard_of(keys, n_shards: int) -> np.ndarray:
    k = np.ascontiguousarray(keys, np.uint64)
    out = np.empty(len(k), np.int32)
    N.call("fd_shard_of_host", _ptr(k), len(k), int(n_shards), _ptr(out))
    return out


def device_count() -> int:
    c = C.c_int()
    rc = N.lib.fd_device_count(C.byref(c))
    return c.value if rc == N.FD_OK else 0


def merge_merchant_windows(parts) -> np.ndarray:
    a = np.concatenate([np.asarray(p, N.MERCHANT_WINDOW_DTYPE) for p in parts]) if len(parts) else \
        np.zeros(0, N.MERCHANT_WINDOW_DTYPE)
    a = np.ascontiguousarray(a)
    out = np.zeros(max(len(a), 1), N.MERCHANT_WINDOW_DTYPE)
    m = C.c_int64()
    N.call("fd_merchant_windows_merge", a.ctypes.data if len(a) else None, len(a), out.ctypes.data, C.byref(m))
    return out[:m.value].copy()


class PipelinedScorer:

    def __init__(self, eng: FraudEngine, params: N.fd_blend_params, slots: Sequence[int],
                 present: Optional[Sequence[int]] = None, pipelined: bool = True):
        M = params.n_models
        self.eng = eng
        self.params = params
        self._sl = np.array(list(slots) + [-1] * (N.FD_MAX_MODELS - len(slots)), np.int32)
        self._pres = np.array([1] * M if present is None else list(present), np.uint8)
        self._ext = (C.c_void_p * N.FD_MAX_MODELS)()
        self._batch = N.fd_txn_batch()
        self.pipelined = pipelined
        self._fn = N.lib.fd_score_batch_pipelined if pipelined else N.lib.fd_score_batch_device
        self._args = [C.byref(params), _ptr(self._sl), self._ext, _ptr(self._pres), C.byref(self._batch)]

    def __call__(self, txn_ptrs: dict, n: int, fp_ptr: int, conf_ptr: int = 0, dec_ptr: int = 0, risk_ptr: int = 0,
                 input_ready: int = 0, vec_ptr: int = 0, model_probs_ptr: int = 0) -> None:
        b = self._batch
        for f in N.TXN_FIELDS:
            setattr(b, f, txn_ptrs[f])
        if self.pipelined:
            rc = self._fn(self.eng._h, *self._args, int(n), vec_ptr or None, model_probs_ptr or None, fp_ptr,
                          conf_ptr or None, dec_ptr or None, risk_ptr or None, input_ready or None)
            N.check(rc, "fd_score_batch_pipelined")
        else:
            rc = self._fn(self.eng._h, *self._args, int(n), vec_ptr or None, model_probs_ptr or None, fp_ptr,
                          conf_ptr or None, dec_ptr or None, risk_ptr or None)
            N.check(rc, "fd_score_batch_device")


class ShardedStep:

    def __init__(self, eng: FraudEngine, params: N.fd_blend_params, slots: Sequence[int],
                 present: Optional[Sequence[int]] = None):
        M = params.n_models
        self.eng, self.params = eng, params
        self._sl = np.array(list(slots) + [-1] * (N.FD_MAX_MODELS - len(slots)), np.int32)
        self._pres = np.array([1] * M if present is None else list(present), np.uint8)
        self._cur, self._next = N.fd_txn_batch(), N.fd_txn_batch()
        self.split_sizes = np.zeros(2 * 64, np.int64)
        self._fn = N.lib.fd_sharded_step

    def __call__(self, txn_ptrs: dict, n: int, fp_ptr: int, conf_ptr: int, dec_ptr: int, risk_ptr: int,
                 input_ready: int = 0, next_ptrs: Optional[dict] = None, next_n: int = 0, next_ready: int = 0,
                 batch_id: int = 0, next_id: int = 0) -> None:
        for f in N.TXN_FIELDS:
            setattr(self._cur, f, txn_ptrs[f])
        nxt = None
        if next_ptrs is not None:
            for f in N.TXN_FIELDS:
                setattr(self._next, f, next_ptrs[f])
            nxt = C.byref(self._next)
        rc = self._fn(self.eng._h, C.byref(self.params), self._sl.ctypes.data, self._pres.ctypes.data,
                      C.byref(self._cur), int(n), int(batch_id), input_ready or None, nxt, int(next_n), int(next_id),
                      next_ready or None, fp_ptr or None, conf_ptr or None, dec_ptr or None, risk_ptr or None,
                      self.split_sizes.ctypes.data)
        N.check(rc, "fd_sharded_step")
```

Measured before the change: 820.8 million.

## Contract forest trees by constant-folding splits on compacted-away features

Adds host-side tree contraction. Splits on features that the compact vector path fixes to constants are resolved at plan time, and the trees are repacked with per-tree or per-group reduced depths. New kernel variants read a per-tree depth and stop walking early, which cuts LDS node loads and steps per transaction. This is enabled by default (ens_contract=1, group-max depth) only when compact vectors are in use. The pipeline also allocates the per-slot vector buffer only when it is not using the split ring. Risks are extra plan-build cost, more kernel instantiations, and divergence if depths vary within a group.

```diff
diff --git a/include/fdengine.h b/include/fdengine.h
--- a/include/fdengine.h
+++ b/include/fdengine.h
@@ -103,6 +103,9 @@
 int fd_pack_forest_binned_host(const fd_forest_params* params, const fd_tree_arrays* trees, void* blob,
                                int64_t blob_cap, float* thresholds, int64_t thr_cap, int32_t* offsets,
                                fd_pack_info* info);
+
+int fd_contract_forest_host(const fd_forest_params* params, const fd_tree_arrays* trees, int64_t* n_nodes,
+                            fd_tree_arrays* out, int32_t* depths, int64_t* n_pruned);
 
 typedef struct {
   int32_t kind;
diff --git a/realtime-fraud-detection_amd/csrc/engine.hip b/realtime-fraud-detection_amd/csrc/engine.hip
--- a/realtime-fraud-detection_amd/csrc/engine.hip
+++ b/realtime-fraud-detection_amd/csrc/engine.hip
@@ -537,6 +537,12 @@
     *value = (int64_t)e.pipe_iter_total;
   } else if (k == "ensemble_single_launches") {
     *value = (int64_t)e.ens_single_total;
+  } else if (k == "ensemble_contracted_launches") {
+    *value = (int64_t)e.ens_contract_total;
+  } else if (k == "ensemble_nodes_pruned") {
+    *value = e.ens.valid ? (int64_t)e.ens.nodes_pruned : 0;
+  } else if (k == "ensemble_node_steps_per_txn") {
+    *value = (int64_t)e.ens_steps_last;
   } else if (k == "forest_sparse_launches") {
     *value = (int64_t)e.sparse_total;
   } else if (k == "mlp_launches") {
@@ -602,6 +608,13 @@
   } else if (k == "ensemble_chunks") {
     FD_REQUIRE(value >= 0 && value <= 2, FD_ERR_INVALID_ARG, "ensemble_chunks must be 0, 1 or 2");
     e.ens_chunks = (int)value;
+  } else if (k == "ensemble_contract") {
+    FD_REQUIRE(value >= 0 && value <= 2, FD_ERR_INVALID_ARG, "ensemble_contract must be 0, 1 or 2");
+    if ((int)value != e.ens_contract) {
+      e.activate();
+      FD_HIP(hipDeviceSynchronize());
+    }
+    e.ens_contract = (int)value;
   } else if (k == "compact_vectors") {
     FD_REQUIRE(value >= 0 && value <= 2, FD_ERR_INVALID_ARG, "compact_vectors must be 0, 1 or 2");
     e.compact_vectors = (int)value;
@@ -765,6 +778,32 @@
   FD_API_END
 }
 
+int fd_contract_forest_host(const fd_forest_params* params, const fd_tree_arrays* trees, int64_t* n_nodes,
+                            fd_tree_arrays* out, int32_t* depths, int64_t* n_pruned) {
+  FD_API_BEGIN
+  FD_REQUIRE(params && trees, FD_ERR_INVALID_ARG, "null params/trees");
+  const fd::ContractedForest c = fd::contract_forest_host(*params, *trees);
+  const int32_t T = (int32_t)c.off.size() - 1;
+  const int64_t M = (int64_t)c.left.size();
+  if (n_nodes) *n_nodes = M;
+  if (n_pruned) *n_pruned = (int64_t)c.pruned;
+  if (depths) std::memcpy(depths, c.depth.data(), (size_t)T * 4);
+  if (out) {
+    FD_REQUIRE(out->tree_offsets && out->left && out->right && out->feature && out->threshold && out->default_left &&
+                   out->leaf_value,
+               FD_ERR_INVALID_ARG, "incomplete output arrays");
+    out->n_trees = T;
+    std::memcpy(const_cast<int64_t*>(out->tree_offsets), c.off.data(), (size_t)(T + 1) * 8);
+    std::memcpy(const_cast<int32_t*>(out->left), c.left.data(), (size_t)M * 4);
+    std::memcpy(const_cast<int32_t*>(out->right), c.right.data(), (size_t)M * 4);
+    std::memcpy(const_cast<int32_t*>(out->feature), c.feature.data(), (size_t)M * 4);
+    std::memcpy(const_cast<double*>(out->threshold), c.threshold.data(), (size_t)M * 8);
+    std::memcpy(const_cast<uint8_t*>(out->default_left), c.dleft.data(), (size_t)M);
+    std::memcpy(const_cast<double*>(out->leaf_value), c.leaf.data(), (size_t)M * 8);
+  }
+  FD_API_END
+}
+
 int fd_pack_forest_binned_host(const fd_forest_params* params, const fd_tree_arrays* trees, void* blob,
                                int64_t blob_cap, float* thresholds, int64_t thr_cap, int32_t* offsets,
                                fd_pack_info* info) {
@@ -1176,8 +1215,7 @@
   hipEvent_t before_buckets = e.pipe_feat_live[prev] ? e.pipe_feat_ev[prev] : nullptr;
   int compact = (e.compact_vectors && d_vectors == nullptr && fd::ensemble_applies(e, *params, slots, present, n))
                     ? e.compact_vectors : 0;
-  e.pipe_vec[s].ensure((size_t)n * FD_VECTOR_WIDTH * 4);
-  float* vec = e.pipe_vec[s].as<float>();
+  float* vec = nullptr;
   const int sr = (int)(e.pipe_iter % (unsigned long long)Engine::kSplitRing);
   float* seq = nullptr;
   bool want_seq = false;
@@ -1195,6 +1233,9 @@
     e.pipe_split[sr].ensure((size_t)n * 64);
     vec = e.pipe_split[sr].as<float>();
     if (Ss && e.pipe_done_live[sr]) FD_HIP(hipStreamWaitEvent(Ss, e.pipe_done_ev[sr], 0));
+  } else {
+    e.pipe_vec[s].ensure((size_t)n * FD_VECTOR_WIDTH * 4);
+    vec = e.pipe_vec[s].as<float>();
   }
   {
     struct SlotPass {
diff --git a/realtime-fraud-detection_amd/csrc/ensemble.hip b/realtime-fraud-detection_amd/csrc/ensemble.hip
--- a/realtime-fraud-detection_amd/csrc/ensemble.hip
+++ b/realtime-fraud-detection_amd/csrc/ensemble.hip
@@ -25,6 +25,90 @@
     pf.t_dleft.assign((size_t)m, 0);
 }
 
+ContractedForest contract_forest_host(const fd_forest_params& p, const fd_tree_arrays& t) {
+  FD_REQUIRE(p.kind == FD_FOREST_XGB_BINARY_LOGISTIC || p.kind == FD_FOREST_SKLEARN_IFOREST, FD_ERR_INVALID_ARG,
+             "contraction: XGBoost binary:logistic or IsolationForest trees");
+  FD_REQUIRE(p.num_feature > 0 && p.num_feature <= kMaxFeatures, FD_ERR_UNSUPPORTED, "num_feature must be in [1, 64]");
+  FD_REQUIRE(forest_depth_probe(t) >= 0, FD_ERR_INVALID_ARG, "incomplete tree arrays or a tree that is not a tree");
+  const bool xgb = p.kind == FD_FOREST_XGB_BINARY_LOGISTIC;
+  ContractedForest c;
+  c.off.push_back(0);
+  struct Item {
+    int32_t o, lo, ro;
+    int depth;
+  };
+  std::vector<Item> st, keep;
+  std::vector<int32_t> remap;
+  for (int i = 0; i < t.n_trees; ++i) {
+    const int64_t a = t.tree_offsets[i], m = t.tree_offsets[i + 1] - a;
+    const int32_t *L = t.left + a, *R = t.right + a, *F = t.feature + a;
+    auto resolve = [&](int32_t o) {
+      while (L[o] >= 0) {
+        FD_REQUIRE(F[o] >= 0 && F[o] < p.num_feature, FD_ERR_INVALID_ARG, "split feature outside [0, num_feature)");
+        const int src = compact_src(F[o]);
+        if (src >= 0) break;
+        const float val = src == -2 ? 0.5f : 0.0f;
+        const float thr = xgb ? (float)t.threshold[a + o] : sklearn_threshold_to_lt(t.threshold[a + o]);
+        o = val < thr ? L[o] : R[o];
+      }
+      return o;
+    };
+    const int64_t base = (int64_t)c.left.size();
+    auto emit = [&](int32_t l, int32_t r, int32_t f, double thr, uint8_t dl, double leaf) {
+      c.left.push_back(l);
+      c.right.push_back(r);
+      c.feature.push_back(f);
+      c.threshold.push_back(thr);
+      c.dleft.push_back(dl);
+      c.leaf.push_back(leaf);
+      return (int32_t)((int64_t)c.left.size() - 1 - base);
+    };
+    int64_t splits_in = 0, splits_out = 0;
+    for (int64_t o = 0; o < m; ++o) splits_in += L[o] >= 0 ? 1 : 0;
+    int depth = 0;
+    const int32_t root = resolve(0);
+    if (L[root] < 0 && L[0] >= 0) {
+      emit(1, 2, 0, 0.0, 0, 0.0);
+      emit(-1, -1, 0, 0.0, 0, t.leaf_value[a + root]);
+      emit(-1, -1, 0, 0.0, 0, t.leaf_value[a + root]);
+      depth = 1;
+    } else {
+      st.clear();
+      st.push_back({root, 0, 0});
+      keep.clear();
+      while (!st.empty()) {
+        Item it = st.back();
+        st.pop_back();
+        depth = std::max(depth, it.depth);
+        if (L[it.o] >= 0) {
+          it.lo = resolve(L[it.o]);
+          it.ro = resolve(R[it.o]);
+          st.push_back({it.ro, 0, 0, it.depth + 1});
+          st.push_back({it.lo, 0, 0, it.depth + 1});
+        }
+        keep.push_back(it);
+      }
+      std::sort(keep.begin() + 1, keep.end(), [](const Item& x, const Item& y) { return x.o < y.o; });
+      remap.assign((size_t)m, -1);
+      for (size_t k = 0; k < keep.size(); ++k) remap[(size_t)keep[k].o] = (int32_t)k;
+      for (const Item& it : keep) {
+        const int32_t o = it.o;
+        if (L[o] < 0) {
+          emit(-1, -1, F[o], t.threshold[a + o], t.default_left ? t.default_left[a + o] : 0, t.leaf_value[a + o]);
+        } else {
+          ++splits_out;
+          emit(remap[(size_t)it.lo], remap[(size_t)it.ro], F[o], t.threshold[a + o],
+               t.default_left ? t.default_left[a + o] : 0, t.leaf_value[a + o]);
+        }
+      }
+    }
+    c.pruned += splits_in - splits_out;
+    c.depth.push_back(std::max(depth, 1));
+    c.off.push_back((int64_t)c.left.size());
+  }
+  return c;
+}
+
 namespace {
 
 constexpr int kEnsWG = 1024;
@@ -57,7 +141,7 @@
   int owner_fixed;
   int prio;
   int n_pass;
-  int pad0;
+  int ldepth;
   unsigned long long pass_global;
   const char* img;
   const char* nodes[2];
@@ -149,9 +233,103 @@
   return ((unsigned long long)hi << 32) | lo;
 }
 
+template <int TPG, bool NAN_AWARE>
+__device__ __forceinline__ void walk_ens_var(uint32_t buf, int t0, uint32_t lane4, const int (&d)[TPG],
+                                             uint32_t (&leaf)[TPG]) {
+  uint32_t tb[TPG], node[TPG], kl[TPG], kr[TPG], xw[TPG];
+  int dw = 1;
+#pragma unroll
+  for (int j = 0; j < TPG; ++j) {
+    tb[j] = buf + (uint32_t)(t0 + j) * 1024u;
+    asm volatile("" : "+v"(tb[j]));
+    node[j] = lds_load<uint32_t>(tb[j] + 4u);
+    dw = max(dw, d[j]);
+    leaf[j] = 0u;
+  }
+#pragma unroll
+  for (int j = 0; j < TPG; ++j) {
+    xw[j] = lds_load<uint16_t>((node[j] & 0xFC02u) | lane4);
+    const u32x2 k = lds_load<u32x2>(tb[j] + 8u);
+    kl[j] = k.x;
+    kr[j] = k.y;
+  }
+#pragma unroll
+  for (int l = 0; l < 8; ++l) {
+    if (l >= dw) break;
+#pragma unroll
+    for (int j = 0; j < TPG; ++j) {
+      bool right = xw[j] > (node[j] >> 16);
+      if (NAN_AWARE) {
+        if (xw[j] == 0xFFFFu) right = (node[j] & 1u) == 0u;
+      }
+      const uint32_t at = ((node[j] & kLinkMask) >> 2) + (right ? 1u : 0u);
+      leaf[j] = (l + 1 == d[j]) ? at : leaf[j];
+      node[j] = right ? kr[j] : kl[j];
+    }
+    if (l + 1 >= dw) break;
+#pragma unroll
+    for (int j = 0; j < TPG; ++j) {
+      if (l + 1 < d[j]) {
+        xw[j] = lds_load<uint16_t>((node[j] & 0xFC02u) | lane4);
+        if (l + 2 < d[j]) {
+          const u32x2 k = lds_load<u32x2>((node[j] & kLinkMask) | tb[j]);
+          kl[j] = k.x;
+          kr[j] = k.y;
+        }
+      }
+    }
+  }
+}
+
+template <int VD, int TPG>
+__device__ __forceinline__ unsigned long long walk_pack_var(uint32_t cur, int gg, uint32_t lane4, bool tile_nan) {
+  static_assert(TPG <= 8, "a byte per tree in a u64");
+  uint32_t leaf[TPG];
+  int d[TPG];
+#pragma unroll
+  for (int j = 0; j < TPG; ++j)
+    d[j] = __builtin_amdgcn_readfirstlane((int)lds_load<uint32_t>(cur + (uint32_t)(gg * TPG + j) * 1024u)) & 0xFF;
+  if (VD == 1) {
+    if (tile_nan)
+      walk_ens_var<TPG, true>(cur, gg * TPG, lane4, d, leaf);
+    else
+      walk_ens_var<TPG, false>(cur, gg * TPG, lane4, d, leaf);
+  } else {
+#define FD_WALK_DEPTH(K)                                          \
+  case K:                                                         \
+    if (tile_nan)                                                 \
+      walk_ens<K, TPG, true>(cur, gg * TPG, lane4, leaf);         \
+    else                                                          \
+      walk_ens<K, TPG, false>(cur, gg * TPG, lane4, leaf);        \
+    break;
+    switch (d[0]) {
+      FD_WALK_DEPTH(1)
+      FD_WALK_DEPTH(2)
+      FD_WALK_DEPTH(3)
+      FD_WALK_DEPTH(4)
+      FD_WALK_DEPTH(5)
+      FD_WALK_DEPTH(6)
+      FD_WALK_DEPTH(7)
+      default:
+        if (tile_nan)
+          walk_ens<8, TPG, true>(cur, gg * TPG, lane4, leaf);
+        else
+          walk_ens<8, TPG, false>(cur, gg * TPG, lane4, leaf);
+        break;
+    }
+#undef FD_WALK_DEPTH
+  }
+  uint32_t lo = 0, hi = 0;
+#pragma unroll
+  for (int j = 0; j < TPG; ++j) {
+    if (j < 4) lo |= leaf[j] << (8 * j);
+    else hi |= leaf[j] << (8 * (j - 4));
+  }
+  return ((unsigned long long)hi << 32) | lo;
+}
+
 template <int D, int TPG, int CH, typename LeafT>
-__device__ __forceinline__ void owner_sum(uint32_t buf, uint32_t tile, uint32_t acc, int txn) {
-  constexpr int NL = 1 << D;
+__device__ __forceinline__ void owner_sum(uint32_t buf, uint32_t tile, uint32_t acc, int txn, const int NL = 1 << D) {
   unsigned long long w[4];
 #pragma unroll
   for (int q = 0; q < 4; ++q) w[q] = lds_load<unsigned long long>(tile + (uint32_t)(q * kTile + txn) * 8u);
@@ -397,7 +575,7 @@
   }
 }
 
-template <int D, int OUT, bool WIDE, bool LUT = true>
+template <int D, int OUT, bool WIDE, bool LUT = true, int VD = 0>
 __global__ void __launch_bounds__(kEnsWG) ensemble_kernel(EnsArgs a) {
   constexpr int kCHA = EnsCfg<WIDE>::CHA, kCHB = EnsCfg<WIDE>::CHB;
   constexpr uint32_t kEnsBuf = EnsCfg<WIDE>::BUF;
@@ -417,6 +595,7 @@
   const int64_t row = (int64_t)blockIdx.x * kTile + txn;
   const bool valid = row < a.n;
   const int nA = a.n_chunks[0], G = nA + a.n_chunks[1];
+  const int NL = VD ? 1 << a.ldepth : 1 << D;
 
 #ifdef FD_FOREST_PROFILE
   unsigned long long pr_top = 0, pr_walk = 0, pr_sync = 0, pr_dma = 0, pr_st[8] = {0, 0, 0, 0, 0, 0, 0, 0};
@@ -600,8 +779,8 @@
       if (g > 0) {
         const int c = g - 1;
         const uint32_t bp = (c & 1) ? bufB : bufA, tp = (c & 1) ? tile1 : tile0;
-        if (c < nA) owner_sum<D, TPGA, kCHA, float>(bp, tp, accA, txn);
-        else owner_sum<D, TPGB, kCHB, double>(bp, tp, accB, txn);
+        if (c < nA) owner_sum<D, TPGA, kCHA, float>(bp, tp, accA, txn, NL);
+        else owner_sum<D, TPGB, kCHB, double>(bp, tp, accB, txn, NL);
         if (lane == 0)
           __hip_atomic_fetch_add(reinterpret_cast<uint32_t*>(lbase + (owner_cnt - s0)), 1u, __ATOMIC_RELAXED,
                                  __HIP_MEMORY_SCOPE_WORKGROUP);
@@ -617,8 +796,11 @@
     }
     const uint32_t cur = (g & 1) ? bufB : bufA, tw = (g & 1) ? tile1 : tile0;
     FD_ESTAMP(q1);
-    const unsigned long long w =
-        g < nA ? walk_pack<D, TPGA>(cur, gg, lane4, tile_nan) : walk_pack<D, TPGB>(cur, gg, lane4, tile_nan);
+    unsigned long long w;
+    if (VD)
+      w = g < nA ? walk_pack_var<VD, TPGA>(cur, gg, lane4, tile_nan) : walk_pack_var<VD, TPGB>(cur, gg, lane4, tile_nan);
+    else
+      w = g < nA ? walk_pack<D, TPGA>(cur, gg, lane4, tile_nan) : walk_pack<D, TPGB>(cur, gg, lane4, tile_nan);
     lds_store<unsigned long long>(tw + (uint32_t)(gg * kTile + txn) * 8u, w);
     FD_ESTAMP(q2);
     if (owner) dma_wait();
@@ -637,8 +819,8 @@
   if (G > 0 && gg == (a.owner_fixed ? 0 : ((G - 1) & 3))) {
     const int c = G - 1;
     const uint32_t bp = (c & 1) ? bufB : bufA, tp = (c & 1) ? tile1 : tile0;
-    if (c < nA) owner_sum<D, TPGA, kCHA, float>(bp, tp, accA, txn);
-    else owner_sum<D, TPGB, kCHB, double>(bp, tp, accB, txn);
+    if (c < nA) owner_sum<D, TPGA, kCHA, float>(bp, tp, accA, txn, NL);
+    else owner_sum<D, TPGB, kCHB, double>(bp, tp, accB, txn, NL);
   }
   __syncthreads();
 #ifdef FD_FOREST_PROFILE
@@ -729,6 +911,15 @@
 const void* pick_ensemble(int out, bool wide, int D) {
   if (wide) return out == 1 ? pick_ensemble<1, true>(D) : out == 2 ? pick_ensemble<2, true>(D) : pick_ensemble<0, true>(D);
   return out == 1 ? pick_ensemble<1, false>(D) : out == 2 ? pick_ensemble<2, false>(D) : pick_ensemble<0, false>(D);
+}
+
+const void* pick_ensemble_var(int out, bool wide, int vd) {
+  if (vd == 2) {
+    if (wide) return out == 1 ? (const void*)ensemble_kernel<8, 1, true, true, 2> : (const void*)ensemble_kernel<8, 0, true, true, 2>;
+    return out == 1 ? (const void*)ensemble_kernel<8, 1, false, true, 2> : (const void*)ensemble_kernel<8, 0, false, true, 2>;
+  }
+  if (wide) return out == 1 ? (const void*)ensemble_kernel<8, 1, true, true, 1> : (const void*)ensemble_kernel<8, 0, true, true, 1>;
+  return out == 1 ? (const void*)ensemble_kernel<8, 1, false, true, 1> : (const void*)ensemble_kernel<8, 0, false, true, 1>;
 }
 
 fd_tree_arrays arrays_of(const PackedForest& f) {
@@ -772,7 +963,7 @@
   }
 }
 
-bool build_plan(Engine& e, EnsemblePlan& P, int sa, int sb, bool wide) {
+bool build_plan(Engine& e, EnsemblePlan& P, int sa, int sb, bool wide, int contract = 0) {
   P.valid = false;
   const PackedForest* F[2] = {sa >= 0 ? &e.forests[sa] : nullptr, sb >= 0 ? &e.forests[sb] : nullptr};
   if (!F[0] && !F[1]) return false;
@@ -854,6 +1045,69 @@
     P.n_chunks[k] = nc;
     P.stride[k] = stride;
   }
+  P.contract = contract;
+  P.contracted = false;
+  P.nodes_pruned = 0;
+  P.steps_full = P.steps_c = 0;
+  for (int k = 0; k < 2 && contract; ++k) {
+    if (!F[k]) continue;
+    const bool xgb = F[k]->params.kind == FD_FOREST_XGB_BINARY_LOGISTIC;
+    const ContractedForest c = contract_forest_host(F[k]->params, arrays_of(*F[k]));
+    const int T = hp[k].n_trees, nc = P.n_chunks[k], ch = CH[k], tpg = ch / 4;
+    const size_t nb = (size_t)nc * ch;
+    std::vector<int> dw(nb, 1);
+    for (int i = 0; i < T; ++i) dw[i] = std::min(c.depth[i], D);
+    if (contract == 1)
+      for (size_t g0 = 0; g0 < nb; g0 += tpg) {
+        const int mx = *std::max_element(dw.begin() + g0, dw.begin() + g0 + tpg);
+        std::fill(dw.begin() + g0, dw.begin() + g0 + tpg, mx);
+      }
+    std::vector<char> blob((size_t)nc * P.stride[k], 0);
+    std::vector<int32_t> cur(2 * NL);
+    for (size_t i = 0; i < nb; ++i) {
+      char* chunk = blob.data() + (i / ch) * P.stride[k];
+      uint32_t* dst = reinterpret_cast<uint32_t*>(chunk + (i % ch) * 1024);
+      dst[0] = (uint32_t)dw[i];
+      const int nl = 1 << dw[i];
+      if ((int)i >= T) {
+        for (int s = 1; s < nl; ++s) dst[s] = (s < (nl >> 1) ? (uint32_t)s : (uint32_t)(s - (nl >> 1))) << 3;
+        continue;
+      }
+      P.steps_c += dw[i];
+      const int64_t a = c.off[i];
+      cur[1] = 0;
+      for (int s = 1; s < nl; ++s) {
+        const int32_t o = cur[s];
+        const uint32_t link = s < (nl >> 1) ? (uint32_t)s : (uint32_t)(s - (nl >> 1));
+        if (c.left[a + o] < 0) {
+          dst[s] = link << 3;
+          cur[2 * s] = cur[2 * s + 1] = o;
+          continue;
+        }
+        const uint32_t f = (uint32_t)c.feature[a + o];
+        const float thr = xgb ? (float)c.threshold[a + o] : sklearn_threshold_to_lt(c.threshold[a + o]);
+        const uint32_t jm = (uint32_t)(std::lower_bound(merged[f].begin(), merged[f].end(), thr) - merged[f].begin());
+        dst[s] = (jm << 16) | ((f >> 1) << 10) | (link << 3) | ((f & 1u) << 1) | (c.dleft[a + o] ? 1u : 0u);
+        cur[2 * s] = c.left[a + o];
+        cur[2 * s + 1] = c.right[a + o];
+      }
+      char* leaves = chunk + (size_t)ch * 1024 + (i % ch) * NL * leaf_sz[k];
+      for (int s = 0; s < nl; ++s) {
+        const double v = c.leaf[a + cur[nl + s]];
+        if (k == 0) {
+          const float vf = (float)v;
+          std::memcpy(leaves + (size_t)s * 4, &vf, 4);
+        } else {
+          std::memcpy(leaves + (size_t)s * 8, &v, 8);
+        }
+      }
+    }
+    P.nodes_c[k].ensure(blob.size());
+    FD_HIP(hipMemcpy(P.nodes_c[k].ptr, blob.data(), blob.size(), hipMemcpyHostToDevice));
+    P.nodes_pruned += c.pruned;
+  }
+  for (int k = 0; k < 2; ++k) P.steps_full += F[k] ? (long long)hp[k].n_trees * D : 0;
+  P.contracted = contract != 0 && P.steps_c < P.steps_full;
   P.thr.ensure(std::max<size_t>(4, thr.size() * sizeof(float)));
   if (!thr.empty()) FD_HIP(hipMemcpy(P.thr.ptr, thr.data(), thr.size() * sizeof(float), hipMemcpyHostToDevice));
   P.h_thr_off = off;
@@ -899,8 +1153,8 @@
   return true;
 }
 
-bool plan_current(const Engine& e, const EnsemblePlan& P, int sa, int sb, bool wide) {
-  return P.valid && P.wide == wide && P.slot[0] == sa && P.slot[1] == sb &&
+bool plan_current(const Engine& e, const EnsemblePlan& P, int sa, int sb, bool wide, int contract = 0) {
+  return P.valid && P.wide == wide && P.contract == contract && P.slot[0] == sa && P.slot[1] == sb &&
          P.gen[0] == (sa >= 0 ? e.forests[sa].gen : 0) && P.gen[1] == (sb >= 0 ? e.forests[sb].gen : 0);
 }
 
@@ -949,7 +1203,9 @@
   }
   if (q.sa < 0 || q.sb < 0) return false;
   const bool wide = want_wide(e);
-  if (!plan_current(e, e.ens, q.sa, q.sb, wide) && !build_plan(e, e.ens, q.sa, q.sb, wide)) return false;
+  if (!plan_current(e, e.ens, q.sa, q.sb, wide, e.ens_contract) &&
+      !build_plan(e, e.ens, q.sa, q.sb, wide, e.ens_contract))
+    return false;
   return true;
 }
 }
@@ -985,8 +1241,8 @@
   a.if_denom = P.if_denominator;
 }
 
-bool run_plan(Engine& e, const EnsemblePlan& P, EnsArgs& a, int out, int timing_kind) {
-  const void* fn = pick_ensemble(out, P.wide, P.D);
+bool run_plan(Engine& e, const EnsemblePlan& P, EnsArgs& a, int out, int timing_kind, int vd = 0) {
+  const void* fn = vd && out != 2 ? pick_ensemble_var(out, P.wide, vd) : pick_ensemble(out, P.wide, P.D);
   if (!fn) return false;
   const size_t lds = ens_lds(P.nf, P.wide);
   FD_HIP(hipFuncSetAttribute(fn, hipFuncAttributeMaxDynamicSharedMemorySize, (int)lds));
@@ -1041,7 +1297,15 @@
   a.res = results;
   const int out = results ? 1 : 0;
   FD_REQUIRE(out == 1 || dfp != nullptr, FD_ERR_INVALID_ARG, "null output");
-  return run_plan(e, e.ens, a, out, FD_TIMING_ENSEMBLE);
+  const int vd = (compact && e.ens.contracted) ? (e.ens.contract == 1 ? 2 : 1) : 0;
+  if (vd) {
+    for (int k = 0; k < 2; ++k) a.nodes[k] = e.ens.nodes_c[k].as<const char>();
+    a.ldepth = e.ens.D;
+  }
+  if (!run_plan(e, e.ens, a, out, FD_TIMING_ENSEMBLE, vd)) return false;
+  if (vd) ++e.ens_contract_total;
+  e.ens_steps_last = vd ? e.ens.steps_c : e.ens.steps_full;
+  return true;
 }
 
 bool launch_ensemble_single(Engine& e, int slot, const float* dX, int64_t n, int32_t ld, double* dprob,
diff --git a/realtime-fraud-detection_amd/csrc/fd_internal.h b/realtime-fraud-detection_amd/csrc/fd_internal.h
--- a/realtime-fraud-detection_amd/csrc/fd_internal.h
+++ b/realtime-fraud-detection_amd/csrc/fd_internal.h
@@ -195,7 +195,33 @@
   DeviceBuffer img;
   EnsPassSet passes;
   int max_feature_thr = 0;
-};
+  DeviceBuffer nodes_c[2];
+  int contract = 0;
+  bool contracted = false;
+  long long nodes_pruned = 0;
+  long long steps_full = 0, steps_c = 0;
+};
+
+struct ContractedForest {
+  std::vector<int64_t> off;
+  std::vector<int32_t> left, right, feature, depth;
+  std::vector<double> threshold, leaf;
+  std::vector<uint8_t> dleft;
+  long long pruned = 0;
+  fd_tree_arrays arrays() const {
+    fd_tree_arrays t{};
+    t.n_trees = (int32_t)off.size() - 1;
+    t.tree_offsets = off.data();
+    t.left = left.data();
+    t.right = right.data();
+    t.feature = feature.data();
+    t.threshold = threshold.data();
+    t.default_left = dleft.data();
+    t.leaf_value = leaf.data();
+    return t;
+  }
+};
+ContractedForest contract_forest_host(const fd_forest_params& p, const fd_tree_arrays& t);
 
 struct __attribute__((aligned(16))) RouteRecord {
   unsigned long long key;
@@ -553,6 +579,9 @@
   int forest_variant = 0;
   bool ens_owner_fixed = true;
   int ens_chunks = 0;
+  int ens_contract = 1;
+  unsigned long long ens_contract_total = 0;
+  long long ens_steps_last = 0;
   int mlp_form = 0;
   int mlp_wgs_per_cu = 0;
   int lstm_rows = 0;
diff --git a/realtime-fraud-detection_amd/fdengine/_native.py b/realtime-fraud-detection_amd/fdengine/_native.py
--- a/realtime-fraud-detection_amd/fdengine/_native.py
+++ b/realtime-fraud-detection_amd/fdengine/_native.py
@@ -397,6 +397,8 @@
     "fd_timing_reset": (C.c_int, [_vp]),
     "fd_pack_forest_host": (C.c_int, [C.POINTER(fd_forest_params), C.POINTER(fd_tree_arrays), _vp, _i64, _vp, _i64,
                                       C.POINTER(fd_pack_info)]),
+    "fd_contract_forest_host": (C.c_int, [C.POINTER(fd_forest_params), C.POINTER(fd_tree_arrays), C.POINTER(_i64),
+                                          C.POINTER(fd_tree_arrays), C.POINTER(C.c_int32), C.POINTER(_i64)]),
     "fd_pack_forest_binned_host": (C.c_int, [C.POINTER(fd_forest_params), C.POINTER(fd_tree_arrays), _vp, _i64,
                                              _vp, _i64, _vp, C.POINTER(fd_pack_info)]),
     "fd_pack_forest_sparse_host": (C.c_int, [C.POINTER(fd_forest_params), C.POINTER(fd_tree_arrays), _vp, _i64,
diff --git a/realtime-fraud-detection_amd/fdengine/engine.py b/realtime-fraud-detection_amd/fdengine/engine.py
--- a/realtime-fraud-detection_amd/fdengine/engine.py
+++ b/realtime-fraud-detection_amd/fdengine/engine.py
@@ -707,6 +707,26 @@
     return blob.tobytes(), ids, info
 
 
+def contract_forest_host(fa: ForestArrays):
+    p, t, keep = fa.c_structs()
+    nn, pruned = C.c_int64(), C.c_int64()
+    N.call("fd_contract_forest_host", C.byref(p), C.byref(t), C.byref(nn), None, None, None)
+    T, M = fa.n_trees, nn.value
+    out = ForestArrays(kind=fa.kind, num_feature=fa.num_feature, offsets=np.zeros(T + 1, np.int64),
+                       left=np.zeros(M, np.int32), right=np.zeros(M, np.int32), feature=np.zeros(M, np.int32),
+                       threshold=np.zeros(M, np.float64), default_left=np.zeros(M, np.uint8),
+                       leaf_value=np.zeros(M, np.float64), base_score=fa.base_score, if_offset=fa.if_offset,
+                       if_denominator=fa.if_denominator)
+    _, to, ko = out.c_structs()
+    depths = np.zeros(T, np.int32)
+    N.call("fd_contract_forest_host", C.byref(p), C.byref(t), C.byref(nn), C.byref(to),
+           depths.ctypes.data_as(C.POINTER(C.c_int32)), C.byref(pruned))
+    del keep
+    for name in ("offsets", "left", "right", "feature", "threshold", "default_left", "leaf_value"):
+        setattr(out, name, ko[name])
+    return out, depths, pruned.value
+
+
 def pack_forest_binned_host(fa: ForestArrays):
     p, t, keep = fa.c_structs()
     info = N.fd_pack_info()
```

After: 841.1 million, median of 6. +2.5%, better.
